# koide3/small_gicp

Measured on AMD Instinct MI355X. Metric: GICP iterations/sec (1M<->1M pts), higher is better.
Workload: dtype f32; 1 GPU; C3: GICP, per-point covariances k=20, 1000000 target <-> 1000000 source points, max_corr_dist 1.0 m; parallelism=single GPU

## Files before the change

include/small_gicp_amd_debug.h:

```cpp
#ifndef SMALL_GICP_AMD_DEBUG_H
#define SMALL_GICP_AMD_DEBUG_H

#include "small_gicp_amd.h"

#ifdef __cplusplus
extern "C" {
#endif

int sga_problem_set_search_stats(sga_context* ctx, sga_problem* pb, int enabled);
int sga_problem_get_search_stats(sga_context* ctx, const sga_problem* pb, int* leaves_per_point);
int sga_problem_get_sorted_points(sga_context* ctx, const sga_problem* pb, float* xyzw);
int sga_problem_get_last_plan(const sga_problem* pb, int out[8]);
int sga_problem_get_grid_stats(const sga_problem* pb, uint64_t out[6]);
void sga_set_grid_mode(int mode, long long min_points);
void sga_set_knn_wave_max(long long max_points);
int sga_index_spacing(const sga_index* index, double* spacing);
int sga_debug_kd_tree(sga_context* ctx, const sga_index* index, int* depth, float* nodes, float* xyzw);
int sga_debug_timer_start(sga_context* ctx);
int sga_debug_timer_stop(sga_context* ctx, double* ms);
#define SGA_FRAME_CHECK_DOUBLES 32
void sga_debug_shard_frame_pack(const double origin[3], double out[SGA_FRAME_CHECK_DOUBLES]);
int sga_debug_shard_frame_agree(const double sum[SGA_FRAME_CHECK_DOUBLES]);
int sga_debug_kd_trips(unsigned long long* out16);
int sga_debug_kd_wave_times(unsigned long long* out, int waves);

#ifdef __cplusplus
}
#endif
#endif
```

small_gicp_amd/_lib.py:

```python
import ctypes as C
import os
import sys

_HERE = os.path.dirname(os.path.abspath(__file__))
LIB_PATH = os.environ.get("SGA_LIB_PATH") or os.path.join(_HERE, "lib", "libsmall_gicp_amd.so")

SGA_OK = 0
ICP, PLANE_ICP, GICP = 0, 1, 2
FLAT_NORMALS, FLAT_COVS = 1, 2
ROBUST_NONE, ROBUST_HUBER, ROBUST_CAUCHY = 0, 1, 2
LEVENBERG_MARQUARDT, GAUSS_NEWTON = 0, 1
MATH_FP32, MATH_FP64 = 0, 1
ACCUM_DOUBLES = 30


class SgaError(RuntimeError):
    pass


class FactorParams(C.Structure):
    _fields_ = [("factor_kind", C.c_int), ("robust_kind", C.c_int), ("robust_c", C.c_double), ("max_dist_sq", C.c_double), ("math_mode", C.c_int)]


class RegistrationSettingC(C.Structure):
# ... 62 lines not shown
    ("sga_index_create_voxelmap_from_voxels", C.c_int, [_vp, C.c_double, C.c_void_p, _dp, _dp, C.c_size_t, _pvp]),
    ("sga_index_create_flatmap_from_voxels", C.c_int, [_vp, C.c_double, C.c_void_p, C.c_void_p, _dp, _dp, C.c_int, C.c_size_t, _pvp]),
    ("sga_index_refresh_attributes", C.c_int, [_vp, _vp, _vp]),
    ("sga_index_clone", C.c_int, [_vp, _vp, _pvp]),
    ("sga_index_destroy", C.c_int, [_vp]),
    ("sga_index_size", C.c_int, [_vp, C.POINTER(C.c_size_t)]),
    ("sga_index_voxelmap_download", C.c_int, [_vp, _vp, C.POINTER(C.c_int32), _fp, _fp, C.POINTER(C.c_uint32)]),
    ("sga_voxelmap_create", C.c_int, [_vp, C.c_double, _pvp]),
    ("sga_voxelmap_insert", C.c_int, [_vp, _vp, _vp, _dp]),
    ("sga_voxelmap_set_lru", C.c_int, [_vp, C.c_uint32, C.c_uint32]),
    ("sga_flatmap_create", C.c_int, [_vp, C.c_double, _pvp]),
    ("sga_flatmap_set_setting", C.c_int, [_vp, C.c_double, C.c_uint32]),
    ("sga_voxelmap_set_search_offsets", C.c_int, [_vp, C.c_int]),
    ("sga_flatmap_download", C.c_int, [_vp, _vp, C.POINTER(C.c_int32), C.POINTER(C.c_uint32), _fp, _fp]),
    ("sga_flatmap_create_contents", C.c_int, [_vp, C.c_double, C.c_int, _pvp]),
    ("sga_flatmap_get_contents", C.c_int, [_vp, C.POINTER(C.c_int)]),
    ("sga_flatmap_download_contents", C.c_int, [_vp, _vp, C.POINTER(C.c_int32), C.POINTER(C.c_uint32), _fp, _fp, _fp]),
    ("sga_index_create_flatmap_from_voxels_contents", C.c_int, [_vp, C.c_double, C.c_void_p, C.c_void_p, _dp, _dp, _dp, C.c_int, C.c_size_t, _pvp]),
    ("sga_index_knn", C.c_int, [_vp, _vp, _fp, C.c_size_t, C.c_int, C.c_double, C.POINTER(C.c_int64), _fp]),
    ("sga_index_knn_f64", C.c_int, [_vp, _vp, _dp, C.c_size_t, C.c_int, C.c_double, C.POINTER(C.c_int64), _dp]),
    ("sga_index_build_projective", C.c_int, [_vp, _vp, C.c_int, C.c_int, _pvp]),
    ("sga_projective_set_search_window", C.c_int, [_vp, C.c_int, C.c_int]),
    ("sga_projective_set_border_modes", C.c_int, [_vp, C.c_int, C.c_int]),
    ("sga_projective_get_params", C.c_int, [_vp, C.POINTER(C.c_int)]),
    ("sga_projective_download_map", C.c_int, [_vp, _vp, C.POINTER(C.c_uint32)]),
    ("sga_factor_params_default", None, [C.POINTER(FactorParams)]),
    ("sga_problem_create", C.c_int, [_vp, _vp, _vp, _dp, _pvp]),
    ("sga_problem_create_from_index", C.c_int, [_vp, _vp, _vp, _dp, _pvp]),
    ("sga_problem_destroy", C.c_int, [_vp]),
    ("sga_linearize", C.c_int, [_vp, _vp, C.POINTER(FactorParams), _dp, _dp, _dp, _dp, C.POINTER(C.c_uint64)]),
    ("sga_error", C.c_int, [_vp, _vp, C.POINTER(FactorParams), _dp, _dp]),
    ("sga_linearize_async", C.c_int, [_vp, _vp, C.POINTER(FactorParams), _dp, _vp]),
    ("sga_error_async", C.c_int, [_vp, _vp, C.POINTER(FactorParams), _dp, _vp]),
    ("sga_comm_unique_id", C.c_int, [C.POINTER(C.c_ubyte)]),
    ("sga_comm_init", C.c_int, [_vp, C.c_int, C.c_int, C.POINTER(C.c_ubyte)]),
    ("sga_comm_destroy", C.c_int, [_vp]),
    ("sga_comm_init_callback", C.c_int, [_vp, C.c_int, C.c_int, ALLREDUCE_FN, _vp]),
    ("sga_error_model_eval", C.c_int, [_dp, _dp, _dp, _dp]),
    ("sga_unpack_accumulator", None, [_dp, _dp, _dp, _dp, C.POINTER(C.c_uint64)]),
    ("sga_problem_set_rejector", C.c_int, [_vp, REJECTOR_FN, _vp]),
    ("sga_linearize_per_point", C.c_int, [_vp, _vp, C.POINTER(FactorParams), _dp, _dp, C.POINTER(C.c_ubyte)]),
    ("sga_problem_get_factors", C.c_int, [_vp, _vp, C.POINTER(C.c_int64), _fp]),
    ("sga_context_set_stream_ordered", C.c_int, [_vp, C.c_int]),
    ("sga_context_set_profiling", C.c_int, [_vp, C.c_int]),
    ("sga_context_get_kernel_ms", C.c_int, [_vp, _dp, C.POINTER(C.c_uint64), _dp, C.POINTER(C.c_uint64)]),
    ("sga_context_get_comm_ms", C.c_int, [_vp, _dp, C.POINTER(C.c_uint64)]),
    ("sga_context_get_search_ms", C.c_int, [_vp, _dp, C.POINTER(C.c_uint64)]),
    ("sga_context_get_pass_ms", C.c_int, [_vp, _dp, C.POINTER(C.c_uint64), _dp, C.POINTER(C.c_uint64), _dp]),
    ("sga_set_warm_limit", None, [C.c_double]),
    ("sga_set_error_model", None, [C.c_int]),
    ("sga_problem_set_search_stats", C.c_int, [C.c_void_p, C.c_void_p, C.c_int]),
    ("sga_problem_get_search_stats", C.c_int, [C.c_void_p, C.c_void_p, C.c_void_p]),
    ("sga_problem_get_sorted_points", C.c_int, [C.c_void_p, C.c_void_p, C.c_void_p]),
    ("sga_problem_get_grid_stats", C.c_int, [C.c_void_p, C.POINTER(C.c_uint64)]),
    ("sga_problem_get_last_plan", C.c_int, [C.c_void_p, C.POINTER(C.c_int)]),
    ("sga_set_grid_mode", None, [C.c_int, C.c_longlong]),
    ("sga_host_alloc", C.c_int, [C.c_size_t, C.POINTER(C.c_void_p)]),
    ("sga_host_free", C.c_int, [C.c_void_p]),
    ("sga_index_spacing", C.c_int, [C.c_void_p, C.POINTER(C.c_double)]),
    ("sga_set_knn_wave_max", None, [C.c_longlong]),
    ("sga_debug_kd_tree", C.c_int, [C.c_void_p, C.c_void_p, C.POINTER(C.c_int), C.c_void_p, C.c_void_p]),
    ("sga_debug_timer_start", C.c_int, [C.c_void_p]),
    ("sga_debug_timer_stop", C.c_int, [C.c_void_p, C.POINTER(C.c_double)]),
    ("sga_debug_shard_frame_pack", None, [C.POINTER(C.c_double), C.POINTER(C.c_double)]),
    ("sga_debug_shard_frame_agree", C.c_int, [C.POINTER(C.c_double)]),
    ("sga_debug_kd_trips", C.c_int, [C.c_void_p]),
    ("sga_debug_kd_wave_times", C.c_int, [C.c_void_p, C.c_int]),
    ("sga_set_search_mode", None, [C.c_int, C.c_int, C.c_int]),
    ("sga_get_warm_limit", C.c_double, []),
    ("sga_problem_get_pass_stats", C.c_int, [_vp, _vp, C.POINTER(C.c_uint64), C.POINTER(C.c_uint64), C.POINTER(C.c_uint64)]),
    ("sga_registration_setting_default", None, [C.POINTER(RegistrationSettingC)]),
    ("sga_align", C.c_int, [_vp, _vp, _vp, _dp, C.POINTER(RegistrationSettingC), C.POINTER(ResultC)]),
    ("sga_align_problem", C.c_int, [_vp, _vp, _dp, C.POINTER(RegistrationSettingC), C.POINTER(ResultC)]),
    ("sga_multi_create", C.c_int, [C.POINTER(C.c_int), C.c_int, _pvp]),
    ("sga_multi_destroy", C.c_int, [_vp]),
    ("sga_multi_num_devices", C.c_int, [_vp]),
    ("sga_multi_set_target_f64", C.c_int, [_vp, _dp, _dp, _dp, C.c_size_t]),
    ("sga_multi_set_target_f32", C.c_int, [_vp, _fp, _fp, _fp, C.c_size_t]),
    ("sga_multi_set_source_f32", C.c_int, [_vp, _fp, _fp, _fp, C.c_size_t, _dp]),
    ("sga_multi_set_target_f32_origin", C.c_int, [_vp, _fp, _fp, _fp, C.c_size_t, _dp]),
    ("sga_multi_set_source_f32_origin", C.c_int, [_vp, _fp, _fp, _fp, C.c_size_t, _dp, _dp]),
    ("sga_multi_set_target_voxels", C.c_int, [_vp, C.c_double, C.c_void_p, _dp, _dp, C.c_size_t]),
    ("sga_multi_set_search_offsets", C.c_int, [_vp, C.c_int]),
    ("sga_multi_set_rejector", C.c_int, [_vp, C.c_void_p, _vp]),
    ("sga_multi_set_target_flat_voxels", C.c_int, [_vp, C.c_double, C.c_void_p, C.c_void_p, _dp, _dp, C.c_int, C.c_size_t]),
    ("sga_multi_set_source_f64", C.c_int, [_vp, _dp, _dp, _dp, C.c_size_t, _dp]),
    ("sga_multi_linearize", C.c_int, [_vp, C.POINTER(FactorParams), _dp, _dp, _dp, _dp, C.POINTER(C.c_uint64)]),
    ("sga_multi_error", C.c_int, [_vp, C.POINTER(FactorParams), _dp, _dp]),
    ("sga_multi_align", C.c_int, [_vp, _dp, C.POINTER(RegistrationSettingC), C.POINTER(ResultC)]),
    ("sga_multi_reset_search_state", C.c_int, [_vp]),
    ("sga_multi_get_factors", C.c_int, [_vp, C.c_void_p, C.c_void_p]),
    ("sga_optimize", C.c_int, [C.POINTER(RegistrationSettingC), _dp, LINEARIZE_FN, ERROR_FN, _vp, C.POINTER(ResultC)]),
    ("sga_se3_exp", None, [_dp, _dp]),
]

_LIB = None


def load():
    global _LIB
    if _LIB is not None:
        return _LIB
    if not os.path.exists(LIB_PATH):
        raise SgaError(f"{LIB_PATH} is missing: build it with `make lib` (hipcc --offload-arch=gfx950). There is no CPU fallback.")
    if "torch" in sys.modules or os.environ.get("SGA_WITH_TORCH", "0") == "1":
        import torch
# ... 14 lines not shown
```

small_gicp_amd/api.py:

```python
import ctypes as C

import numpy as np

from . import _lib
from ._lib import GICP, ICP, PLANE_ICP, FactorParams, RegistrationSettingC, ResultC, check, load

_FACTOR_BY_NAME = {"ICP": ICP, "PLANE_ICP": PLANE_ICP, "GICP": GICP, "VGICP": GICP}


def _fp(a):
    return None if a is None else a.ctypes.data_as(C.POINTER(C.c_float))


def _dp(a):
    return None if a is None else a.ctypes.data_as(C.POINTER(C.c_double))


def _T16(T):
    T = np.eye(4) if T is None else np.asarray(T, dtype=np.float64).reshape(4, 4)
    return np.ascontiguousarray(T.T).reshape(16)


class Context:

# ... 705 lines not shown

                    traceback.print_exc()
                    return 1

            self._rejector_cb = _lib.REJECTOR_FN(cb)
        check(load().sga_problem_set_rejector(self.h, self._rejector_cb, None))

    def linearize_per_point(self, factor_params, T):
        n = self.source.size()
        vals = np.zeros((n, 28))
        ok = np.zeros(n, np.uint8)
        t16 = _T16(T)
        check(load().sga_linearize_per_point(self.ctx.h, self.h, C.byref(factor_params), _dp(t16), _dp(vals), ok.ctypes.data_as(C.POINTER(C.c_ubyte))))
        H = np.zeros((n, 6, 6))
        iu = np.triu_indices(6)
        H[:, iu[0], iu[1]] = vals[:, :21]
        H[:, iu[1], iu[0]] = vals[:, :21]
        return ok.astype(bool), H, vals[:, 21:27].copy(), vals[:, 27].copy()

    def factors(self):
        n = self.source.size()
        ti = np.empty(n, np.int64)
        m6 = np.empty((n, 6), np.float32)
        check(load().sga_problem_get_factors(self.ctx.h, self.h, ti.ctypes.data_as(C.POINTER(C.c_int64)), _fp(m6)))
        return ti, m6

    ROUTES = ("factors", "grid", "certify", "fused_lane", "fused_queue", "queue", "lane")

    def last_plan(self):
        out = (C.c_int * 8)()
        check(load().sga_problem_get_last_plan(self.h, out))
        v = list(out)
        return {"route": self.ROUTES[v[0]], "warm": bool(v[1]), "grid": bool(v[2]), "pts": v[3], "tail": bool(v[4]), "chunk_tiles": v[5], "reduce_rows": v[6], "reduce_groups": v[7]}

    def align(self, setting, init_T=None):
        res = ResultC()
        t16 = _T16(init_T)
        check(load().sga_align_problem(self.ctx.h, self.h, _dp(t16), C.byref(setting), C.byref(res)))
        return RegistrationResult(res)

    def search_stats(self, enable=None):
        if enable is not None:
            check(load().sga_problem_set_search_stats(self.ctx.h, self.h, 1 if enable else 0))
            return None
        out = np.zeros(len(self.source), dtype=np.int32)
        check(load().sga_problem_get_search_stats(self.ctx.h, self.h, out.ctypes.data_as(C.c_void_p)))
        return out

    def sorted_points(self):
        out = np.zeros((len(self.source), 4), dtype=np.float32)
        check(load().sga_problem_get_sorted_points(self.ctx.h, self.h, out.ctypes.data_as(C.c_void_p)))
        return out

    def pass_stats(self):
        c, w, f = C.c_uint64(), C.c_uint64(), C.c_uint64()
        check(load().sga_problem_get_pass_stats(self.ctx.h, self.h, C.byref(c), C.byref(w), C.byref(f)))
        g = (C.c_uint64 * 6)()
        check(load().sga_problem_get_grid_stats(self.h, g))
        return {"cold_passes": c.value, "warm_passes": w.value, "walked_points": f.value, "grid_passes": g[0], "grid_open": g[1], "grid_rings": g[2], "grid_cell_m": g[3] * 1e-6,
                "adj_queries": g[4], "adj_unsettled": g[5]}


class MultiProblem:

    def __init__(self, devices, target, source, init_T=None):
        devs = (C.c_int * len(devices))(*[int(d) for d in devices])
        self.h = C.c_void_p()
        check(load().sga_multi_create(devs, len(devices), C.byref(self.h)))
        tp, tn, tc = self._pack(*target)
        check(load().sga_multi_set_target_f64(self.h, _dp(tp), _dp(tn) if tn is not None else None, _dp(tc) if tc is not None else None, len(tp)))
        sp, sn, sc = self._pack(*source)
        self.n_source = len(sp)
        check(load().sga_multi_set_source_f64(self.h, _dp(sp), _dp(sn) if sn is not None else None, _dp(sc) if sc is not None else None, len(sp), _dp(_T16(np.eye(4) if init_T is None else init_T))))

    @staticmethod
    def _pack(points, normals=None, covs=None):
        p = np.ones((len(points), 4))
        p[:, :3] = np.asarray(points, dtype=np.float64)[:, :3]
        nr = cv = None
        if normals is not None:
            nr = np.zeros((len(points), 4))
            nr[:, :3] = np.asarray(normals, dtype=np.float64)[:, :3]
        if covs is not None:
            cv = np.zeros((len(points), 4, 4))
            cv[:, :3, :3] = np.asarray(covs, dtype=np.float64)[:, :3, :3]
            cv = np.ascontiguousarray(cv.transpose(0, 2, 1))
        return np.ascontiguousarray(p), nr, cv

    def __del__(self):
        if getattr(self, "h", None):
            load().sga_multi_destroy(self.h)
            self.h = None

    def linearize(self, factor_params, T):
        H, b, e, n = np.zeros(36), np.zeros(6), C.c_double(), C.c_uint64()
        check(load().sga_multi_linearize(self.h, C.byref(factor_params), _dp(_T16(T)), _dp(H), _dp(b), C.byref(e), C.byref(n)))
        return H.reshape(6, 6), b, e.value, n.value

    def error(self, factor_params, T):
        e = C.c_double()
        check(load().sga_multi_error(self.h, C.byref(factor_params), _dp(_T16(T)), C.byref(e)))
        return e.value

    def align(self, setting, init_T=None):
        res = ResultC()
        check(load().sga_multi_align(self.h, _dp(_T16(np.eye(4) if init_T is None else init_T)), C.byref(setting), C.byref(res)))
# ... 150 lines not shown
```

small_gicp_amd/csrc/cell_grid.hip:

```cpp
#include "common.hpp"

#include <algorithm>
#include <cmath>
#include <rocprim/rocprim.hpp>

#include "cell_grid.hpp"
#include "device_math.hpp"
#include "kd_search.hpp"
#include "sort_util.hpp"

namespace sga {

int ensure_temp(sga_context* ctx, size_t bytes);
extern int g_grid_mode;
extern long long g_grid_min_points;

__global__ void grid_keys_kernel(const float4* __restrict__ kd_pts, uint32_t n, GridView g, uint32_t* __restrict__ keys, uint32_t* __restrict__ vals) {
  const uint32_t i = blockIdx.x * blockDim.x + threadIdx.x;
  if (i >= n) return;
  const float4 p = kd_pts[i];
  const int cx = grid_cell(p.x, g.ox, g.inv_h, g.nx), cy = grid_cell(p.y, g.oy, g.inv_h, g.ny), cz = grid_cell(p.z, g.oz, g.inv_h, g.nz);
  keys[i] = static_cast<uint32_t>((cz * g.ny + cy) * g.nx + cx);
  if (vals != nullptr) vals[i] = i;
}
// ... 94 lines not shown
        SGA_TRY(bitmap.reserve(words));
        SGA_HIP(hipMemsetAsync(bitmap.p, 0, words * sizeof(uint32_t), ctx->stream));
        hipLaunchKernelGGL(grid_mark_cells_kernel, dim3(std::min<uint32_t>(2048u, (un + 255u) / 256u)), block, 0, ctx->stream, idx->kd_pts.p, un, g, bitmap.p, d_count.p);
      } else {
        hipLaunchKernelGGL(grid_keys_kernel, grid, block, 0, ctx->stream, idx->kd_pts.p, un, g, keys.p, static_cast<uint32_t*>(nullptr));
        SGA_HIP(rocprim::radix_sort_keys(ctx->d_temp.p, tb, keys.p, keys2.p, n, 0, 32, ctx->stream));
        hipLaunchKernelGGL(grid_count_distinct_kernel, dim3(256), block, 0, ctx->stream, keys2.p, un, d_count.p);
      }
      uint32_t occupied = 0;
      SGA_HIP(hipMemcpyAsync(&occupied, d_count.p, sizeof(uint32_t), hipMemcpyDeviceToHost, ctx->stream));
      SGA_HIP(hipStreamSynchronize(ctx->stream));
      const double m = static_cast<double>(n) / std::max<uint32_t>(occupied, 1u);
      if (std::fabs(std::log(m / fill)) < 0.08) break;
      const double next = std::max(h_floor, h * std::sqrt(fill / m));
      if (next == h) break;
      h = next;
    }
  }
  h = std::max(h, h_floor);
  grid_geometry(idx, h);
  const double cells_d = grid_cells(idx);
  if (cells_d > 2.0e9 || cells_d > 4.0 * max_cells) {
    idx->grid_h = 0.f;
    return SGA_OK;
  }
  const size_t cells = static_cast<size_t>(cells_d);
  const GridView g0 = make_grid_view(idx);
  SGA_TRY(idx->grid_start.alloc(cells + 1));
  SGA_TRY(idx->grid_pts.alloc(n));
  hipLaunchKernelGGL(grid_keys_kernel, grid, block, 0, ctx->stream, idx->kd_pts.p, un, g0, keys.p, vals.p);
  SGA_TRY(sort_pairs(ctx, keys.p, keys2.p, vals.p, vals2.p, n, 0, 32));
  hipLaunchKernelGGL(grid_gather_kernel, grid, block, 0, ctx->stream, idx->kd_pts.p, vals2.p, un, idx->grid_pts.p);
  SGA_HIP(hipMemsetAsync(idx->grid_start.p, 0, (cells + 1) * sizeof(uint32_t), ctx->stream));
  hipLaunchKernelGGL(grid_histogram_kernel, grid, block, 0, ctx->stream, keys2.p, un, idx->grid_start.p);
  size_t sb = 0;
  SGA_HIP(rocprim::exclusive_scan(nullptr, sb, idx->grid_start.p, idx->grid_start.p, 0u, cells + 1, rocprim::plus<uint32_t>(), ctx->stream));
  SGA_TRY(ensure_temp(ctx, sb));
  SGA_HIP(rocprim::exclusive_scan(ctx->d_temp.p, sb, idx->grid_start.p, idx->grid_start.p, 0u, cells + 1, rocprim::plus<uint32_t>(), ctx->stream));
  SGA_HIP(hipGetLastError());
  SGA_HIP(hipStreamSynchronize(ctx->stream));
  if (getenv("SGA_GRID_VERBOSE")) fprintf(stderr, "[sga] cell grid: h = %.4f m, %d x %d x %d = %.1f M cells, eps %.2e\n", h, idx->grid_dim[0], idx->grid_dim[1], idx->grid_dim[2], cells_d * 1e-6, idx->grid_eps);
  return SGA_OK;
}

template <typename Real>
struct GridParams {
  const float4* __restrict__ src_pts;
  int n;
  GridView g;
  Rigid<Real> T;
  float bound2;
  int* __restrict__ nn;
  int* __restrict__ nn2;
  float* __restrict__ rex;
  int chunk_tiles;
  uint32_t* __restrict__ stats;
};

__device__ __forceinline__ int grid_tile_of_block() {
  const int nblk = gridDim.x, per_xcd = nblk >> 3, b = blockIdx.x;
  return b < 8 * per_xcd ? (b & 7) * per_xcd + (b >> 3) : b;
}

constexpr int kRing1Waves = 4;
template <typename Real>
__global__ __launch_bounds__(64 * kRing1Waves) void grid_ring1_kernel(const GridParams<Real> p) {
  const int tile = grid_tile_of_block() * kRing1Waves + static_cast<int>(threadIdx.x >> 6);
  const int i = tile * 64 + static_cast<int>(threadIdx.x & 63);
  if (i >= p.n) return;
  const GridView& g = p.g;
  const float4 ps = p.src_pts[i];
  Real x, y, z;
  transform_point<Real>(p.T, ps.x, ps.y, ps.z, x, y, z);
  const float qx = static_cast<float>(x), qy = static_cast<float>(y), qz = static_cast<float>(z);
  int nn, nn2;
  float rex, seen;
  if (grid_ring1_lane(g, qx, qy, qz, p.bound2, nn, nn2, rex, seen)) {
    p.nn[i] = nn;
    p.nn2[i] = nn2;
    p.rex[i] = rex;
  } else {
    p.rex[i] = seen < 3.0e38f ? -fmaxf(seen, 1e-30f) : -INFINITY;
  }
}

constexpr int kGridQueue = 1024;
constexpr int kGridLaneRings = 3;

template <typename Real>
__global__ __launch_bounds__(64) void grid_finish_kernel(const GridParams<Real> p) {
  __shared__ int q_idx[kGridQueue];
  const int lane = threadIdx.x;
  const GridView& g = p.g;
  const int num_tiles = (p.n + 63) >> 6;
  const int nchunks = (num_tiles + p.chunk_tiles - 1) / p.chunk_tiles;
  const int per_xcd = nchunks >> 3, b = blockIdx.x;
  const int chunk = b < 8 * per_xcd ? (b & 7) * per_xcd + (b >> 3) : b;
  int total = 0;
  for (int t = 0; t < p.chunk_tiles; t++) {
    const int tile = chunk * p.chunk_tiles + t;
    const int i = tile * 64 + lane;
    const bool open = tile < num_tiles && i < p.n && p.rex[i] < 0.f;
    const unsigned long long m = __ballot(open);
    if (open) q_idx[total + __popcll(m & ((1ull << lane) - 1ull))] = i;
    total += __popcll(m);
  }
  if (total == 0) return;
  __syncthreads();
  const float reach = sqrtf(p.bound2) * 1.00001f;
  unsigned ring_sum = 0;
  for (int k0 = 0; k0 < total; k0 += 64) {
    const bool active = k0 + lane < total;
    const int i = active ? q_idx[k0 + lane] : 0;
    float qx = 0.f, qy = 0.f, qz = 0.f, seen = INFINITY;
    int cx = 1, cy = 1, cz = 1, r = 2;
    if (active) {
      const float4 ps = p.src_pts[i];
      Real x, y, z;
      transform_point<Real>(p.T, ps.x, ps.y, ps.z, x, y, z);
      qx = static_cast<float>(x), qy = static_cast<float>(y), qz = static_cast<float>(z);
      cx = grid_cell(qx, g.ox, g.inv_h, g.nx), cy = grid_cell(qy, g.oy, g.inv_h, g.ny), cz = grid_cell(qz, g.oz, g.inv_h, g.nz);
      seen = -p.rex[i];
      if (seen < 3.0e38f) r = grid_ring_for(g, fminf(seen * 1.00001f, reach), qx, qy, qz, cx, cy, cz);
    }
    bool done = !active;
    for (;;) {
      const bool mine = !done && r <= kGridLaneRings;
      int R = mine ? r : 0;
#pragma unroll
      for (int sft = 32; sft >= 1; sft >>= 1) R = max(R, __shfl_xor(R, sft, 64));
      if (R == 0) break;
      if (mine) ring_sum += static_cast<unsigned>(r);
      GridTop3 t = grid_top3();
      const int xlo = max(cx - r, 0), xhi = min(cx + r, g.nx - 1);
      for (int dz = -R; dz <= R; dz++) {
        const int zz = cz + dz;
        const bool zok = mine && dz >= -r && dz <= r && zz >= 0 && zz < g.nz;
        uint32_t s[8], e[8];
#pragma unroll
        for (int u = 0; u < 8; u++) {
          const int dy = u - R, yy = cy + dy;
          const bool ok = zok && u <= 2 * R && dy >= -r && dy <= r && yy >= 0 && yy < g.ny;
          s[u] = e[u] = 0u;
          if (ok) {
            const int row = (zz * g.ny + yy) * g.nx;
            s[u] = g.start[row + xlo];
            e[u] = g.start[row + xhi + 1];
          }
        }
#pragma unroll
        for (int u = 0; u < 8; u++) grid_scan_run(g, s[u], e[u], qx, qy, qz, t);
      }
      if (mine) {
        int nn, nn2;
        float rex;
        if (grid_settle(t, grid_rho2(g, qx, qy, qz, cx, cy, cz, r), p.bound2, nn, nn2, rex)) {
          p.nn[i] = nn;
          p.nn2[i] = nn2;
          p.rex[i] = rex;
          done = true;
        } else {
          const float d1 = sqrtf(grid_key_dist(t.k1));
          seen = fminf(seen, d1);
          r = seen < 3.0e38f ? max(r + 1, grid_ring_for(g, fminf(seen * 1.00001f, reach), qx, qy, qz, cx, cy, cz)) : r + 1;
        }
      }
    }
    unsigned long long open = __ballot(!done);
    while (open != 0ull) {
      const int l = __ffsll(static_cast<long long>(open)) - 1;
      open &= open - 1ull;
      const float ux = __shfl(qx, l, 64), uy = __shfl(qy, l, 64), uz = __shfl(qz, l, 64), useen = __shfl(seen, l, 64);
      const int ui = __shfl(i, l, 64);
      int nn, nn2;
      float rex;
      ring_sum += grid_settle_wave(g, lane, ux, uy, uz, useen, p.bound2, nn, nn2, rex);
      if (lane == 0) {
        p.nn[ui] = nn;
        p.nn2[ui] = nn2;
        p.rex[ui] = rex;
      }
    }
  }
  if (p.stats != nullptr) {
#pragma unroll
    for (int sft = 32; sft >= 1; sft >>= 1) ring_sum += __shfl_xor(ring_sum, sft, 64);
    if (lane == 0) {
      atomicAdd(&p.stats[0], static_cast<uint32_t>(total));
      atomicAdd(&p.stats[1], ring_sum);
    }
  }
}

template <typename Real>
int grid_search_pass(sga_context* ctx, const sga_index* idx, const float4* src_pts, int n, const Rigid<Real>& T, float reach2, int* nn, int* nn2, float* rex, uint32_t* stats) {
  static const int chunk_tiles = std::min(16, std::max(1, getenv("SGA_GRID_CHUNK") ? atoi(getenv("SGA_GRID_CHUNK")) : 4));
  GridParams<Real> p{};
  p.src_pts = src_pts;
  p.n = n;
  p.g = make_grid_view(idx);
  p.T = T;
  p.bound2 = reach2;
  p.nn = nn;
  p.nn2 = nn2;
  p.rex = rex;
  p.chunk_tiles = chunk_tiles;
  p.stats = stats;
  const int tiles = (n + 63) / 64;
  if (stats != nullptr) SGA_HIP(hipMemsetAsync(stats, 0, 2 * sizeof(uint32_t), ctx->stream));
  hipLaunchKernelGGL((grid_ring1_kernel<Real>), dim3((tiles + kRing1Waves - 1) / kRing1Waves), dim3(64 * kRing1Waves), 0, ctx->stream, p);
  hipLaunchKernelGGL((grid_finish_kernel<Real>), dim3((tiles + chunk_tiles - 1) / chunk_tiles), dim3(64), 0, ctx->stream, p);
  SGA_HIP(hipGetLastError());
  return SGA_OK;
}
template int grid_search_pass<float>(sga_context*, const sga_index*, const float4*, int, const Rigid<float>&, float, int*, int*, float*, uint32_t*);
template int grid_search_pass<double>(sga_context*, const sga_index*, const float4*, int, const Rigid<double>&, float, int*, int*, float*, uint32_t*);

int grid_rings_for(const sga_index* idx, double reach) {
  if (idx->grid_h <= 0.f) return -1;
  const double rings = std::ceil(reach / idx->grid_h) + 1.0;
  if ((2.0 * rings + 1.0) * (2.0 * rings + 1.0) > 1048576.0) return -1;
  return static_cast<int>(rings);
}

}
```

small_gicp_amd/csrc/cell_grid.hpp:

```cpp
#pragma once
#include <hip/hip_runtime.h>

#include "common.hpp"
#include "kd_search.hpp"

namespace sga {

struct GridView {
  const float4* __restrict__ pts;
  const uint32_t* __restrict__ start;
  float ox, oy, oz;
  float h, inv_h;
  float eps;
  int nx, ny, nz;
};

inline GridView make_grid_view(const sga_index* idx) {
  GridView g;
  g.pts = idx->grid_pts.p;
  g.start = idx->grid_start.p;
  g.ox = idx->grid_org[0], g.oy = idx->grid_org[1], g.oz = idx->grid_org[2];
  g.h = idx->grid_h;
  g.inv_h = 1.0f / idx->grid_h;
  g.eps = idx->grid_eps;
  g.nx = idx->grid_dim[0], g.ny = idx->grid_dim[1], g.nz = idx->grid_dim[2];
  return g;
}

__device__ __forceinline__ int grid_cell(float x, float o, float inv_h, int n) {
  const int c = static_cast<int>(floorf((x - o) * inv_h));
  return min(max(c, 1), n - 2);
}

struct GridTop3 {
  unsigned long long k1, k2;
  float d3;
};
constexpr unsigned long long kGridNoKey = (0x7f800000ull << 32) | 0x7fffffffull;
__device__ __forceinline__ GridTop3 grid_top3() { return {kGridNoKey, kGridNoKey, INFINITY}; }
__device__ __forceinline__ float grid_key_dist(unsigned long long k) { return __uint_as_float(static_cast<uint32_t>(k >> 32)); }
__device__ __forceinline__ int grid_key_pos(unsigned long long k) { return static_cast<int>(static_cast<uint32_t>(k)); }
__device__ __forceinline__ void grid_offer(GridTop3& s, float d, uint32_t pos) {
  const unsigned long long key = (static_cast<unsigned long long>(__float_as_uint(d)) << 32) | pos;
  const bool lt1 = key < s.k1, lt2 = key < s.k2;
  s.d3 = __builtin_amdgcn_fmed3f(grid_key_dist(s.k2), s.d3, d);
  s.k2 = lt1 ? s.k1 : (lt2 ? key : s.k2);
  s.k1 = lt1 ? key : s.k1;
}

struct GridBatch {
  float4 c[4];
};
__device__ __forceinline__ GridBatch grid_load4(const GridView& g, uint32_t j, uint32_t e) {
  GridBatch b;
#pragma unroll
  for (int u = 0; u < 4; u++) b.c[u] = g.pts[j + u < e ? j + u : 0u];
  return b;
}
__device__ __forceinline__ void grid_offer4(const GridBatch& b, uint32_t j, uint32_t e, float qx, float qy, float qz, GridTop3& t) {
#pragma unroll
  for (int u = 0; u < 4; u++) {
    const bool v = j + u < e;
    grid_offer(t, v ? kd_dist2(b.c[u].x, b.c[u].y, b.c[u].z, qx, qy, qz) : INFINITY, v ? __float_as_uint(b.c[u].w) : 0x7fffffffu);
  }
}
__device__ __forceinline__ void grid_scan_run(const GridView& g, uint32_t s, uint32_t e, float qx, float qy, float qz, GridTop3& t) {
  uint32_t j = s;
  while (__ballot(j < e) != 0ull) {
    const GridBatch b = grid_load4(g, j, e);
    grid_offer4(b, j, e, qx, qy, qz, t);
    j += 4u;
  }
}

__device__ __forceinline__ float grid_axis_rho(float q, float o, float h, int c, int r, int n) {
  float rho = INFINITY;
  const int a = c - r, b = c + r;
  if (a > 1) rho = fminf(rho, q - fmaf(static_cast<float>(a), h, o));
  if (b < n - 2) rho = fminf(rho, fmaf(static_cast<float>(b + 1), h, o) - q);
  return rho;
}
__device__ __forceinline__ float grid_rho2(const GridView& g, float qx, float qy, float qz, int cx, int cy, int cz, int r) {
  const float rho = fminf(fminf(grid_axis_rho(qx, g.ox, g.h, cx, r, g.nx), grid_axis_rho(qy, g.oy, g.h, cy, r, g.ny)), grid_axis_rho(qz, g.oz, g.h, cz, r, g.nz));
  if (!(rho < 3.0e38f)) return INFINITY;
  const float safe = (rho - g.eps) * 0.99999f;
  return safe > 0.f ? safe * safe : 0.f;
}

__device__ __forceinline__ float grid_rex_from_r2(float r2) { return sqrtf(r2) * 0.9999995f; }

__device__ __forceinline__ bool grid_settle(const GridTop3& t, float rho2, float bound2, int& nn, int& nn2, float& rex, bool* by_face = nullptr) {
  const float d1 = grid_key_dist(t.k1);
  const bool hit = d1 < bound2;
  const bool settled = d1 < rho2 || rho2 >= bound2;
  nn = hit ? grid_key_pos(t.k1) : -1;
  nn2 = (hit && t.k2 != kGridNoKey) ? grid_key_pos(t.k2) : -1;
  rex = grid_rex_from_r2(fminf(hit ? t.d3 : d1, rho2));
  if (by_face != nullptr) *by_face = rho2 < (hit ? t.d3 : d1);
  return settled;
}

__device__ __forceinline__ bool grid_ring1_lane(const GridView& g, float qx, float qy, float qz, float bound2, int& nn, int& nn2, float& rex, float& seen, bool* by_face = nullptr) {
  const int cx = grid_cell(qx, g.ox, g.inv_h, g.nx), cy = grid_cell(qy, g.oy, g.inv_h, g.ny), cz = grid_cell(qz, g.oz, g.inv_h, g.nz);
  uint32_t s[9], e[9];
#pragma unroll
  for (int r = 0; r < 9; r++) {
    constexpr int order[9] = {4, 3, 5, 1, 7, 0, 2, 6, 8};
    const int k = order[r];
    const int row = ((cz + k / 3 - 1) * g.ny + (cy + k % 3 - 1)) * g.nx + cx;
    s[r] = g.start[row - 1];
    e[r] = g.start[row + 2];
  }
  GridTop3 t = grid_top3();
  GridBatch nxt = grid_load4(g, s[0], e[0]);
#pragma unroll
  for (int r = 0; r < 9; r++) {
    const GridBatch cur = nxt;
    if (r + 1 < 9) nxt = grid_load4(g, s[r + 1], e[r + 1]);
    grid_offer4(cur, s[r], e[r], qx, qy, qz, t);
    grid_scan_run(g, s[r] + 4u, e[r], qx, qy, qz, t);
  }
  seen = t.k1 != kGridNoKey ? sqrtf(grid_key_dist(t.k1)) : INFINITY;
  return grid_settle(t, grid_rho2(g, qx, qy, qz, cx, cy, cz, 1), bound2, nn, nn2, rex, by_face);
}

__device__ __forceinline__ unsigned long long grid_wave_min_u64(unsigned long long v) {
#pragma unroll
  for (int sft = 32; sft >= 1; sft >>= 1) {
    const uint32_t lo = __shfl_xor(static_cast<uint32_t>(v), sft, 64), hi = __shfl_xor(static_cast<uint32_t>(v >> 32), sft, 64);
    const unsigned long long o = (static_cast<unsigned long long>(hi) << 32) | lo;
    v = o < v ? o : v;
  }
  return v;
}
__device__ __forceinline__ float grid_wave_min_f32(float v) {
#pragma unroll
  for (int sft = 32; sft >= 1; sft >>= 1) v = fminf(v, __shfl_xor(v, sft, 64));
  return v;
}

__device__ __forceinline__ int grid_ring_for(const GridView& g, float need, float qx, float qy, float qz, int cx, int cy, int cz) {
  const float fx = qx - fmaf(static_cast<float>(cx), g.h, g.ox), fy = qy - fmaf(static_cast<float>(cy), g.h, g.oy), fz = qz - fmaf(static_cast<float>(cz), g.h, g.oz);
  const float inside = fminf(fminf(fminf(fx, g.h - fx), fminf(fy, g.h - fy)), fminf(fz, g.h - fz));
  const float rr = ceilf((need - inside + 2.f * g.eps) * g.inv_h * 1.0001f);
  return static_cast<int>(fminf(fmaxf(rr, 2.f), 1.0e6f));
}

__device__ __forceinline__ unsigned grid_settle_wave(const GridView& g, int lane, float ux, float uy, float uz, float useen, float bound2, int& nn, int& nn2, float& rex) {
  const float reach = sqrtf(bound2) * 1.00001f;
  const int rcap = max(max(g.nx, g.ny), g.nz);
  const int ucx = grid_cell(ux, g.ox, g.inv_h, g.nx), ucy = grid_cell(uy, g.oy, g.inv_h, g.ny), ucz = grid_cell(uz, g.oz, g.inv_h, g.nz);
  int ur = min(grid_ring_for(g, fminf(useen * 1.00001f, reach), ux, uy, uz, ucx, ucy, ucz), rcap);
  unsigned ring_sum = 0;
  for (;;) {
    ring_sum += lane == 0 ? static_cast<unsigned>(ur) : 0u;
    const int W = 2 * ur + 1, rows = W * W;
    const float inv_w = 1.0f / static_cast<float>(W);
    const int xlo = max(ucx - ur, 0), xhi = min(ucx + ur, g.nx - 1);
    GridTop3 t = grid_top3();
    for (int base = 0; base < rows; base += 64) {
      const int k = base + lane;
      int a = static_cast<int>((static_cast<float>(k) + 0.5f) * inv_w);
      a -= a * W > k ? 1 : 0;
      a += (a + 1) * W <= k ? 1 : 0;
      const int zz = ucz + a - ur, yy = ucy + (k - a * W) - ur;
      uint32_t s = 0u, e = 0u;
      if (k < rows && zz >= 0 && zz < g.nz && yy >= 0 && yy < g.ny) {
        const int row = (zz * g.ny + yy) * g.nx;
        s = g.start[row + xlo];
        e = g.start[row + xhi + 1];
      }
      grid_scan_run(g, s, e, ux, uy, uz, t);
    }
    const unsigned long long g1 = grid_wave_min_u64(t.k1);
    const unsigned long long c2 = t.k1 == g1 ? t.k2 : t.k1;
    const unsigned long long g2 = grid_wave_min_u64(c2);
    const float third = t.k1 == g1 ? (t.k2 == g2 ? t.d3 : grid_key_dist(t.k2)) : (t.k1 == g2 ? grid_key_dist(t.k2) : grid_key_dist(t.k1));
    GridTop3 m;
    m.k1 = g1;
    m.k2 = g2;
    m.d3 = grid_wave_min_f32(third);
    if (grid_settle(m, grid_rho2(g, ux, uy, uz, ucx, ucy, ucz, ur), bound2, nn, nn2, rex)) return ring_sum;
    const float d1 = sqrtf(grid_key_dist(g1));
    ur = min(max(ur + 1, d1 < 3.0e38f ? grid_ring_for(g, fminf(d1 * 1.00001f, reach), ux, uy, uz, ucx, ucy, ucz) : ur + 1), rcap + 1);
  }
}

__device__ __forceinline__ bool grid_ring1_group(const GridView& g, int G, int gl, bool has, float qx, float qy, float qz, float bound2, int& nn, int& nn2, float& rex, float& seen, bool* by_face = nullptr) {
  const int cx = grid_cell(qx, g.ox, g.inv_h, g.nx), cy = grid_cell(qy, g.oy, g.inv_h, g.ny), cz = grid_cell(qz, g.oz, g.inv_h, g.nz);
  uint32_t off[9], pre[10];
  pre[0] = 0u;
#pragma unroll
  for (int r = 0; r < 9; r++) {
    const int row = ((cz + r / 3 - 1) * g.ny + (cy + r % 3 - 1)) * g.nx + cx;
    const uint32_t s = has ? g.start[row - 1] : 0u, e = has ? g.start[row + 2] : 0u;
    off[r] = s - pre[r];
    pre[r + 1] = pre[r] + (e - s);
  }
  const uint32_t total = pre[9];
  GridTop3 t = grid_top3();
  for (uint32_t c0 = static_cast<uint32_t>(gl); __ballot(c0 < total) != 0ull; c0 += 4u * static_cast<uint32_t>(G)) {
    float4 cand[4];
    bool ok[4];
#pragma unroll
    for (int u = 0; u < 4; u++) {
      const uint32_t c = c0 + static_cast<uint32_t>(u * G);
      ok[u] = c < total;
      uint32_t o = off[0];
#pragma unroll
      for (int r = 1; r < 9; r++) o = c >= pre[r] ? off[r] : o;
      cand[u] = g.pts[ok[u] ? c + o : 0u];
    }
#pragma unroll
    for (int u = 0; u < 4; u++) grid_offer(t, ok[u] ? kd_dist2(cand[u].x, cand[u].y, cand[u].z, qx, qy, qz) : INFINITY, ok[u] ? __float_as_uint(cand[u].w) : 0x7fffffffu);
  }
  auto min_u64 = [G](unsigned long long v) {
    for (int sft = G >> 1; sft >= 1; sft >>= 1) {
      const uint32_t lo = __shfl_xor(static_cast<uint32_t>(v), sft, 64), hi = __shfl_xor(static_cast<uint32_t>(v >> 32), sft, 64);
      const unsigned long long o = (static_cast<unsigned long long>(hi) << 32) | lo;
      v = o < v ? o : v;
    }
    return v;
  };
  const unsigned long long g1 = min_u64(t.k1);
  const unsigned long long c2 = t.k1 == g1 ? t.k2 : t.k1;
  const unsigned long long g2 = min_u64(c2);
  float third = t.k1 == g1 ? (t.k2 == g2 ? t.d3 : grid_key_dist(t.k2)) : (t.k1 == g2 ? grid_key_dist(t.k2) : grid_key_dist(t.k1));
  for (int sft = G >> 1; sft >= 1; sft >>= 1) third = fminf(third, __shfl_xor(third, sft, 64));
  GridTop3 m;
  m.k1 = g1, m.k2 = g2, m.d3 = third;
  seen = g1 != kGridNoKey ? sqrtf(grid_key_dist(g1)) : INFINITY;
  return grid_settle(m, grid_rho2(g, qx, qy, qz, cx, cy, cz, 1), bound2, nn, nn2, rex, by_face);
}

}
```

small_gicp_amd/csrc/common.hpp:

```cpp
#pragma once
#include <hip/hip_runtime.h>

#include <atomic>
#include <cstdarg>
#include <cstdint>
#include <cstdio>
#include <cstdlib>
#include <cstring>
#include <string>
#include <vector>

#include "../../include/small_gicp_amd.h"
#include "../../include/small_gicp_amd_debug.h"

namespace sga {

void set_error(const char* fmt, ...);
int fail(int code, const char* fmt, ...);

#define SGA_HIP(expr)                                                                                             \
  do {                                                                                                            \
    hipError_t _e = (expr);                                                                                       \
    if (_e != hipSuccess) return ::sga::fail(SGA_ERR_HIP, "%s:%d %s -> %s", __FILE__, __LINE__, #expr, hipGetErrorString(_e)); \
  } while (0)
// ... 169 lines not shown
  sga::DevBuf<float4> kd_boxes;
  sga::DevBuf<float4> kd_groups;
  sga::DevBuf<float4> kd_leaf;
  int kd_depth = 0;
  float bbox_lo[3] = {0, 0, 0}, bbox_hi[3] = {0, 0, 0};
  mutable std::atomic<double> spacing{0.0};
  mutable std::atomic<unsigned long long> spacing_seq{0};
  sga::DevBuf<float4> grid_pts;
  sga::DevBuf<uint32_t> grid_start;
  float grid_h = 0.f, grid_eps = 0.f;
  float grid_org[3] = {0, 0, 0};
  int grid_dim[3] = {0, 0, 0};
  sga::DevBuf<float4> pts;
  double leaf = 0.0;
  sga::DevBuf<unsigned long long> hkeys;
  sga::DevBuf<uint32_t> hvals;
  uint32_t hmask = 0;
  sga::DevBuf<int> vcoords;
  sga::DevBuf<uint32_t> vcounts;
  bool incremental = false;
  size_t vcap = 0;
  sga::DevBuf<double> vmean64;
  sga::DevBuf<double> vcov64;
  sga::DevBuf<uint32_t> vlru;
  uint32_t lru_counter = 0, lru_horizon = 100, lru_clear_cycle = 10;
  sga::DevBuf<double> fpts64;
  sga::DevBuf<double> fnrm64;
  sga::DevBuf<double> fcov64;
  uint32_t flat_max = 10;
  double flat_min_sq = 0.1 * 0.1;
  int search_offsets = 1;
  sga::DevBuf<uint32_t> proj_img;
  int proj_w = 0, proj_h = 0;
  int proj_win_h = 10, proj_win_v = 5;
  int proj_repeat_h = 1, proj_repeat_v = 0;
};

struct sga_problem {
  int device = 0;
  const sga_index* target = nullptr;
  size_t n = 0;
  double src_origin[3] = {0, 0, 0};
  bool frame_checked = false;
  bool has_normals = false, has_covs = false;
  sga::DevBuf<float4> pts;
  sga::DevBuf<sga::Cov8> cov;
  const float4* pts_view = nullptr;
  const sga::Cov8* cov_view = nullptr;
  const float4* src_pts() const { return pts_view ? pts_view : pts.p; }
  const sga::Cov8* src_cov() const { return cov_view ? cov_view : cov.p; }
  sga::DevBuf<int> corr;
  sga::DevBuf<int> hint;
  sga::DevBuf<int> hint2;
  sga::DevBuf<float> rex;
  sga::DevBuf<int> dbg_leaves;
  sga::DevBuf<uint32_t> walked;
  bool state_fresh = false;
  double T_prev[16] = {0};
  bool prev_valid = false;
  int prev_math = 0;
  int lin_factor = -1;
  double lin_T[16] = {0};
  bool maha_valid = false;
  int last_math = 0;
  float bbox_lo[3] = {0, 0, 0}, bbox_hi[3] = {0, 0, 0};
  uint64_t cold_passes = 0, warm_passes = 0;
  uint64_t grid_passes = 0;
  sga::DevBuf<uint32_t> grid_stats;
  bool grid_stats_pending = false;
  uint64_t grid_open_total = 0, grid_ring_total = 0;
  double grid_open_frac = 0.0;
  sga::DevBuf<uint32_t> tile_cost, tile_order;
  unsigned order_tiles = 0;
  hipStream_t order_stream = nullptr;
  sga::DevBuf<float> maha;
  sga::DevBuf<double> maha64;
  sga_rejector_fn rejector_fn = nullptr;
  void* rejector_user = nullptr;
  const double* caller_T = nullptr;
  sga::DevBuf<unsigned char> reject;
  bool model_valid = false;
  double model[96] = {0};
  double model_T[16] = {0};
  int last_plan[8] = {0};
  sga::DevBuf<double> partials;
};
```

small_gicp_amd/csrc/kd_search.hpp:

```cpp
#pragma once
#include <hip/hip_runtime.h>

#include "common.hpp"

namespace sga {

constexpr int kKdLeafMax = 8;
constexpr int kKdMaxDepth = 24;

struct KdView {
  const float4* __restrict__ pts;
  const float2* __restrict__ nodes;
  const float4* __restrict__ nodes4;
  const float4* __restrict__ boxes;
  const float4* __restrict__ groups;
  const float4* __restrict__ leafblk;
  uint32_t n;
  int depth;
  int gdepth;
  int glevels;
};

inline KdView make_kd_view(const sga_index* idx) {
  KdView k;
  k.pts = idx->kd_pts.p;
  k.nodes = idx->kd_nodes.p;
  k.nodes4 = idx->kd_nodes4.p;
  k.boxes = idx->kd_boxes.p;
  k.groups = idx->kd_groups.p;
  k.leafblk = idx->kd_leaf.p;
  k.n = static_cast<uint32_t>(idx->n);
  k.depth = idx->kd_depth;
  k.glevels = idx->kd_depth < 2 ? idx->kd_depth : 2;
  k.gdepth = idx->kd_depth - k.glevels;
  return k;
}

struct KdBest {
  float d2;
  int idx;
  int idx2;
  float r2;
  int leaves;
};

__host__ __device__ __forceinline__ uint32_t kd_bound(uint32_t n, int d, uint32_t k) { return static_cast<uint32_t>((static_cast<unsigned long long>(k) * n) >> d); }

__device__ __forceinline__ uint32_t kd_leaf_of(uint32_t i, uint32_t n, int d) {
  uint32_t k = static_cast<uint32_t>((static_cast<unsigned long long>(i) << d) / n);
  while (kd_bound(n, d, k + 1) <= i) k++;
  while (kd_bound(n, d, k) > i) k--;
  return k;
}

__host__ __device__ __forceinline__ uint32_t kd_pair_index(int , uint32_t node) { return node; }
__host__ __device__ __forceinline__ uint32_t kd_pair_count(int D) { return 1u << D; }

__device__ __forceinline__ uint32_t kd_pack(float cut, int depth) { return ((__float_as_uint(cut) >> 4) << 5) | static_cast<uint32_t>(depth); }
__device__ __forceinline__ float kd_cut(uint32_t e) { return __uint_as_float((e >> 5) << 4); }

__device__ __forceinline__ float kd_min(float a, float b) { return __builtin_amdgcn_fmed3f(a, b, -INFINITY); }

__device__ __forceinline__ float kd_dist2(float cx, float cy, float cz, float qx, float qy, float qz) {
  const float dx = cx - qx, dy = cy - qy, dz = cz - qz;
  return fmaf(dx, dx, fmaf(dy, dy, dz * dz));
}

__device__ __forceinline__ float kd_box_dist2(const KdView& t, uint32_t node, float qx, float qy, float qz) {
  const float4 lo = t.boxes[2 * node], hi = t.boxes[2 * node + 1];
  const float dx = fmaxf(fmaxf(lo.x - qx, qx - hi.x), 0.f);
  const float dy = fmaxf(fmaxf(lo.y - qy, qy - hi.y), 0.f);
  const float dz = fmaxf(fmaxf(lo.z - qz, qz - hi.z), 0.f);
  return fmaf(dx, dx, fmaf(dy, dy, dz * dz));
}

struct KdState {
  unsigned long long win;
  unsigned long long second;
  float third;
  float dropped;
  float prune0;
  float prune;
  float open;
  float slack;
  int leaves;
#ifdef SGA_KD_TRIPS
  int own[8], wav[8];
#endif
};
#ifdef SGA_KD_TRIPS
static __device__ unsigned long long g_kd_trips[16];
#define KD_TRIP(s, k)                                                                      \
  do {                                                                                     \
    (s).own[k]++;                                                                          \
    if (static_cast<int>(threadIdx.x & 63) == __ffsll(static_cast<long long>(__ballot(true))) - 1) (s).wav[k]++; \
  } while (0)
#else
#define KD_TRIP(s, k)
#endif

constexpr unsigned long long kKdNoPoint = (0x7f800000ull << 32) | 0xffffffffull;
__device__ __forceinline__ float kd_open_bound(float prune, float slack) {
  return slack > 0.f ? fmaf(slack, fmaf(2.f, sqrtf(prune), slack), prune) * 1.000001f : prune;
}
__device__ __forceinline__ KdState kd_state(float prune0, float slack = 0.f) {
  KdState s{};
  s.win = s.second = kKdNoPoint;
  s.third = s.dropped = INFINITY;
  s.prune0 = s.prune = prune0;
  s.open = kd_open_bound(prune0, slack);
  s.slack = slack;
  return s;
}
__device__ __forceinline__ float kd_key_dist(unsigned long long key) { return __uint_as_float(static_cast<uint32_t>(key >> 32)); }

__device__ __forceinline__ KdBest kd_result(const KdState& s, float bound2) {
  KdBest best;
  const float wd2 = kd_key_dist(s.win);
  const bool hit = wd2 < bound2;
  best.idx = hit ? static_cast<int>(static_cast<uint32_t>(s.win)) : -1;
  best.idx2 = (hit && s.second != kKdNoPoint) ? static_cast<int>(static_cast<uint32_t>(s.second)) : -1;
  best.d2 = hit ? wd2 : bound2;
  best.r2 = hit ? fminf(s.third, s.dropped) : fminf(wd2, s.dropped);
  best.leaves = s.leaves;
  return best;
}

__device__ __forceinline__ void kd_scan_leaf(const KdView& t, uint32_t leaf_node, float qx, float qy, float qz, KdState& s) {
  const uint32_t k = leaf_node - (1u << t.depth);
  const uint32_t first = kd_bound(t.n, t.depth, k);
  const uint32_t count = kd_bound(t.n, t.depth, k + 1) - first;
  const float4* __restrict__ lp = t.pts + first;
  float4 p[kKdLeafMax];
#pragma unroll
  for (int i = 0; i < kKdLeafMax; i++) p[i] = lp[i];
#pragma unroll
  for (int i = 0; i < kKdLeafMax; i++) {
    float d2 = kd_dist2(p[i].x, p[i].y, p[i].z, qx, qy, qz);
    d2 = static_cast<uint32_t>(i) < count ? d2 : INFINITY;
    s.third = __builtin_amdgcn_fmed3f(kd_key_dist(s.second), s.third, d2);
    const unsigned long long key = (static_cast<unsigned long long>(__float_as_uint(d2)) << 32) | (first + static_cast<uint32_t>(i));
    const bool before_win = key < s.win;
    const unsigned long long low = key < s.second ? key : s.second;
    s.second = before_win ? s.win : low;
    s.win = before_win ? key : s.win;
  }
  s.prune = fminf(s.prune0, kd_key_dist(s.win));
  s.open = kd_open_bound(s.prune, s.slack);
  s.leaves++;
  KD_TRIP(s, 3);
}

constexpr float kKdFar = 1e18f;
constexpr uint32_t kKdNoneKey = 0x7149f2cau;
struct KdFast {
  uint32_t w1, w2, w3;
  uint32_t l1, l2;
  float dropped;
  float prune0;
  float open;
  float slack;
  int leaves;
#ifdef SGA_KD_TRIPS
  int own[8], wav[8];
#endif
};
__device__ __forceinline__ KdFast kd_fast_state(float prune0, float slack = 0.f) {
  KdFast s{};
  s.w1 = s.w2 = s.w3 = 0xffffffffu;
  s.l1 = s.l2 = 0u;
  s.dropped = INFINITY;
  s.prune0 = prune0;
  s.open = kd_open_bound(prune0, slack);
  s.slack = slack;
  return s;
}
__device__ __forceinline__ uint32_t kd_umed3(uint32_t a, uint32_t b, uint32_t c) { return max(min(a, b), min(max(a, b), c)); }
__device__ __forceinline__ float kd_key_hi(uint32_t key) { return key < kKdNoneKey ? __uint_as_float(key | 7u) : INFINITY; }
__device__ __forceinline__ float kd_key_lo(uint32_t key) { return key < kKdNoneKey ? __uint_as_float(key & ~7u) : INFINITY; }

typedef float kd_f32x2 __attribute__((ext_vector_type(2)));
__device__ __forceinline__ void kd_scan_leaf(const KdView& t, uint32_t leaf_node, float qx, float qy, float qz, KdFast& s) {
  const uint32_t k = leaf_node - (1u << t.depth);
  const float4* __restrict__ b = t.leafblk + 8ull * k;
  const float4 x0 = b[0], x1 = b[1], y0 = b[2], y1 = b[3], z0 = b[4], z1 = b[5];
  const kd_f32x2 X[4] = {{x0.x, x0.y}, {x0.z, x0.w}, {x1.x, x1.y}, {x1.z, x1.w}};
  const kd_f32x2 Y[4] = {{y0.x, y0.y}, {y0.z, y0.w}, {y1.x, y1.y}, {y1.z, y1.w}};
  const kd_f32x2 Z[4] = {{z0.x, z0.y}, {z0.z, z0.w}, {z1.x, z1.y}, {z1.z, z1.w}};
  const uint32_t o1 = s.w1, o2 = s.w2;
#pragma unroll
  for (int i = 0; i < 4; i++) {
    const kd_f32x2 dx = X[i] - qx, dy = Y[i] - qy, dz = Z[i] - qz;
    const kd_f32x2 d2 = __builtin_elementwise_fma(dx, dx, __builtin_elementwise_fma(dy, dy, dz * dz));
    const uint32_t k0 = (__float_as_uint(d2.x) & ~7u) | static_cast<uint32_t>(2 * i), k1 = (__float_as_uint(d2.y) & ~7u) | static_cast<uint32_t>(2 * i + 1);
    s.w3 = kd_umed3(s.w2, s.w3, k0);
    s.w2 = kd_umed3(s.w1, s.w2, k0);
    s.w1 = min(s.w1, k0);
    s.w3 = kd_umed3(s.w2, s.w3, k1);
    s.w2 = kd_umed3(s.w1, s.w2, k1);
    s.w1 = min(s.w1, k1);
  }
  s.l2 = s.w2 != o2 ? (s.w2 == o1 ? s.l1 : k) : s.l2;
  s.l1 = s.w1 != o1 ? k : s.l1;
  s.open = kd_open_bound(fminf(s.prune0, kd_key_hi(s.w1)), s.slack);
  s.leaves++;
  KD_TRIP(s, 3);
}

__device__ __forceinline__ float kd_box_dist2_vals(float lox, float loy, float loz, float hix, float hiy, float hiz, float qx, float qy, float qz) {
  const float dx = fmaxf(fmaxf(lox - qx, qx - hix), 0.f);
  const float dy = fmaxf(fmaxf(loy - qy, qy - hiy), 0.f);
  const float dz = fmaxf(fmaxf(loz - qz, qz - hiz), 0.f);
  return fmaf(dx, dx, fmaf(dy, dy, dz * dz));
}

template <class S>
__device__ __forceinline__ void kd_visit_group(const KdView& t, uint32_t gnode, float qx, float qy, float qz, S& s) {
  const float4* __restrict__ h = t.groups + 8ull * (gnode - (1u << t.gdepth));
  const float4 lox = h[0], loy = h[1], loz = h[2], hix = h[3], hiy = h[4], hiz = h[5];
  float lb0 = kd_box_dist2_vals(lox.x, loy.x, loz.x, hix.x, hiy.x, hiz.x, qx, qy, qz);
  float lb1 = kd_box_dist2_vals(lox.y, loy.y, loz.y, hix.y, hiy.y, hiz.y, qx, qy, qz);
  float lb2 = kd_box_dist2_vals(lox.z, loy.z, loz.z, hix.z, hiy.z, hiz.z, qx, qy, qz);
  float lb3 = kd_box_dist2_vals(lox.w, loy.w, loz.w, hix.w, hiy.w, hiz.w, qx, qy, qz);
  const uint32_t leaf0 = gnode << t.glevels;
  KD_TRIP(s, 2);
  for (int trip = 0; trip < 4; trip++) {
    float m = lb0;
    uint32_t l = 0;
    if (lb1 < m) m = lb1, l = 1;
    if (lb2 < m) m = lb2, l = 2;
    if (lb3 < m) m = lb3, l = 3;
    if (!(m <= s.open)) break;
    kd_scan_leaf(t, leaf0 + l, qx, qy, qz, s);
    lb0 = l == 0 ? INFINITY : lb0;
    lb1 = l == 1 ? INFINITY : lb1;
    lb2 = l == 2 ? INFINITY : lb2;
    lb3 = l == 3 ? INFINITY : lb3;
  }
  s.dropped = kd_min(s.dropped, fminf(fminf(lb0, lb1), fminf(lb2, lb3)));
}

template <int STRIDE, class S>
__device__ __forceinline__ void kd_walk(const KdView& t, float qx, float qy, float qz, S& s, uint32_t node, int depth, int sp, uint32_t* __restrict__ stack, int tid) {
  const int D = t.gdepth;
  for (;;) {
    KD_TRIP(s, 5);
    while (depth < D) {
      KD_TRIP(s, 1);
      const int odd = depth & 1;
      typedef unsigned int u32x4 __attribute__((ext_vector_type(4)));
      u32x4 raw;
      asm volatile("global_load_dwordx4 %0, %1, off\n\ts_waitcnt vmcnt(0)" : "=v"(raw) : "v"(t.nodes4 + kd_pair_index(depth - odd, node >> odd)) : "memory");
      const float4 nd = make_float4(__uint_as_float(raw.x), __uint_as_float(raw.y), __uint_as_float(raw.z), __uint_as_float(raw.w));
      const uint32_t axes = raw.w;
// ... 135 lines not shown
      const float qa = axis == 0 ? qx : (axis == 1 ? qy : qz);
      const float diff = qa - nd.x;
      const float cut = diff * diff;
      depth++;
      stack[sp * STRIDE + tid] = kd_pack(cut, depth);
      const bool keep = cut <= s.open;
      sp += keep ? 1 : 0;
      s.dropped = kd_min(s.dropped, keep ? INFINITY : cut);
      node = 2 * node + (diff < 0.f ? 0u : 1u);
    }
    if (depth < D) {
      const uint32_t right = node & 1u;
      const uint32_t axis = (axes >> (2u + 2u * right)) & 3u;
      const float thr = right ? nd.z : nd.y;
      const float qa = axis == 0 ? qx : (axis == 1 ? qy : qz);
      const float diff = qa - thr;
      const float cut = diff * diff;
      depth++;
      stack[sp * STRIDE + tid] = kd_pack(cut, depth);
      const bool keep = cut <= s.open;
      sp += keep ? 1 : 0;
      s.dropped = kd_min(s.dropped, keep ? INFINITY : cut);
      node = 2 * node + (diff < 0.f ? 0u : 1u);
    }
  }
}

template <int STRIDE, class S>
__device__ __forceinline__ bool kd_pop(const KdView& t, float qx, float qy, float qz, S& s, uint32_t& node, int& depth, int& sp, const uint32_t* __restrict__ stack, int tid) {
  const int D = t.gdepth;
  uint32_t e = 0;
  bool found = false;
  while (sp > 0 && !found) {
    sp--;
    e = stack[sp * STRIDE + tid];
    float lb = kd_cut(e);
    if (lb <= s.open) {
      lb = fmaxf(lb, kd_box_dist2(t, (node >> (D - static_cast<int>(e & 31u))) ^ 1u, qx, qy, qz));
      found = lb <= s.open;
    }
    s.dropped = kd_min(s.dropped, found ? INFINITY : lb);
  }
  if (found) {
    depth = static_cast<int>(e & 31u);
    node = (node >> (D - depth)) ^ 1u;
  }
  return found;
}

__device__ __forceinline__ float kd_next_up(float d2) { return __uint_as_float(__float_as_uint(d2) + 1u); }

template <int STRIDE>
__device__ __forceinline__ KdBest kd_nearest(const KdView& t, float qx, float qy, float qz, float bound2, int seed, uint32_t* __restrict__ stack, int tid, float slack = 0.f) {
  if (t.n == 0) return {bound2, -1, -1, INFINITY, 0};
  float prune0 = bound2;
  if (seed >= 0 && static_cast<uint32_t>(seed) < t.n) {
    const float4 c = t.pts[seed];
    const float d2 = kd_dist2(c.x, c.y, c.z, qx, qy, qz);
    prune0 = d2 < prune0 ? kd_next_up(d2) : prune0;
  }
  KdState s = kd_state(prune0, slack);
  const int D = t.gdepth;
  int sp = 0, depth = 0;
  uint32_t node = 1;
  {
    const unsigned long long active = __ballot(true);
    while (depth < D) {
      KD_TRIP(s, 0);
      const uint32_t un = __builtin_amdgcn_readfirstlane(node);
      const float2 nd = t.nodes[un];
      const int axis = __builtin_amdgcn_readfirstlane(__float_as_int(nd.y));
      const float thr = __int_as_float(__builtin_amdgcn_readfirstlane(__float_as_int(nd.x)));
      const float qa = axis == 0 ? qx : (axis == 1 ? qy : qz);
      const float diff = qa - thr;
      const unsigned long long right = __ballot(!(diff < 0.f));
      if (right != 0ull && right != active) break;
      const float cut = diff * diff;
      depth++;
      stack[sp * STRIDE + tid] = kd_pack(cut, depth);
      const bool keep = cut <= s.open;
      sp += keep ? 1 : 0;
      s.dropped = kd_min(s.dropped, keep ? INFINITY : cut);
      node = 2 * un + (right != 0ull ? 1u : 0u);
    }
  }
  kd_walk<STRIDE>(t, qx, qy, qz, s, node, depth, sp, stack, tid);
#if defined(SGA_KD_TRIPS) && !defined(SGA_KD_NO_COUNT)
  for (int k = 0; k < 8; k++) {
    atomicAdd(&g_kd_trips[k], static_cast<unsigned long long>(s.own[k]));
    atomicAdd(&g_kd_trips[8 + k], static_cast<unsigned long long>(s.wav[k]));
  }
#endif
  return kd_result(s, bound2);
}

struct KdBestFast {
  KdBest best;
  bool ambiguous;
};
__device__ __forceinline__ KdBestFast kd_result(const KdView& t, const KdFast& s, float bound2) {
  KdBestFast r;
  const bool none = s.w1 >= kKdNoneKey;
  const float lo = kd_key_lo(s.w1), hi = kd_key_hi(s.w1);
  const bool hit = !none && hi < bound2;
  const bool miss = none ? bound2 <= 1e30f : !(lo < bound2);
  r.ambiguous = !(hit || miss) || (hit && ((s.w1 ^ s.w2) < 8u));
  r.best.idx = hit ? static_cast<int>(kd_bound(t.n, t.depth, s.l1) + (s.w1 & 7u)) : -1;
  r.best.idx2 = (hit && s.w2 < kKdNoneKey) ? static_cast<int>(kd_bound(t.n, t.depth, s.l2) + (s.w2 & 7u)) : -1;
  r.best.d2 = hit ? lo : bound2;
  r.best.r2 = hit ? fminf(kd_key_lo(s.w3), s.dropped) : fminf(lo, s.dropped);
  r.best.leaves = s.leaves;
  return r;
}

template <int STRIDE>
__device__ __forceinline__ KdBestFast kd_nearest_fast(const KdView& t, float qx, float qy, float qz, float bound2, int seed, uint32_t* __restrict__ stack, int tid, float slack = 0.f) {
  if (t.n == 0) return {{bound2, -1, -1, INFINITY, 0}, false};
  float prune0 = bound2;
  if (seed >= 0 && static_cast<uint32_t>(seed) < t.n) {
    const float4 c = t.pts[seed];
    const float d2 = kd_dist2(c.x, c.y, c.z, qx, qy, qz);
    prune0 = d2 < prune0 ? kd_next_up(d2) : prune0;
  }
  KdFast s = kd_fast_state(prune0, slack);
  const int D = t.gdepth;
  int sp = 0, depth = 0;
  uint32_t node = 1;
  {
    const unsigned long long active = __ballot(true);
    while (depth < D) {
      KD_TRIP(s, 0);
      const uint32_t un = __builtin_amdgcn_readfirstlane(node);
      const float2 nd = t.nodes[un];
      const int axis = __builtin_amdgcn_readfirstlane(__float_as_int(nd.y));
      const float thr = __int_as_float(__builtin_amdgcn_readfirstlane(__float_as_int(nd.x)));
      const float qa = axis == 0 ? qx : (axis == 1 ? qy : qz);
      const float diff = qa - thr;
      const unsigned long long right = __ballot(!(diff < 0.f));
      if (right != 0ull && right != active) break;
      const float cut = diff * diff;
      depth++;
      stack[sp * STRIDE + tid] = kd_pack(cut, depth);
      const bool keep = cut <= s.open;
      sp += keep ? 1 : 0;
      s.dropped = kd_min(s.dropped, keep ? INFINITY : cut);
      node = 2 * un + (right != 0ull ? 1u : 0u);
    }
  }
  kd_walk<STRIDE>(t, qx, qy, qz, s, node, depth, sp, stack, tid);
#if defined(SGA_KD_TRIPS) && !defined(SGA_KD_NO_COUNT)
  for (int k = 0; k < 8; k++) {
    atomicAdd(&g_kd_trips[k], static_cast<unsigned long long>(s.own[k]));
    atomicAdd(&g_kd_trips[8 + k], static_cast<unsigned long long>(s.wav[k]));
  }
#endif
  return kd_result(t, s, bound2);
}


template <int STRIDE>
__device__ __forceinline__ void kd_knn(const KdView& t, float qx, float qy, float qz, int k, float bound2, float* __restrict__ sd, int* __restrict__ si, uint32_t* __restrict__ stack, int tid, bool sort_result = true,
                                       uint32_t pre_first = 0, uint32_t pre_end = 0, const float4* __restrict__ pre_pts = nullptr ,
                                       uint32_t pre_own_first = 0, uint32_t pre_own_end = 0 ) {
  if (t.n == 0) return;
  const int D = t.depth;
  float worst = bound2;
  int worst_id = 0x7fffffff;
  int worst_slot = 0, count = 0;
  auto scan_range = [&](uint32_t first, uint32_t end, bool skip_pre) {
    for (uint32_t j0 = first; j0 < end; j0 += 4) {
// ... 312 lines not shown
```

small_gicp_amd/csrc/linearize.hip:

```cpp
#include <algorithm>
#include <chrono>
#include <thread>
#include <type_traits>
#include <utility>

#include "common.hpp"
#include "device_math.hpp"
#include "cell_grid.hpp"
#include "kd_search.hpp"
#include "projective.hpp"
#include "voxel_hash.hpp"

void sga_profile_collect_pending(sga_context* ctx);

namespace sga {

int comm_allreduce_sum(sga_context* ctx, double* d_buf, size_t count);
template <typename Real>
int grid_search_pass(sga_context* ctx, const sga_index* idx, const float4* src_pts, int n, const Rigid<Real>& T, float reach2, int* nn, int* nn2, float* rex, uint32_t* stats);
int grid_rings_for(const sga_index* idx, double reach);

#ifndef SGA_SPACING_REF
#define SGA_SPACING_REF 0.5486
#endif
constexpr int kTile = 256;
constexpr int kRow = 96;
constexpr int kCols = 128;
constexpr int kModelOff = 32;
constexpr int kModelCols = 95;
constexpr int kStatsCol = 30;
constexpr int kSearchBlock = 64;
#ifndef SGA_MAX_BLOCKS
#define SGA_MAX_BLOCKS 2048
#endif
constexpr int kMaxBlocks = SGA_MAX_BLOCKS;

constexpr int kFuseMaxBlocks = 32;
constexpr int kSeqWord = 128;
struct FusedTail {
  int enabled;
  unsigned* ticket;
  double* out;
  int out_n;
  double* host;
  unsigned long long seq;
};

__host__ __device__ inline double derived_entry(int col, const double* m);
__host__ __device__ inline bool is_derived_col(int c);

__device__ __forceinline__ void fused_tail(const FusedTail& f, const double* __restrict__ partials, int nrows, int ncols, int row_stride, bool derive = false) {
  __shared__ unsigned sh_last;
  asm volatile("s_waitcnt vmcnt(0)" ::: "memory");
  __syncthreads();
  if (threadIdx.x == 0) sh_last = __hip_atomic_fetch_add(f.ticket, 1u, __ATOMIC_ACQ_REL, __HIP_MEMORY_SCOPE_AGENT) == static_cast<unsigned>(nrows - 1) ? 1u : 0u;
  __syncthreads();
  if (!sh_last) return;
  __shared__ double sh_slice[2][kCols];
  {
    const int c = threadIdx.x & (kCols - 1), sl = threadIdx.x / kCols;
    double t = 0.0;
    if (c < ncols && sl < 2)
      for (int r = sl; r < nrows; r += 2) t += __hip_atomic_load(&partials[static_cast<size_t>(r) * row_stride + c], __ATOMIC_RELAXED, __HIP_MEMORY_SCOPE_AGENT);
    if (sl < 2) sh_slice[sl][c] = t;
  }
  __syncthreads();
  if (derive) {
    if (threadIdx.x < kCols) sh_slice[0][threadIdx.x] += sh_slice[1][threadIdx.x];
    __syncthreads();
    if (threadIdx.x < kCols) sh_slice[1][threadIdx.x] = 0.0;
    __syncthreads();
  }
  if (threadIdx.x < kCols) {
    const int c = threadIdx.x;
    const double t = (derive && is_derived_col(c)) ? derived_entry(c, sh_slice[0]) : sh_slice[0][c] + sh_slice[1][c];
    if (c < f.out_n) {
      const double v = c < ncols ? t : 0.0;
      f.out[c] = v;
      if (f.host != nullptr) f.host[c] = v;
    }
  }
  if (threadIdx.x == 0) __hip_atomic_store(f.ticket, 0u, __ATOMIC_RELAXED, __HIP_MEMORY_SCOPE_AGENT);
  if (f.host != nullptr) {
    __threadfence_system();
    __syncthreads();
    if (threadIdx.x == 0) __hip_atomic_store(reinterpret_cast<unsigned long long*>(f.host + kSeqWord), f.seq, __ATOMIC_RELEASE, __HIP_MEMORY_SCOPE_SYSTEM);
  }
}

template <typename Real>
struct LinParams {
  const float4* __restrict__ src_pts;
  const Cov8* __restrict__ src_cov;
  int n;
  int num_tiles;
  const float4* __restrict__ tgt_pts;
  const float4* __restrict__ tgt_nrm;
  const Cov8* __restrict__ tgt_cov;
  KdView kd;
  VoxelView vox;
  FlatView flat;
  int* __restrict__ corr;
  const int* __restrict__ hint;
  const unsigned char* __restrict__ reject;
  Real* __restrict__ maha;
  int store_maha;
  Rigid<Real> T;
  Real max_sq;
  float bound2;
  int robust_kind;
  Real robust_c;
  double* __restrict__ partials;
  FusedTail tail;
  int* __restrict__ cert_nn;
  int* __restrict__ cert_nn2;
  float* __restrict__ cert_rex;
  uint32_t* __restrict__ cert_walked;
  Rigid<Real> T_prev;
  float cert_within2, cert_slack_min, cert_slack_max;
  float cert_pad;
};

__device__ __forceinline__ void tile_schedule(int num_tiles, int& first, int& stride, int& end, int nblocks = 0) {
  if (nblocks == 0) nblocks = gridDim.x;
  if (nblocks % 8 == 0 && num_tiles >= nblocks) {
    const int xcd = blockIdx.x & 7, slot = blockIdx.x >> 3, per_xcd_blocks = nblocks >> 3;
    const int t0 = static_cast<int>((static_cast<long long>(num_tiles) * xcd) >> 3);
    const int t1 = static_cast<int>((static_cast<long long>(num_tiles) * (xcd + 1)) >> 3);
    first = t0 + slot;
    stride = per_xcd_blocks;
    end = t1;
  } else {
    first = blockIdx.x;
    stride = nblocks;
    end = num_tiles;
  }
}

template <typename Real>
__device__ __forceinline__ Sym3<Real> load_sym(const Cov8* __restrict__ c, int i) {
  const float4 a = reinterpret_cast<const float4*>(c)[2 * i];
  const float4 b = reinterpret_cast<const float4*>(c)[2 * i + 1];
  return {Real(a.x), Real(a.y), Real(a.z), Real(a.w), Real(b.x), Real(b.y)};
}

__device__ __forceinline__ float rex_from_r2(float r2) { return sqrtf(r2) * 0.9999995f; }

constexpr float kSearchMargin = 0.05f;

template <typename Real>
struct NNParams {
  const float4* __restrict__ src_pts;
  int n;
  KdView kd;
  Rigid<Real> T;
  float bound2;
  float within2;
  float slack_min, slack_max;
  float cert_pad;
  int* __restrict__ nn;
  int* __restrict__ nn2;
  float* __restrict__ rex;
  int check;
  Rigid<Real> T_prev;
  uint32_t* __restrict__ walked;
  const uint32_t* __restrict__ tile_order;
  uint32_t* __restrict__ tile_cost;
  int* __restrict__ leaves;
  double inv_leaf;
  int chunk_tiles;
  int fast;
  GridView grid;
  int grid_walk;
};

__device__ __forceinline__ float certify(float rex, float moved, bool has_neighbour, float d2_new, float within2, float pad) {
  const float lim = rex - moved * 1.000001f;
  const float lim_d = lim - moved * pad;
  const float lim2 = lim_d > 0.f ? lim_d * lim_d * 0.999995f : -1.f;
  const bool ok = has_neighbour ? d2_new < lim2 : lim2 > within2;
  return ok ? lim * 0.9999995f : -1.f;
}

template <typename Real, int BLOCK>
__device__ __forceinline__ int walk_lane(const NNParams<Real>& p, int i, float fx, float fy, float fz, int seed, float slack, uint32_t* __restrict__ kd_stack, int tid) {
  KdBest nb{};
  bool exact = p.fast == 0;
  if (!exact) {
    const KdBestFast f = kd_nearest_fast<BLOCK>(p.kd, fx, fy, fz, p.bound2, seed, kd_stack, tid, slack);
    nb = f.best;
    exact = f.ambiguous;
  }
  if (exact) nb = kd_nearest<BLOCK>(p.kd, fx, fy, fz, p.bound2, seed, kd_stack, tid, slack);
  p.nn[i] = nb.idx;
  p.nn2[i] = nb.idx2;
  p.rex[i] = rex_from_r2(nb.r2);
  if (p.leaves != nullptr) p.leaves[i] = nb.leaves;
  return nb.idx;
}

template <typename Real, int BLOCK, bool CHECK>
__device__ __forceinline__ int search_lane(const NNParams<Real>& p, int tile, int i, const float4& ps, float fx, float fy, float fz, uint32_t* __restrict__ kd_stack) {
  int seed = p.nn[i];
  float slack = 0.f;
  if constexpr (CHECK) {
    Real ox, oy, oz;
    transform_point<Real>(p.T_prev, ps.x, ps.y, ps.z, ox, oy, oz);
    const float moved = sqrtf(kd_dist2(static_cast<float>(ox), static_cast<float>(oy), static_cast<float>(oz), fx, fy, fz));
    const int cand2 = p.nn2[i];
    float d1 = INFINITY, d2 = INFINITY;
    if (seed >= 0) {
      const float4 c = p.kd.pts[seed];
      d1 = kd_dist2(c.x, c.y, c.z, fx, fy, fz);
    }
    if (cand2 >= 0) {
      const float4 c = p.kd.pts[cand2];
      d2 = kd_dist2(c.x, c.y, c.z, fx, fy, fz);
    }
    const bool swap = cand2 >= 0 && (d2 < d1 || (d2 == d1 && cand2 < seed));
    const int best = swap ? cand2 : seed;
    const float r = certify(p.rex[i], moved, best >= 0, swap ? d2 : d1, p.within2, p.cert_pad);
    if (r >= 0.f) {
      p.rex[i] = r;
      if (swap) {
        p.nn[i] = cand2;
        p.nn2[i] = seed;
      }
      return best;
    }
    seed = best;
    slack = fminf(fmaxf(moved, p.slack_min), p.slack_max);
    const unsigned long long walking = __ballot(true);
    if (threadIdx.x == __ffsll(static_cast<long long>(walking)) - 1) p.walked[tile] += static_cast<uint32_t>(__popcll(walking));
    if (p.grid_walk & 2) {
      int g_nn, g_nn2;
      float g_rex, g_seen;
      bool g_face = false;
      if (grid_ring1_lane(p.grid, fx, fy, fz, p.bound2, g_nn, g_nn2, g_rex, g_seen, &g_face) && !(g_face && g_nn >= 0 && (p.grid_walk & 32) && g_rex - g_seen < slack)) {
        p.nn[i] = g_nn;
        p.nn2[i] = g_nn2;
        p.rex[i] = g_rex;
        return g_nn;
      }
    }
  }
  return walk_lane<Real, BLOCK>(p, i, fx, fy, fz, seed, CHECK ? slack : 0.f, kd_stack, threadIdx.x);
}

__device__ __forceinline__ int search_tile_of_block(int nblk = 0) {
  if (nblk == 0) nblk = gridDim.x;
  const int per_xcd = nblk >> 3, b = blockIdx.x;
  return b < 8 * per_xcd ? (b & 7) * per_xcd + (b >> 3) : b;
}

#ifdef SGA_KD_TRIPS
static __device__ unsigned long long g_kd_wave_times[2 * 32768];
#endif

template <typename Real, int BLOCK, bool CHECK>
__global__ __launch_bounds__(BLOCK) __attribute__((amdgpu_waves_per_eu(8, 8))) void nn_search_kernel(const NNParams<Real> p) {
  extern __shared__ uint32_t kd_stack[];
#ifdef SGA_KD_TRIPS
  const unsigned long long wave_t0 = wall_clock64();
#endif
  const int tile = search_tile_of_block();
  const int i = tile * BLOCK + threadIdx.x;
  if (i >= p.n) return;
  const float4 ps = p.src_pts[i];
  Real x, y, z;
  transform_point<Real>(p.T, ps.x, ps.y, ps.z, x, y, z);
  search_lane<Real, BLOCK, CHECK>(p, tile, i, ps, static_cast<float>(x), static_cast<float>(y), static_cast<float>(z), kd_stack);
#ifdef SGA_KD_TRIPS
  if (blockIdx.x < 32768) {
    const unsigned long long t1 = wall_clock64();
    if (threadIdx.x == __ffsll(static_cast<long long>(__ballot(true))) - 1) {
      g_kd_wave_times[2 * blockIdx.x] = wave_t0;
      g_kd_wave_times[2 * blockIdx.x + 1] = t1;
    }
  }
#endif
}

constexpr int kQueueCap = 128;
constexpr int kPathRecords = 10;

template <typename Real, int FACTOR, int TARGET, int PTS, bool FRESH_NN = false, bool CERT = false, bool STAGED = false>
__device__ __forceinline__ void linearize_group(const LinParams<Real>& p, int first, int stride, int limit, double* __restrict__ acc_row, int lane, unsigned long long* __restrict__ failed_masks = nullptr,
                                                const ProjView* __restrict__ proj = nullptr);
template <typename Real, int FACTOR, bool OWN_D2 = true>
__device__ __forceinline__ bool pair_moments(const LinParams<Real>& p, int i, int j, bool within_bound, Real qx, Real qy, Real qz, Real tx, Real ty, Real tz, Sym3<Real>& Mp, Real* g, Real& e, Sym3<Real>& M_out,
                                             const float4* nn_pre = nullptr);
template <typename Real, int PTS>
__device__ __forceinline__ void accumulate_moments(const Real (&P)[PTS][3], const Sym3<Real> (&Mp)[PTS], const Real (&G)[PTS][3], const Real (&E)[PTS], int inliers, double* __restrict__ acc_row, int lane);

template <typename Real, bool CHECK, int FACTOR = -1>
__global__ __launch_bounds__(64) __attribute__((amdgpu_waves_per_eu(4, 6))) void nn_search_queue_kernel(const NNParams<Real> p, const LinParams<Real> lp) {
  extern __shared__ uint32_t kd_stack[];
  __shared__ float4 q_pt[kQueueCap];
  __shared__ int q_idx[kQueueCap];
  __shared__ uint32_t q_leaf[kQueueCap];
  const int lane = threadIdx.x;
  const int D = p.kd.gdepth;
  const int num_tiles = (p.n + 63) >> 6;
  const int nblk = static_cast<int>(gridDim.x), per_xcd = nblk >> 3, b = blockIdx.x;
  const int chunk = b < 8 * per_xcd ? (b & 7) * per_xcd + (b >> 3) : b;
  int tile = chunk * p.chunk_tiles;
  const int tile_end = min(tile + p.chunk_tiles, num_tiles);
  int q_head = 0, q_count = 0;
#ifdef SGA_KD_TRIPS
  const unsigned long long qt0 = wall_clock64();
  unsigned long long qt_stage = 0, qt_last = qt0;
#endif

  bool busy = false, fresh = false;
  float qx = 0.f, qy = 0.f, qz = 0.f;
  int qi = -1;
  uint32_t node = 1;
  int depth = 0, sp = 0;
  KdState s = kd_state(p.bound2, 0.f);

  for (;;) {
    while (tile < tile_end && q_count <= kQueueCap - 64) {
      const int i = tile * 64 + lane;
      bool need = i < p.n;
      float fx = 0.f, fy = 0.f, fz = 0.f, slack = 0.f;
      int seed = -1, cand2 = -1;
      if (need) {
        const float4 ps = p.src_pts[i];
        Real x, y, z;
        transform_point<Real>(p.T, ps.x, ps.y, ps.z, x, y, z);
        fx = static_cast<float>(x), fy = static_cast<float>(y), fz = static_cast<float>(z);
        seed = p.nn[i];
        cand2 = p.nn2[i];
        if constexpr (CHECK) {
          Real ox, oy, oz;
          transform_point<Real>(p.T_prev, ps.x, ps.y, ps.z, ox, oy, oz);
          const float moved = sqrtf(kd_dist2(static_cast<float>(ox), static_cast<float>(oy), static_cast<float>(oz), fx, fy, fz));
          float d1 = INFINITY, d2 = INFINITY;
          if (seed >= 0) {
            const float4 c = p.kd.pts[seed];
            d1 = kd_dist2(c.x, c.y, c.z, fx, fy, fz);
          }
          if (cand2 >= 0) {
            const float4 c = p.kd.pts[cand2];
            d2 = kd_dist2(c.x, c.y, c.z, fx, fy, fz);
          }
          const bool swap = cand2 >= 0 && (d2 < d1 || (d2 == d1 && cand2 < seed));
          const int best = swap ? cand2 : seed;
          const float r = certify(p.rex[i], moved, best >= 0, swap ? d2 : d1, p.within2, p.cert_pad);
          if (r >= 0.f) {
            p.rex[i] = r;
            if (swap) {
              p.nn[i] = cand2;
              p.nn2[i] = seed;
            }
            need = false;
          }
          seed = best;
          slack = fminf(fmaxf(moved, p.slack_min), p.slack_max);
        }
      }
      uint32_t leaf = 0;
      const bool seeded = need && seed >= 0, remembered = need && seed < 0 && cand2 <= -2;
      if (seeded) leaf = (1u << D) + (kd_leaf_rank(static_cast<uint32_t>(seed), p.kd.n, p.kd.depth, p.inv_leaf) >> p.kd.glevels);
      if (remembered) leaf = (1u << D) + min(static_cast<uint32_t>(-2 - cand2), (1u << D) - 1u);
      if (__ballot(need && !seeded && !remembered) != 0ull) {
        if (need && !seeded && !remembered) leaf = kd_locate(p.kd, fx, fy, fz);
      }
      const unsigned long long mask = __ballot(need);
      if (mask != 0ull) {
        if (need) {
          const int rank = __builtin_amdgcn_mbcnt_hi(static_cast<uint32_t>(mask >> 32), __builtin_amdgcn_mbcnt_lo(static_cast<uint32_t>(mask), 0u));
          const int slot = (q_head + q_count + rank) & (kQueueCap - 1);
          q_pt[slot] = make_float4(fx, fy, fz, slack);
          q_idx[slot] = i;
          q_leaf[slot] = leaf;
        }
        const int added = __popcll(mask);
        if constexpr (CHECK) {
          if (lane == 0) p.walked[tile] += static_cast<uint32_t>(added);
        }
        q_count += added;
      }
      tile++;
    }
#ifdef SGA_KD_TRIPS
    {
      const unsigned long long now = wall_clock64();
      qt_stage += now - qt_last;
      qt_last = now;
    }
#endif
    const unsigned long long idle = __ballot(!busy);
    if (q_count > 0 && idle != 0ull) {
      const int rank = __builtin_amdgcn_mbcnt_hi(static_cast<uint32_t>(idle >> 32), __builtin_amdgcn_mbcnt_lo(static_cast<uint32_t>(idle), 0u));
      if (!busy && rank < q_count) {
        const int slot = (q_head + rank) & (kQueueCap - 1);
        const float4 e = q_pt[slot];
        qx = e.x, qy = e.y, qz = e.z;
        qi = q_idx[slot];
        node = q_leaf[slot];
        depth = D;
        sp = 0;
        s = kd_state(p.bound2, CHECK ? e.w : 0.f);
        busy = true;
        fresh = true;
      }
      const int taken = min(__popcll(idle), q_count);
      q_head = (q_head + taken) & (kQueueCap - 1);
      q_count -= taken;
      if constexpr (CHECK) {
        if (p.grid_walk & 4) {
          const bool trying = busy && fresh;
          if (__ballot(trying) != 0ull) {
            if (trying) {
              int g_nn, g_nn2;
              float g_rex, g_seen;
              bool g_face = false;
              if (grid_ring1_lane(p.grid, qx, qy, qz, p.bound2, g_nn, g_nn2, g_rex, g_seen, &g_face) && !(g_face && g_nn >= 0 && (p.grid_walk & 32) && g_rex - g_seen < s.slack)) {
                p.nn[qi] = g_nn;
                p.nn2[qi] = g_nn2;
                p.rex[qi] = g_rex;
                busy = false;
                fresh = false;
              }
            }
          }
        }
      }
    }
    if (__ballot(busy) == 0ull) {
      if (tile >= tile_end && q_count == 0) break;
      continue;
    }
    if (busy) {
      kd_descend<64>(p.kd, qx, qy, qz, s, node, depth, sp, kd_stack, lane);
      kd_visit_group(p.kd, node, qx, qy, qz, s);
    }
    if (__ballot(fresh) != 0ull) {
      if (fresh) {
        kd_push_path<64, kPathRecords>(p.kd, node, 0, qx, qy, qz, s, sp, kd_stack, lane);
        if (D > 2 * kPathRecords) kd_push_path<64, kKdMaxDepth / 2 - kPathRecords>(p.kd, node, 2 * kPathRecords, qx, qy, qz, s, sp, kd_stack, lane);
        fresh = false;
      }
    }
    if (busy) {
      if (!kd_pop<64>(p.kd, qx, qy, qz, s, node, depth, sp, kd_stack, lane)) {
        const KdBest nb = kd_result(s, p.bound2);
        p.nn[qi] = nb.idx;
        p.nn2[qi] = nb.idx >= 0 ? nb.idx2 : -2 - static_cast<int>(node - (1u << D));
        p.rex[qi] = rex_from_r2(nb.r2);
        busy = false;
      }
    }
  }
#ifdef SGA_KD_TRIPS
  const unsigned long long qt1 = wall_clock64();
#endif
  if constexpr (FACTOR >= 0) {
    asm volatile("s_waitcnt vmcnt(0)" ::: "memory");
    __syncthreads();
    double* row = reinterpret_cast<double*>(kd_stack);
    for (int c = lane; c < kRow; c += 64) row[c] = 0.0;
    __syncthreads();
    const int limit = min(p.n, tile_end * 64);
    if (p.chunk_tiles == 1)
      linearize_group<Real, FACTOR, 0, 1, true>(lp, chunk * 64 + lane, 64, limit, row, lane);
    else
      for (int t0 = chunk * p.chunk_tiles; t0 < tile_end; t0 += 4) linearize_group<Real, FACTOR, 0, 4, true>(lp, t0 * 64 + lane, 64, limit, row, lane);
    __syncthreads();
    for (int c = lane; c < kRow; c += 64) lp.partials[static_cast<size_t>(chunk) * kRow + c] = row[c];
  }
#ifdef SGA_KD_TRIPS
  if (lane == 0) {
    const unsigned long long qt2 = wall_clock64();
    atomicAdd(&g_kd_trips[12], qt_stage);
    atomicAdd(&g_kd_trips[13], (qt1 - qt0) - qt_stage);
    atomicAdd(&g_kd_trips[14], qt2 - qt1);
    atomicAdd(&g_kd_trips[15], 1ull);
    if (blockIdx.x < 32768) {
      g_kd_wave_times[2 * blockIdx.x] = qt0;
      g_kd_wave_times[2 * blockIdx.x + 1] = qt2;
    }
  }
#endif
}

template <typename Real, int FACTOR>
__device__ __forceinline__ bool pair_factor(const LinParams<Real>& p, int i, int j, bool within_bound, Real px, Real py, Real pz, Real qx, Real qy, Real qz, Real tx, Real ty, Real tz, Real* vals, Sym3<Real>* Mp_out = nullptr,
                                            Real* g_out = nullptr) {
  const Real rx = tx - qx, ry = ty - qy, rz = tz - qz;
  const Real d2 = rx * rx + ry * ry + rz * rz;
  const bool inlier = (j >= 0) && within_bound && !(d2 > p.max_sq);
  if (inlier) {
    Sym3<Real> M;
    if constexpr (FACTOR == SGA_GICP) {
      const Sym3<Real> Cs = load_sym<Real>(p.src_cov, i);
      const Sym3<Real> Ct = load_sym<Real>(p.tgt_cov, j);
      const Sym3<Real> RCR = rotate_sym(p.T.r, Cs);
      M = inverse_sym<Real>({Ct.xx + RCR.xx, Ct.xy + RCR.xy, Ct.xz + RCR.xz, Ct.yy + RCR.yy, Ct.yz + RCR.yz, Ct.zz + RCR.zz});
      Real* m = p.maha + static_cast<size_t>(i) * 6;
      m[0] = M.xx;
      m[1] = M.xy;
// ... 170 lines not shown
  int inliers = 0;
  float4 ps4[PTS];
  int jn[PTS];
  bool act[PTS];
#pragma unroll
  for (int u = 0; u < PTS; u++) {
    const int i = first + u * stride;
    act[u] = i < limit;
    ps4[u] = act[u] ? p.src_pts[i] : make_float4(0.f, 0.f, 0.f, 0.f);
    jn[u] = -1;
    if constexpr (TARGET == 0 && CERT)
      jn[u] = act[u] ? p.cert_nn[i] : -1;
    else if constexpr (TARGET == 0)
      jn[u] = act[u] ? (FRESH_NN ? __hip_atomic_load(&p.hint[i], __ATOMIC_RELAXED, __HIP_MEMORY_SCOPE_AGENT) : p.hint[i]) : -1;
  }
  Real Q[PTS][3], Tg[PTS][3];
  bool within[PTS];
  {
  SGA_STAGE_PARAMS(p);
#pragma unroll
  for (int u = 0; u < PTS; u++) {
    P[u][0] = ps4[u].x, P[u][1] = ps4[u].y, P[u][2] = ps4[u].z;
    Q[u][0] = Q[u][1] = Q[u][2] = Real(0);
    if (act[u]) transform_point(p.T, P[u][0], P[u][1], P[u][2], Q[u][0], Q[u][1], Q[u][2]);
    Tg[u][0] = Tg[u][1] = Tg[u][2] = Real(0);
    within[u] = true;
    if constexpr (TARGET == 2) {
      if (act[u]) {
        float4 m = make_float4(0.f, 0.f, 0.f, 0.f);
        jn[u] = flat_nearest<Real>(p.flat, p.tgt_pts, Q[u][0], Q[u][1], Q[u][2], m);
        Tg[u][0] = m.x, Tg[u][1] = m.y, Tg[u][2] = m.z;
      }
    } else if constexpr (TARGET == 3) {
      if (act[u]) {
        Real d2 = Real(0);
        jn[u] = projective_nearest<Real>(*proj, p.tgt_pts, Q[u][0], Q[u][1], Q[u][2], d2);
        within[u] = jn[u] >= 0 && !(d2 > p.max_sq);
        const float4 m = jn[u] >= 0 ? p.tgt_pts[jn[u]] : make_float4(0.f, 0.f, 0.f, 0.f);
        Tg[u][0] = m.x, Tg[u][1] = m.y, Tg[u][2] = m.z;
      }
    } else if constexpr (TARGET == 1) {
      if (act[u]) {
        if (p.vox.offsets == 1)
          jn[u] = voxel_lookup(p.vox, static_cast<float>(Q[u][0]), static_cast<float>(Q[u][1]), static_cast<float>(Q[u][2]));
        else
          jn[u] = voxel_nearest<Real>(p.vox, p.tgt_pts, Q[u][0], Q[u][1], Q[u][2]);
      }
    }
  }
  }
  if constexpr (TARGET != 2 && TARGET != 3) {
    float4 m4[PTS];
    if constexpr (CERT && TARGET == 0) {
      int c2[PTS];
      float rx[PTS];
      float4 m4b[PTS];
      {
        SGA_STAGE_PARAMS(p);
#pragma unroll
        for (int u = 0; u < PTS; u++) {
          const int i = first + u * stride;
          c2[u] = act[u] ? p.cert_nn2[i] : -1;
          rx[u] = act[u] ? p.cert_rex[i] : 0.f;
        }
#pragma unroll
        for (int u = 0; u < PTS; u++) {
          m4[u] = jn[u] >= 0 ? p.tgt_pts[jn[u]] : make_float4(0.f, 0.f, 0.f, 0.f);
          m4b[u] = c2[u] >= 0 ? p.tgt_pts[c2[u]] : make_float4(0.f, 0.f, 0.f, 0.f);
        }
      }
      SGA_STAGE_PARAMS(p);
#pragma unroll
      for (int u = 0; u < PTS; u++) {
        const int i = first + u * stride;
        bool failed = false;
        if (act[u]) {
          const float fx = static_cast<float>(Q[u][0]), fy = static_cast<float>(Q[u][1]), fz = static_cast<float>(Q[u][2]);
          Real ox, oy, oz;
          transform_point<Real>(p.T_prev, P[u][0], P[u][1], P[u][2], ox, oy, oz);
          const float moved = sqrtf(kd_dist2(static_cast<float>(ox), static_cast<float>(oy), static_cast<float>(oz), fx, fy, fz));
          const float d1 = jn[u] >= 0 ? kd_dist2(m4[u].x, m4[u].y, m4[u].z, fx, fy, fz) : INFINITY;
          const float d2 = c2[u] >= 0 ? kd_dist2(m4b[u].x, m4b[u].y, m4b[u].z, fx, fy, fz) : INFINITY;
          const bool swap = c2[u] >= 0 && (d2 < d1 || (d2 == d1 && c2[u] < jn[u]));
          const int best = swap ? c2[u] : jn[u];
          const float r = certify(rx[u], moved, best >= 0, swap ? d2 : d1, p.cert_within2, p.cert_pad);
          failed = !(r >= 0.f);
          p.cert_rex[i] = failed ? -fminf(fmaxf(moved, p.cert_slack_min), p.cert_slack_max) : r;
          if (swap) {
            p.cert_nn[i] = c2[u];
            p.cert_nn2[i] = jn[u];
            m4[u] = m4b[u];
          }
          jn[u] = failed ? -1 : best;
        }
        const unsigned long long fm = __ballot(failed);
        if (lane == 0) {
          failed_masks[u] = fm;
          if (fm != 0ull) p.cert_walked[i >> 6] += static_cast<uint32_t>(__popcll(fm));
        }
        if (failed) act[u] = false;
      }
    } else {
#pragma unroll
      for (int u = 0; u < PTS; u++) m4[u] = jn[u] >= 0 ? p.tgt_pts[jn[u]] : make_float4(0.f, 0.f, 0.f, 0.f);
    }
    bool decided64[PTS];
#pragma unroll
    for (int u = 0; u < PTS; u++) decided64[u] = false;
    if constexpr (TARGET == 0 && !CERT && sizeof(Real) == 8) {
      if (p.cert_nn2 != nullptr) {
#pragma unroll
        for (int u = 0; u < PTS; u++) {
          const int i = first + u * stride;
          if (!act[u] || jn[u] < 0) continue;
          const int j2 = p.cert_nn2[i];
          const double ax = static_cast<double>(m4[u].x) - Q[u][0], ay = static_cast<double>(m4[u].y) - Q[u][1], az = static_cast<double>(m4[u].z) - Q[u][2];
          double d1 = ax * ax + ay * ay + az * az;
          if (j2 >= 0) {
            const float4 c = p.tgt_pts[j2];
            const double bx = static_cast<double>(c.x) - Q[u][0], by = static_cast<double>(c.y) - Q[u][1], bz = static_cast<double>(c.z) - Q[u][2];
            const double d2 = bx * bx + by * by + bz * bz;
            if (d2 < d1 || (d2 == d1 && j2 < jn[u])) {
              d1 = d2;
              jn[u] = j2;
              m4[u] = c;
            }
          }
          within[u] = d1 <= p.max_sq;
          if (p.reject != nullptr) within[u] = within[u] && p.reject[__float_as_uint(ps4[u].w)] == 0;
          decided64[u] = true;
        }
      }
    }
    SGA_STAGE_PARAMS(p);
#pragma unroll
    for (int u = 0; u < PTS; u++) {
      Tg[u][0] = m4[u].x, Tg[u][1] = m4[u].y, Tg[u][2] = m4[u].z;
      if constexpr (TARGET == 0) {
        if (jn[u] >= 0 && !decided64[u]) {
          within[u] = kd_dist2(m4[u].x, m4[u].y, m4[u].z, static_cast<float>(Q[u][0]), static_cast<float>(Q[u][1]), static_cast<float>(Q[u][2])) < p.bound2;
          if (p.reject != nullptr) within[u] = within[u] && p.reject[__float_as_uint(ps4[u].w)] == 0;
        }
      }
    }
  }
  Sym3<Real> Mh[PTS];
  bool inl[PTS];
  constexpr bool kFlatNormals = TARGET == 2 && FACTOR == SGA_PLANE_ICP;
  float4 nn4[kFlatNormals ? PTS : 1];
  if constexpr (kFlatNormals) {
    SGA_STAGE_PARAMS(p);
#pragma unroll
    for (int u = 0; u < PTS; u++) nn4[u] = act[u] && jn[u] >= 0 ? p.tgt_nrm[jn[u]] : make_float4(0.f, 0.f, 0.f, 0.f);
  }
  {
  SGA_STAGE_PARAMS(p);
#pragma unroll
  for (int u = 0; u < PTS; u++) {
    const int i = first + u * stride;
    inl[u] = false;
    Mp[u] = Sym3<Real>{};
    Mh[u] = Sym3<Real>{};
    G[u][0] = G[u][1] = G[u][2] = E[u] = Real(0);
    if (act[u]) inl[u] = pair_moments<Real, FACTOR, TARGET != 3>(p, i, jn[u], within[u], Q[u][0], Q[u][1], Q[u][2], Tg[u][0], Tg[u][1], Tg[u][2], Mp[u], G[u], E[u], Mh[u], kFlatNormals ? &nn4[u] : nullptr);
    inliers += __popcll(__ballot(inl[u]));
  }
  }
  SGA_STAGE_PARAMS(pw);
#pragma unroll
  for (int u = 0; u < PTS; u++) {
    const int i = first + u * stride;
    if (act[u]) {
      pw.corr[i] = inl[u] ? jn[u] : -1;
      if constexpr (FACTOR == SGA_GICP) {
        if (inl[u] && pw.store_maha) {
          Real* m = pw.maha + static_cast<size_t>(i) * 6;
          m[0] = Mh[u].xx, m[1] = Mh[u].xy, m[2] = Mh[u].xz, m[3] = Mh[u].yy, m[4] = Mh[u].yz, m[5] = Mh[u].zz;
// ... 57 lines not shown

#ifndef SGA_CERT_WAVES
#define SGA_CERT_WAVES 4
#endif
template <typename Real, int FACTOR, int PTS>
__global__ __launch_bounds__(kTile) __attribute__((amdgpu_waves_per_eu(SGA_CERT_WAVES))) void certify_linearize_kernel(const LinParams<Real> p, const NNParams<Real> q_arg) {
  extern __shared__ uint32_t kd_stack[];
  __shared__ double sh_acc[kTile / 64][kRow];
  __shared__ unsigned long long sh_failed[kTile / 64][PTS];
  __shared__ int sh_list[PTS * kTile];
  const int lane = threadIdx.x & 63, wave = threadIdx.x >> 6;
  for (int c = lane; c < kRow; c += 64) sh_acc[wave][c] = 0.0;
  double* acc_row = sh_acc[wave];

  int tile, stride, tile_end;
  tile_schedule(p.num_tiles, tile, stride, tile_end);
  for (; tile < tile_end; tile += stride) {
    const int base = tile * PTS * kTile;
    linearize_group<Real, FACTOR, 0, PTS, false, true, true>(p, base + static_cast<int>(threadIdx.x), kTile, p.n, acc_row, lane, sh_failed[wave]);
    __syncthreads();
    {
      int total = 0;
#pragma unroll
      for (int u = 0; u < PTS; u++)
#pragma unroll
        for (int w = 0; w < kTile / 64; w++) {
          const unsigned long long m = sh_failed[w][u];
          if (wave == 0 && ((m >> lane) & 1ull)) sh_list[total + __popcll(m & ((1ull << lane) - 1ull))] = base + u * kTile + w * 64 + lane;
          total += __popcll(m);
        }
      __syncthreads();
      using SearchArgs = const __attribute__((address_space(4))) NNParams<Real>;
      static_assert(alignof(NNParams<Real>) <= 8 && sizeof(LinParams<Real>) % 8 == 0, "kernel argument layout");
      SearchArgs* qa = (SearchArgs*)((const __attribute__((address_space(4))) char*)__builtin_amdgcn_kernarg_segment_ptr() + sizeof(LinParams<Real>));
      asm volatile("" : "+s"(qa));
      const NNParams<Real>& q = *(const NNParams<Real>*)qa;
      uint32_t* my_stack = kd_stack + static_cast<size_t>(wave) * static_cast<size_t>(max(q.kd.depth, 1)) * 64;
      int Gw = 1;
      if ((q.grid_walk & 8) && total > 0 && total <= kTile / 2) {
        Gw = 64;
        while (Gw * total > kTile) Gw >>= 1;
      }
      const int per_round = kTile / Gw;
      for (int k0 = 0; k0 < total; k0 += per_round) {
        const int sub = lane / Gw, gl = lane & (Gw - 1);
        const int k = k0 + 4 * sub + wave;
        const bool has = k < total, mine = has && gl == 0;
        const int i = has ? sh_list[k] : 0;
        Real P[1][3] = {{Real(0), Real(0), Real(0)}}, G[1][3] = {{Real(0), Real(0), Real(0)}}, E[1] = {Real(0)};
        Sym3<Real> Mp[1] = {Sym3<Real>{}};
        Sym3<Real> Mh{};
        bool inl = false;
        bool g_settled = false;
        int g_nn = -1, g_nn2 = -1;
        float g_rex = 0.f, g_seen = INFINITY;
        bool g_face = false;
        if (Gw > 1) {
          float gx = 0.f, gy = 0.f, gz = 0.f;
          if (has) {
            const float4 ps = p.src_pts[i];
            Real t[3];
            transform_point<Real>(p.T, Real(ps.x), Real(ps.y), Real(ps.z), t[0], t[1], t[2]);
            gx = static_cast<float>(t[0]), gy = static_cast<float>(t[1]), gz = static_cast<float>(t[2]);
          }
          g_settled = grid_ring1_group(q.grid, Gw, gl, has, gx, gy, gz, q.bound2, g_nn, g_nn2, g_rex, g_seen, &g_face);
        }
        if (mine) {
          const float4 ps = p.src_pts[i];
          P[0][0] = ps.x, P[0][1] = ps.y, P[0][2] = ps.z;
          Real t[3];
          transform_point<Real>(p.T, P[0][0], P[0][1], P[0][2], t[0], t[1], t[2]);
          const float fx = static_cast<float>(t[0]), fy = static_cast<float>(t[1]), fz = static_cast<float>(t[2]);
          int j = -1;
          bool settled = g_settled;
          if (Gw == 1 && (q.grid_walk & 1)) settled = grid_ring1_lane(q.grid, fx, fy, fz, q.bound2, g_nn, g_nn2, g_rex, g_seen, &g_face);
          if (settled && g_face && g_nn >= 0 && (q.grid_walk & 32)) {
            const float need = -__hip_atomic_load(&q.rex[i], __ATOMIC_RELAXED, __HIP_MEMORY_SCOPE_AGENT);
            if (g_rex - g_seen < need) settled = false;
          }
          if (settled) {
            q.nn[i] = g_nn;
            q.nn2[i] = g_nn2;
            q.rex[i] = g_rex;
            j = g_nn;
          }
          if (!settled) {
            const int seed = __hip_atomic_load(&q.nn[i], __ATOMIC_RELAXED, __HIP_MEMORY_SCOPE_AGENT);
            const float slack = -__hip_atomic_load(&q.rex[i], __ATOMIC_RELAXED, __HIP_MEMORY_SCOPE_AGENT);
            j = walk_lane<Real, 64>(q, i, fx, fy, fz, seed, slack, my_stack, lane);
          }
          if (j >= 0) {
            const float4 m = p.tgt_pts[j];
            const bool within = kd_dist2(m.x, m.y, m.z, fx, fy, fz) < p.bound2;
            inl = pair_moments<Real, FACTOR>(p, i, j, within, t[0], t[1], t[2], Real(m.x), Real(m.y), Real(m.z), Mp[0], G[0], E[0], Mh);
          }
          p.corr[i] = inl ? j : -1;
          if constexpr (FACTOR == SGA_GICP) {
            if (inl && p.store_maha) {
              Real* mm = p.maha + static_cast<size_t>(i) * 6;
              mm[0] = Mh.xx, mm[1] = Mh.xy, mm[2] = Mh.xz, mm[3] = Mh.yy, mm[4] = Mh.yz, mm[5] = Mh.zz;
            }
          }
        }
        const int inliers = __popcll(__ballot(inl));
        if (inliers > 0) accumulate_moments<Real, 1>(P, Mp, G, E, inliers, acc_row, lane);
      }
    }
    __syncthreads();
  }
  __syncthreads();
  if (threadIdx.x < kRow) {
    double t = 0.0;
#pragma unroll
    for (int w = 0; w < kTile / 64; w++) t += sh_acc[w][threadIdx.x];
    if (p.tail.enabled)
      __hip_atomic_store(&p.partials[static_cast<size_t>(blockIdx.x) * kRow + threadIdx.x], t, __ATOMIC_RELAXED, __HIP_MEMORY_SCOPE_AGENT);
    else
      p.partials[static_cast<size_t>(blockIdx.x) * kRow + threadIdx.x] = t;
  }
  if (p.tail.enabled) fused_tail(p.tail, p.partials, gridDim.x, kModelCols, kRow, true);
}

#ifndef SGA_SL_WAVES
#define SGA_SL_WAVES 7
#endif
#ifndef SGA_SL_WAVES_WARM
#define SGA_SL_WAVES_WARM 6
#endif
template <typename Real, int FACTOR, bool CHECK>
__global__ __launch_bounds__(64) __attribute__((amdgpu_waves_per_eu(CHECK ? SGA_SL_WAVES_WARM : SGA_SL_WAVES, CHECK ? SGA_SL_WAVES_WARM : SGA_SL_WAVES))) void search_linearize_kernel(const NNParams<Real> p, const LinParams<Real> lp) {
  extern __shared__ uint32_t kd_stack[];
#ifdef SGA_KD_TRIPS
  const unsigned long long wave_t0 = wall_clock64();
#endif
  const int lane = threadIdx.x;
// ... 423 lines not shown
  if constexpr (sizeof(Real) == 8) {
    if (rejects && p.n > 0 && max_sq_f < 3.0e38f) {
      double m2 = 0.0;
      for (int a = 0; a < 3; a++) {
        double ma = std::fabs(T[12 + a]);
        for (int b = 0; b < 3; b++) ma += std::fabs(T[4 * b + a]) * std::max(std::fabs(static_cast<double>(pb->bbox_lo[b])), std::fabs(static_cast<double>(pb->bbox_hi[b])));
        m2 += ma * ma;
      }
      const double r = std::sqrt(fp->max_dist_sq) + 0x1p-24 * (1.0 + 1e-6) * std::sqrt(m2);
      p.bound2 = std::max(p.bound2, static_cast<float>(r * r * (1.0 + 0x1p-20)));
    }
  }
  p.robust_kind = fp->robust_kind;
  p.robust_c = static_cast<Real>(fp->robust_c);
  return p;
}

template <typename Real>
static int linearize_dispatch(sga_context* ctx, sga_problem* pb, const sga_factor_params* fp, const double T[16], double* d_out30, double* host, unsigned long long seq, bool with_model = false) {
  const sga_index* idx = pb->target;
  const bool voxel = idx->kind != SGA_INDEX_KDTREE;
  const bool flat = idx->kind == SGA_INDEX_FLATMAP;
  const bool proj = idx->kind == SGA_INDEX_PROJECTIVE;
  if (fp->factor_kind == SGA_GICP && ((pb->n > 0 && !pb->has_covs) || (idx->n > 0 && !idx->has_covs))) return fail(SGA_ERR_INVALID, "GICP needs covariances on both source and target");
  if (fp->factor_kind == SGA_PLANE_ICP && proj && idx->n > 0 && !idx->has_normals) return fail(SGA_ERR_UNSUPPORTED, "PLANE_ICP needs a projective search over a target with normals");
  if (fp->factor_kind == SGA_PLANE_ICP && !proj && ((voxel && !flat) || ((flat || idx->n > 0) && !idx->has_normals)))
    return fail(SGA_ERR_UNSUPPORTED, "PLANE_ICP needs a kd-tree index over a target with normals");
  if (fp->factor_kind < 0 || fp->factor_kind > 2) return fail(SGA_ERR_INVALID, "invalid factor_kind %d", fp->factor_kind);

  if constexpr (sizeof(Real) == 8)
    if (pb->maha64.n < pb->n * 6) SGA_TRY(pb->maha64.alloc(pb->n * 6));
  const bool host_rejector = pb->rejector_fn != nullptr && !voxel;
  LinParams<Real> p = factor_params<Real>(pb, fp, T, host_rejector);
  if (flat) {
    p.flat.hkeys = idx->hkeys.p;
    p.flat.hvals = idx->hvals.p;
    p.flat.hmask = idx->hmask;
    p.flat.inv_leaf = 1.0 / idx->leaf;
    p.flat.vnum = idx->vcounts.p;
    p.flat.offsets = idx->search_offsets;
    for (int k = 0; k < 3; k++) p.flat.org[k] = idx->origin[k];
  } else if (proj) {
  } else if (voxel) {
    p.vox.hkeys = idx->hkeys.p;
    p.vox.hvals = idx->hvals.p;
    p.vox.hmask = idx->hmask;
    p.vox.inv_leaf = 1.0 / idx->leaf;
    for (int k = 0; k < 3; k++) p.vox.org[k] = idx->origin[k];
    p.vox.offsets = idx->search_offsets;
  } else {
    p.kd = make_kd_view(idx);
  }
  p.cert_nn2 = (!voxel && sizeof(Real) == 8) ? pb->hint2.p : nullptr;
  p.store_maha = fp->robust_kind != SGA_ROBUST_NONE ? 1 : 0;
  p.partials = pb->partials.p;
  const int ncols = kModelCols, out_n = with_model ? kRow : SGA_ACCUM_DOUBLES;

  const int math = sizeof(Real) == 4 ? SGA_MATH_FP32 : SGA_MATH_FP64;
  const double displacement = (!voxel && p.n > 0 && pb->prev_valid && pb->prev_math == math) ? max_displacement(T, pb->T_prev, pb->bbox_lo, pb->bbox_hi) : INFINITY;
  const double unit = voxel ? 1.0 : routing_unit(idx);
  NNParams<Real> q{};
  q.src_pts = pb->src_pts();
  q.n = p.n;
  q.kd = p.kd;
  q.T = p.T;
  q.within2 = p.bound2;
  q.slack_min = static_cast<float>(kSlackMin * unit), q.slack_max = static_cast<float>(kSlackMax * unit);
  q.cert_pad = std::max(g_cert_pad, 0.f);
  q.bound2 = p.bound2 * (1.f + kSearchMargin) * (1.f + kSearchMargin);
  q.nn = pb->hint.p, q.nn2 = pb->hint2.p, q.rex = pb->rex.p, q.walked = pb->walked.p;
  q.fast = g_fast_scan;
  q.leaves = pb->dbg_leaves.n >= pb->n ? pb->dbg_leaves.p : nullptr;

  const PassPlan plan = plan_pass<Real>(ctx, pb, q, displacement, unit, host_rejector);
  p.num_tiles = factor_tiles(p.n, plan.pts);
  const int blocks = grid_blocks(p.num_tiles);
  p.tail = FusedTail{plan.tail ? 1 : 0, ctx->d_ticket.p, d_out30, out_n, host, seq};
  q.check = plan.warm ? 1 : 0;
  if (plan.warm) q.T_prev = rigid_from_colmajor<Real>(pb->T_prev);
  if (plan.grid) {
    q.grid_walk = g_grid_walk;
    q.grid = make_grid_view(idx);
  }
  q.chunk_tiles = plan.chunk_tiles;

  const bool timed = ctx->profiling && (ctx->lin_seq++ % ctx->profile_period) == 0;
  if (timed) {
    sga_profile_collect_pending(ctx);
    (void)hipEventRecord(ctx->ev0, ctx->stream);
    ctx->pending_warm = plan.warm;
  }
  int rows = p.n > 0 ? blocks : 0;
  const bool first_pass = !pb->prev_valid;
  if (!voxel) pb->prev_valid = false;
  pb->state_fresh = false;
  if (plan.route != Route::kFactors) {
    if (q.leaves != nullptr) SGA_HIP(hipMemsetAsync(q.leaves, 0, pb->n * sizeof(int), ctx->stream));
    if (plan.grid && (first_pass || (plan.route != Route::kGrid && !plan.warm))) pb->grid_open_frac = 0.0;
    pb->order_tiles = 0;
    const size_t words = static_cast<size_t>(p.kd.depth);
    const dim3 sgrid((p.n + kSearchBlock - 1) / kSearchBlock), sblock(kSearchBlock);
    switch (plan.route) {
      case Route::kGrid:
        if (pb->grid_stats.n < 4) {
          SGA_TRY(pb->grid_stats.alloc(4));
          SGA_HIP(hipMemsetAsync(pb->grid_stats.p, 0, 4 * sizeof(uint32_t), ctx->stream));
        }
        SGA_TRY(grid_search_pass<Real>(ctx, idx, pb->src_pts(), p.n, p.T, q.bound2, pb->hint.p, pb->hint2.p, pb->rex.p, pb->grid_stats.p));
        pb->grid_passes++;
        break;
      case Route::kCertify:
        if constexpr (sizeof(Real) == 4) {
          p.cert_nn = q.nn, p.cert_nn2 = q.nn2, p.cert_rex = q.rex, p.cert_walked = q.walked;
          p.T_prev = q.T_prev, p.cert_within2 = q.within2, p.cert_pad = q.cert_pad;
          p.cert_slack_min = q.slack_min, p.cert_slack_max = q.slack_max;
          const size_t lds = std::max<size_t>(words, 1) * 64 * sizeof(uint32_t) * (kTile / 64);
          with_factor(fp->factor_kind, [&](auto f) { hipLaunchKernelGGL((certify_linearize_kernel<Real, decltype(f)::value, 1>), dim3(blocks), dim3(kTile), lds, ctx->stream, p, q); });
        }
        break;
      case Route::kFusedLane:
        if constexpr (sizeof(Real) == 4) {
          rows = static_cast<int>(sgrid.x);
          if (plan.order_record) {
            SGA_TRY(pb->tile_cost.reserve(sgrid.x));
            SGA_TRY(pb->tile_order.reserve(sgrid.x));
            q.tile_cost = pb->tile_cost.p;
            if (plan.order_use) q.tile_order = pb->tile_order.p;
          }
          const size_t lds = std::max<size_t>(words, 3) * 64 * sizeof(uint32_t);
          with_factor(fp->factor_kind, [&](auto f) {
            if (plan.warm)
              hipLaunchKernelGGL((search_linearize_kernel<Real, decltype(f)::value, true>), sgrid, sblock, lds, ctx->stream, q, p);
            else
              hipLaunchKernelGGL((search_linearize_kernel<Real, decltype(f)::value, false>), sgrid, sblock, lds, ctx->stream, q, p);
          });
        }
        break;
      case Route::kFusedQueue:
      case Route::kQueue: {
        q.inv_leaf = p.kd.n > 0 ? std::ldexp(1.0, p.kd.depth) / static_cast<double>(p.kd.n) : 0.0;
        const dim3 qgrid((sgrid.x + q.chunk_tiles - 1) / q.chunk_tiles);
        const size_t lds = std::max<size_t>(words, 3) * 64 * sizeof(uint32_t);
        if (plan.route == Route::kFusedQueue) {
          if constexpr (sizeof(Real) == 4) {
            rows = static_cast<int>(qgrid.x);
            with_factor(fp->factor_kind, [&](auto f) { hipLaunchKernelGGL((nn_search_queue_kernel<Real, true, decltype(f)::value>), qgrid, sblock, lds, ctx->stream, q, p); });
          }
        } else if (plan.warm)
          hipLaunchKernelGGL((nn_search_queue_kernel<Real, true>), qgrid, sblock, lds, ctx->stream, q, p);
        else
          hipLaunchKernelGGL((nn_search_queue_kernel<Real, false>), qgrid, sblock, lds, ctx->stream, q, p);
        break;
      }
      case Route::kLane:
        if (plan.warm)
          hipLaunchKernelGGL((nn_search_kernel<Real, kSearchBlock, true>), sgrid, sblock, words * kSearchBlock * sizeof(uint32_t), ctx->stream, q);
        else
          hipLaunchKernelGGL((nn_search_kernel<Real, kSearchBlock, false>), sgrid, sblock, words * kSearchBlock * sizeof(uint32_t), ctx->stream, q);
        break;
      case Route::kFactors: break;
    }
    if (timed) {
      (void)hipEventRecord(ctx->ev_mid, ctx->stream);
      ctx->mid_recorded = true;
    }
    if (host_rejector) {
// ... 551 lines not shown

extern "C" {

int sga_error(sga_context* ctx, sga_problem* pb, const sga_factor_params* fp, const double T[16], double* e) {
  SGA_TRY(check_args(ctx, pb, fp, T));
  if (!e) return fail(SGA_ERR_INVALID, "null output");
  if (pb->model_valid && fp->robust_kind == SGA_ROBUST_NONE && g_error_model) {
    double Tdev[16];
    *e = evaluate_error_model(pb->model, pb->model_T, problem_pose(pb, T, Tdev));
    return SGA_OK;
  }
  SGA_ENTER(ctx);
  unsigned long long seq = 0;
  SGA_TRY(error_enqueue(ctx, pb, fp, T, &seq));
  return error_collect(ctx, seq, e);
}

int sga_error_model_eval(const double acc96[SGA_MODEL_DOUBLES], const double T_lin[16], const double T[16], double* e) {
  if (!acc96 || !T_lin || !T || !e) return fail(SGA_ERR_INVALID, "null argument");
  *e = evaluate_error_model(acc96, T_lin, T);
  return SGA_OK;
}

void sga_set_error_model(int enabled) { g_error_model = enabled != 0; }

int sga_problem_set_search_stats(sga_context* ctx, sga_problem* pb, int enabled) {
  if (!ctx || !pb) return fail(SGA_ERR_INVALID, "null argument");
  SGA_ENTER(ctx);
  if (enabled) return pb->dbg_leaves.alloc(pb->n);
  pb->dbg_leaves.release();
  return SGA_OK;
}
int sga_problem_get_sorted_points(sga_context* ctx, const sga_problem* pb, float* xyzw) {
  if (!ctx || !pb || !xyzw) return fail(SGA_ERR_INVALID, "null argument");
  if (pb->n == 0) return SGA_OK;
  SGA_ENTER(ctx);
  SGA_HIP(hipMemcpyAsync(xyzw, pb->src_pts(), pb->n * sizeof(float4), hipMemcpyDeviceToHost, ctx->stream));
  SGA_HIP(hipStreamSynchronize(ctx->stream));
  return SGA_OK;
}
int sga_problem_get_last_plan(const sga_problem* pb, int out[8]) {
  if (!pb || !out) return fail(SGA_ERR_INVALID, "null argument");
  std::copy(pb->last_plan, pb->last_plan + 8, out);
  return SGA_OK;
}
int sga_problem_get_search_stats(sga_context* ctx, const sga_problem* pb, int* leaves_per_point) {
  if (!ctx || !pb || !leaves_per_point) return fail(SGA_ERR_INVALID, "null argument");
  if (pb->dbg_leaves.n < pb->n) return fail(SGA_ERR_INVALID, "search statistics are not enabled");
  SGA_ENTER(ctx);
  SGA_HIP(hipMemcpyAsync(leaves_per_point, pb->dbg_leaves.p, pb->n * sizeof(int), hipMemcpyDeviceToHost, ctx->stream));
  SGA_HIP(hipStreamSynchronize(ctx->stream));
  return SGA_OK;
}

#ifdef SGA_KD_TRIPS
int sga_debug_kd_trips(unsigned long long* out16) {
  unsigned long long zero[16] = {0};
  if (hipMemcpyFromSymbol(out16, HIP_SYMBOL(g_kd_trips), sizeof(zero)) != hipSuccess) return SGA_ERR_HIP;
  if (hipMemcpyToSymbol(HIP_SYMBOL(g_kd_trips), zero, sizeof(zero)) != hipSuccess) return SGA_ERR_HIP;
  return SGA_OK;
}
int sga_debug_kd_wave_times(unsigned long long* out, int waves) {
  if (waves > 32768) waves = 32768;
  if (hipMemcpyFromSymbol(out, HIP_SYMBOL(g_kd_wave_times), sizeof(unsigned long long) * 2 * static_cast<size_t>(waves)) != hipSuccess) return SGA_ERR_HIP;
  return SGA_OK;
}
#else
int sga_debug_kd_trips(unsigned long long*) { return fail(SGA_ERR_UNSUPPORTED, "loop-trip counters exist in the diagnostics build only (make trips)"); }
int sga_debug_kd_wave_times(unsigned long long*, int) { return fail(SGA_ERR_UNSUPPORTED, "wave timers exist in the diagnostics build only (make trips)"); }
#endif

}

namespace sga {
void preload_hot_kernels() {
  hipFuncAttributes a;
#define SGA_PRELOAD(...) (void)hipFuncGetAttributes(&a, reinterpret_cast<const void*>(&__VA_ARGS__))
#define SGA_PRELOAD_FACTOR(F)                                        \
  SGA_PRELOAD(search_linearize_kernel<float, F, false>);            \
  SGA_PRELOAD(search_linearize_kernel<float, F, true>);             \
  SGA_PRELOAD(nn_search_queue_kernel<float, true, F>);              \
  SGA_PRELOAD(certify_linearize_kernel<float, F, 1>);               \
  SGA_PRELOAD(linearize_kernel<float, F, 0, kLinPts>);              \
  SGA_PRELOAD(linearize_kernel<float, F, 0, 1>)
  SGA_PRELOAD_FACTOR(SGA_GICP);
  SGA_PRELOAD_FACTOR(SGA_PLANE_ICP);
  SGA_PRELOAD_FACTOR(SGA_ICP);
  SGA_PRELOAD(linearize_kernel<float, SGA_GICP, 1, kLinPts>);
  SGA_PRELOAD(linearize_kernel<float, SGA_GICP, 1, 1>);
  SGA_PRELOAD(reduce_rows_kernel);
  SGA_PRELOAD(tile_order_kernel);
  SGA_PRELOAD(publish_kernel);
  SGA_PRELOAD(error_kernel<float, SGA_GICP>);
#undef SGA_PRELOAD_FACTOR
#undef SGA_PRELOAD
  (void)hipGetLastError();
}
}

extern "C" {

void sga_set_grid_mode(int mode, long long min_points) {
  if (mode >= 0) sga::g_grid_mode = mode;
  if (min_points >= 0) sga::g_grid_min_points = min_points;
}

// ... 8 lines not shown
```

small_gicp_amd/csrc/multi.hip:

```cpp
#include <memory>
#include <vector>

#include "common.hpp"

namespace sga {
int linearize_enqueue(sga_context* ctx, sga_problem* pb, const sga_factor_params* fp, const double T[16], unsigned long long* seq_out, int* count_out);
int linearize_collect(sga_context* ctx, sga_problem* pb, const double T[16], unsigned long long seq, int count);
int error_enqueue(sga_context* ctx, sga_problem* pb, const sga_factor_params* fp, const double T[16], unsigned long long* seq_out);
int error_collect(sga_context* ctx, unsigned long long seq, double* e);
double error_model_value(const double* acc96, const double T_lin[16], const double T[16]);
bool error_model_enabled();
const double* problem_pose(const sga_problem* pb, const double T[16], double Td[16]);
void problem_system_to_caller(const sga_problem* pb, double H[36], double b[6]);
int cloud_create_f32_about(sga_context* ctx, const float* xyz, const float* normals, const float* cov6, size_t n, const double origin[3], sga_cloud** out);
void host_bbox_f32(const float* xyz, size_t n, double lo[3], double hi[3]);
void host_bbox_f64(const double* xyzw, size_t n, double lo[3], double hi[3]);
}

using namespace sga;

struct sga_multi {
  struct Shard {
    int device = 0;
    sga_context* ctx = nullptr;
// ... 263 lines not shown
    m->model_valid = true;
  }
  return SGA_OK;
}

int sga_multi_error(sga_multi* m, const sga_factor_params* fp, const double T[16], double* e) {
  if (!m || !fp || !T || !e) return fail(SGA_ERR_INVALID, "null argument");
  if (!m->has_source) return fail(SGA_ERR_INVALID, "sga_multi_error without clouds");
  if (m->model_valid && fp->robust_kind == SGA_ROBUST_NONE && error_model_enabled()) {
    double Tdev[16];
    *e = error_model_value(m->model, m->model_T, problem_pose(m->shards[0].problem, T, Tdev));
    return SGA_OK;
  }
  const size_t G = m->shards.size();
  std::vector<unsigned long long> seq(G, 0);
  for (size_t g = 0; g < G; g++) {
    auto& s = m->shards[g];
    SGA_HIP(hipSetDevice(s.device));
    Entered in(s.ctx);
    SGA_TRY(error_enqueue(s.ctx, s.problem, fp, T, &seq[g]));
  }
  double sum = 0.0;
  for (size_t g = 0; g < G; g++) {
    auto& s = m->shards[g];
    SGA_HIP(hipSetDevice(s.device));
    Entered in(s.ctx);
    double part = 0.0;
    SGA_TRY(error_collect(s.ctx, seq[g], &part));
    sum += part;
  }
  *e = sum;
  return SGA_OK;
}

int sga_multi_get_factors(sga_multi* m, int64_t* target_index, float* mahalanobis6) {
  if (!m) return fail(SGA_ERR_INVALID, "null argument");
  if (!m->has_source) return fail(SGA_ERR_INVALID, "sga_multi_get_factors without clouds");
  for (auto& s : m->shards) {
    if (s.count == 0) continue;
    SGA_TRY(sga_problem_get_factors(s.ctx, s.problem, target_index ? target_index + s.first : nullptr, mahalanobis6 ? mahalanobis6 + 6 * s.first : nullptr));
  }
  return SGA_OK;
}

int sga_multi_reset_search_state(sga_multi* m) {
  if (!m) return fail(SGA_ERR_INVALID, "null argument");
  for (auto& s : m->shards) {
    if (!s.problem) continue;
    SGA_HIP(hipSetDevice(s.device));
    Entered in(s.ctx);
    sga_problem* pb = s.problem;
    if (pb->n > 0 && pb->hint.n >= pb->n) SGA_HIP(hipMemsetAsync(pb->hint.p, 0xff, pb->n * sizeof(int), s.ctx->stream));
    if (pb->n > 0 && pb->hint2.n >= pb->n) SGA_HIP(hipMemsetAsync(pb->hint2.p, 0xff, pb->n * sizeof(int), s.ctx->stream));
    pb->prev_valid = false;
  }
  m->model_valid = false;
  return SGA_OK;
}

int sga_multi_align(sga_multi* m, const double init_T[16], const sga_registration_setting* setting, sga_result* out) {
  if (!m || !setting || !out) return fail(SGA_ERR_INVALID, "null argument");
  if (!m->has_source) return fail(SGA_ERR_INVALID, "sga_multi_align without clouds");
  static const double I16[16] = {1, 0, 0, 0, 0, 1, 0, 0, 0, 0, 1, 0, 0, 0, 0, 1};
  if (m->n_target <= 10) std::fprintf(stderr, "warning: target point cloud is too small. |target|=%zu\n", m->n_target);
  if (m->n_source <= 10) std::fprintf(stderr, "warning: source point cloud is too small. |source|=%zu\n", m->n_source);
  SGA_TRY(sga_multi_reset_search_state(m));
  MultiReduction r{m, &setting->factor};
  return sga_optimize(setting, init_T ? init_T : I16, multi_lin_cb, multi_err_cb, &r, out);
}

}

namespace {
int multi_lin_cb(void* user, const double T[16], double H[36], double b[6], double* e, uint64_t* inl) {
  auto* r = static_cast<MultiReduction*>(user);
  return sga_multi_linearize(r->m, r->fp, T, H, b, e, inl);
}
int multi_err_cb(void* user, const double T[16], double* e) {
  auto* r = static_cast<MultiReduction*>(user);
  return sga_multi_error(r->m, r->fp, T, e);
}
}
```

small_gicp_amd/csrc/optimizer.hip:

```cpp
#include <cmath>
#include <cstdio>

#include "common.hpp"

namespace sga {

struct M4 {
  double a[16];
};

static M4 mul(const M4& A, const M4& B) {
  M4 C;
  for (int c = 0; c < 4; c++)
    for (int r = 0; r < 4; r++) {
      double s = 0;
      for (int k = 0; k < 4; k++) s += A.a[4 * k + r] * B.a[4 * c + k];
      C.a[4 * c + r] = s;
    }
  return C;
}

static M4 se3_exp(const double d[6]) {
  const double wx = d[0], wy = d[1], wz = d[2];
  const double theta_sq = wx * wx + wy * wy + wz * wz;
// ... 166 lines not shown
};

static int gpu_linearize(void* user, const double T[16], double H[36], double b[6], double* e, uint64_t* inl) {
  auto* g = static_cast<GpuReduction*>(user);
  return sga_linearize(g->ctx, g->pb, g->fp, T, H, b, e, inl);
}
static int gpu_error(void* user, const double T[16], double* e) {
  auto* g = static_cast<GpuReduction*>(user);
  return sga_error(g->ctx, g->pb, g->fp, T, e);
}

}

using namespace sga;

extern "C" {

void sga_registration_setting_default(sga_registration_setting* s) {
  if (!s) return;
  sga_factor_params_default(&s->factor);
  s->optimizer = SGA_LEVENBERG_MARQUARDT;
  s->max_iterations = 20;
  s->max_inner_iterations = 10;
  s->init_lambda = 1e-3;
  s->lambda_factor = 10.0;
  s->gn_lambda = 1e-6;
  s->translation_eps = 1e-3;
  s->rotation_eps = 0.1 * M_PI / 180.0;
  s->verbose = 0;
  s->restrict_dof_lambda = 0.0;
  for (int i = 0; i < 6; i++) s->restrict_dof_mask[i] = 1.0;
}

void sga_se3_exp(const double twist[6], double T[16]) {
  const M4 m = se3_exp(twist);
  memcpy(T, m.a, sizeof(m.a));
}

int sga_optimize(const sga_registration_setting* setting, const double init_T[16], sga_linearize_fn linearize, sga_error_fn error, void* user, sga_result* out) {
  if (!setting || !init_T || !linearize || !out) return fail(SGA_ERR_INVALID, "null argument");
  if (setting->optimizer == SGA_LEVENBERG_MARQUARDT && !error) return fail(SGA_ERR_INVALID, "LM needs an error callback");
  return optimize_impl(*setting, init_T, linearize, error, user, out);
}

int sga_align_problem(sga_context* ctx, sga_problem* problem, const double init_T[16], const sga_registration_setting* setting, sga_result* out) {
  if (!ctx || !problem || !setting || !out) return fail(SGA_ERR_INVALID, "null argument");
  static const double I16[16] = {1, 0, 0, 0, 0, 1, 0, 0, 0, 0, 1, 0, 0, 0, 0, 1};
  if (problem->target->n <= 10) std::fprintf(stderr, "warning: target point cloud is too small. |target|=%zu\n", problem->target->n);
  if (problem->n <= 10) std::fprintf(stderr, "warning: source point cloud is too small. |source|=%zu\n", problem->n);
  if (!problem->state_fresh) {
    SGA_HIP(hipSetDevice(ctx->device));
    if (problem->n > 0) SGA_HIP(hipMemsetAsync(problem->hint.p, 0xff, problem->n * sizeof(int), ctx->stream));
    if (problem->n > 0 && problem->hint2.n >= problem->n) SGA_HIP(hipMemsetAsync(problem->hint2.p, 0xff, problem->n * sizeof(int), ctx->stream));
  }
  problem->prev_valid = false;
  GpuReduction g{ctx, problem, &setting->factor};
  return optimize_impl(*setting, init_T ? init_T : I16, gpu_linearize, gpu_error, &g, out);
}

int sga_align(sga_context* ctx, const sga_index* target, const sga_cloud* source, const double init_T[16], const sga_registration_setting* setting, sga_result* out) {
  if (!ctx || !target || !source || !setting || !out) return fail(SGA_ERR_INVALID, "null argument");
  sga_problem* pb = nullptr;
  SGA_TRY(sga_problem_create(ctx, target, source, init_T, &pb));
  const int rc = sga_align_problem(ctx, pb, init_T, setting, out);
  sga_problem_destroy(pb);
  return rc;
}

}
```

small_gicp_amd/csrc/problem.hip:

```cpp
#include "common.hpp"

#include <cmath>
#include <memory>
#include <rocprim/rocprim.hpp>
#include "device_math.hpp"
#include "kd_search.hpp"
#include "sort_util.hpp"
#include "voxel_hash.hpp"

namespace sga {

int ensure_temp(sga_context* ctx, size_t bytes);
size_t problem_partials_doubles(size_t n);
int problem_ensure_maha(sga_context* ctx, sga_problem* pb);
int cloud_bbox(sga_context* ctx, const float4* pts, size_t n, float lo[3], float hi[3]);
int projective_source_keys(sga_context* ctx, const sga_index* idx, const float4* pts, size_t n, const double T_dev[16], unsigned long long* keys, uint32_t* vals);
int projective_index_knn(sga_context* ctx, const sga_index* index, const float* queries, const double* queries64, size_t m, int k, double max_sq_dist, int64_t* idx, float* sq_dist, double* sq_dist64);

__device__ __forceinline__ unsigned long long spread3(unsigned long long v) {
  v &= 0x1fffffull;
  v = (v | (v << 32)) & 0x1f00000000ffffull;
  v = (v | (v << 16)) & 0x1f0000ff0000ffull;
  v = (v | (v << 8)) & 0x100f00f00f00f00full;
  v = (v | (v << 4)) & 0x10c30c30c30c30c3ull;
// ... 154 lines not shown
  auto push = [&](long long index, float d) {
    if (d > max_sq || d >= d2[k - 1]) return;
    int loc = min(found, k - 1);
    for (; loc > 0 && d < d2[loc - 1]; loc--) {
      idx[loc] = idx[loc - 1];
      d2[loc] = d2[loc - 1];
    }
    idx[loc] = index;
    d2[loc] = d;
    found = min(found + 1, k);
  };
  auto scan = [&](int ox, int oy, int oz) {
    const int vox = flat_voxel_at(v, cx + ox, cy + oy, cz + oz);
    if (vox < 0) return;
    const uint32_t n = FLAT ? v.vnum[vox] : 1u;
    for (uint32_t i = 0; i < n; i++) {
      const float4 p = FLAT ? pts[static_cast<size_t>(vox) * kFlatCap + i] : pts[vox];
      const double dx = static_cast<double>(p.x) - qx, dy = static_cast<double>(p.y) - qy, dz = static_cast<double>(p.z) - qz;
      push((static_cast<long long>(vox) << 32) | static_cast<long long>(i), static_cast<float>(dx * dx + dy * dy + dz * dz));
    }
  };
  scan(0, 0, 0);
  if (v.offsets == 27) {
    for (int a = -1; a <= 1; a++)
      for (int b = -1; b <= 1; b++)
        for (int c = -1; c <= 1; c++) scan(a, b, c);
  } else {
    if (v.offsets == 7) {
      scan(1, 0, 0);
      scan(0, 1, 0);
      scan(0, 0, 1);
      scan(-1, 0, 0);
      scan(0, -1, 0);
      scan(0, 0, -1);
    }
  }
}

}

using namespace sga;

extern "C" {

void sga_factor_params_default(sga_factor_params* p) {
  if (!p) return;
  p->factor_kind = SGA_GICP;
  p->robust_kind = SGA_ROBUST_NONE;
  p->robust_c = 1.0;
  p->max_dist_sq = 1.0;
  p->math_mode = SGA_MATH_FP32;
}

__global__ void problem_state_init_kernel(int* __restrict__ corr, int* __restrict__ hint, int* __restrict__ hint2, uint32_t* __restrict__ walked, size_t n) {
  const size_t i = blockIdx.x * static_cast<size_t>(blockDim.x) + threadIdx.x;
  if (i < n) corr[i] = hint[i] = hint2[i] = -1;
  if (i < n / 64 + 1) walked[i] = 0u;
}

static int problem_alloc_state(sga_context* ctx, sga_problem* pb, size_t n, bool has_covs, bool own_arrays = true) {
  SGA_TRY(pb->partials.alloc(problem_partials_doubles(n)));
  SGA_TRY(pb->walked.alloc(n / 64 + 1));
  if (n > 0 && own_arrays) {
    SGA_TRY(pb->pts.alloc(n));
    if (has_covs) SGA_TRY(pb->cov.alloc(n));
  }
  if (n > 0) {
    SGA_TRY(pb->corr.alloc(n));
    SGA_TRY(pb->hint.alloc(n));
    SGA_TRY(pb->hint2.alloc(n));
    SGA_TRY(pb->rex.alloc(n));
    SGA_TRY(pb->maha.alloc(n * 6));
  }
  hipLaunchKernelGGL(problem_state_init_kernel, dim3((n + 255) / 256 + 1), dim3(256), 0, ctx->stream, pb->corr.p, pb->hint.p, pb->hint2.p, pb->walked.p, n);
  SGA_HIP(hipGetLastError());
  pb->state_fresh = true;
  return SGA_OK;
}

int sga_problem_create_from_index(sga_context* ctx, const sga_index* target, const sga_index* source, const double init_T[16], sga_problem** out) {
  if (!ctx || !target || !source || !out) return fail(SGA_ERR_INVALID, "null argument");
  if (target->device != ctx->device || source->device != ctx->device) return fail(SGA_ERR_INVALID, "target/source live on another device");
  if (source->kind == SGA_INDEX_PROJECTIVE) return fail(SGA_ERR_UNSUPPORTED, "a projective search cannot serve as the source index: pass its cloud");
  if (source->kind != SGA_INDEX_KDTREE) return fail(SGA_ERR_INVALID, "the source index must be a kd-tree");
  (void)init_T;
  *out = nullptr;
  SGA_ENTER(ctx);
  SGA_TRY(wait_ready(ctx, target->ready));
  SGA_TRY(wait_ready(ctx, source->ready));
  std::unique_ptr<sga_problem> pb(new sga_problem);
  pb->device = ctx->device;
  pb->target = target;
  pb->n = source->n;
  pb->has_normals = source->has_normals;
  pb->has_covs = source->has_covs;
  const size_t n = source->n;
  SGA_TRY(problem_alloc_state(ctx, pb.get(), n, source->has_covs, false));
  if (n > 0) {
    for (int k = 0; k < 3; k++) pb->src_origin[k] = source->origin[k];
    pb->pts_view = source->kd_pts.p;
    pb->cov_view = source->has_covs ? source->cov.p : nullptr;
    for (int k = 0; k < 3; k++) {
      pb->bbox_lo[k] = source->bbox_lo[k];
      pb->bbox_hi[k] = source->bbox_hi[k];
    }
  }
  *out = pb.release();
  return SGA_OK;
}

int sga_problem_create(sga_context* ctx, const sga_index* target, const sga_cloud* source, const double init_T[16], sga_problem** out) {
  if (!ctx || !target || !source || !out) return fail(SGA_ERR_INVALID, "null argument");
  if (target->device != ctx->device || source->device != ctx->device) return fail(SGA_ERR_INVALID, "target/source live on another device");
  *out = nullptr;
  SGA_ENTER(ctx);
  SGA_TRY(wait_ready(ctx, target->ready));
  SGA_TRY(wait_ready(ctx, source->ready));
  static const double I16[16] = {1, 0, 0, 0, 0, 1, 0, 0, 0, 0, 1, 0, 0, 0, 0, 1};
  double T[16];
  pose_to_device(init_T ? init_T : I16, source->origin, target->origin, T);
  std::unique_ptr<sga_problem> pb(new sga_problem);
  pb->device = ctx->device;
  pb->target = target;
  pb->n = source->n;
  for (int k = 0; k < 3; k++) pb->src_origin[k] = source->origin[k];
  pb->has_normals = source->has_normals;
  pb->has_covs = source->has_covs;
// ... 184 lines not shown
```

Baseline: 8896 iterations/s.

## Track third-nearest candidate in correspondence certificates to widen warm-start radius

Extends the grid and kd-tree searches from tracking the top two neighbours to the top three, plus the fourth distance as the certificate bound. A third hint array is stored per source point, and the certify pass checks all three cached candidates. The larger certified radius should let more points skip a full re-search on later iterations. The cost is extra registers, a 64-bit compare per offered point, and one more int array written per search. A debug getter for certificates is also added.

```diff
diff --git a/include/small_gicp_amd_debug.h b/include/small_gicp_amd_debug.h
--- a/include/small_gicp_amd_debug.h
+++ b/include/small_gicp_amd_debug.h
@@ -10,6 +10,7 @@
 int sga_problem_set_search_stats(sga_context* ctx, sga_problem* pb, int enabled);
 int sga_problem_get_search_stats(sga_context* ctx, const sga_problem* pb, int* leaves_per_point);
 int sga_problem_get_sorted_points(sga_context* ctx, const sga_problem* pb, float* xyzw);
+int sga_problem_get_certificates(sga_context* ctx, const sga_problem* pb, int* cand, float* rex);
 int sga_problem_get_last_plan(const sga_problem* pb, int out[8]);
 int sga_problem_get_grid_stats(const sga_problem* pb, uint64_t out[6]);
 void sga_set_grid_mode(int mode, long long min_points);
diff --git a/small_gicp_amd/_lib.py b/small_gicp_amd/_lib.py
--- a/small_gicp_amd/_lib.py
+++ b/small_gicp_amd/_lib.py
@@ -138,6 +138,7 @@
     ("sga_problem_set_search_stats", C.c_int, [C.c_void_p, C.c_void_p, C.c_int]),
     ("sga_problem_get_search_stats", C.c_int, [C.c_void_p, C.c_void_p, C.c_void_p]),
     ("sga_problem_get_sorted_points", C.c_int, [C.c_void_p, C.c_void_p, C.c_void_p]),
+    ("sga_problem_get_certificates", C.c_int, [C.c_void_p, C.c_void_p, C.c_void_p, C.c_void_p]),
     ("sga_problem_get_grid_stats", C.c_int, [C.c_void_p, C.POINTER(C.c_uint64)]),
     ("sga_problem_get_last_plan", C.c_int, [C.c_void_p, C.POINTER(C.c_int)]),
     ("sga_set_grid_mode", None, [C.c_int, C.c_longlong]),
diff --git a/small_gicp_amd/api.py b/small_gicp_amd/api.py
--- a/small_gicp_amd/api.py
+++ b/small_gicp_amd/api.py
@@ -781,6 +781,12 @@
         check(load().sga_problem_get_sorted_points(self.ctx.h, self.h, out.ctypes.data_as(C.c_void_p)))
         return out
 
+    def certificates(self):
+        cand = np.zeros((len(self.source), 3), dtype=np.int32)
+        rex = np.zeros(len(self.source), dtype=np.float32)
+        check(load().sga_problem_get_certificates(self.ctx.h, self.h, cand.ctypes.data_as(C.c_void_p), rex.ctypes.data_as(C.c_void_p)))
+        return cand, rex
+
     def pass_stats(self):
         c, w, f = C.c_uint64(), C.c_uint64(), C.c_uint64()
         check(load().sga_problem_get_pass_stats(self.ctx.h, self.h, C.byref(c), C.byref(w), C.byref(f)))
diff --git a/small_gicp_amd/csrc/cell_grid.hip b/small_gicp_amd/csrc/cell_grid.hip
--- a/small_gicp_amd/csrc/cell_grid.hip
+++ b/small_gicp_amd/csrc/cell_grid.hip
@@ -170,6 +170,7 @@
   float bound2;
   int* __restrict__ nn;
   int* __restrict__ nn2;
+  int* __restrict__ nn3;
   float* __restrict__ rex;
   int chunk_tiles;
   uint32_t* __restrict__ stats;
@@ -191,11 +192,12 @@
   Real x, y, z;
   transform_point<Real>(p.T, ps.x, ps.y, ps.z, x, y, z);
   const float qx = static_cast<float>(x), qy = static_cast<float>(y), qz = static_cast<float>(z);
-  int nn, nn2;
+  int nn, nn2, nn3;
   float rex, seen;
-  if (grid_ring1_lane(g, qx, qy, qz, p.bound2, nn, nn2, rex, seen)) {
+  if (grid_ring1_lane(g, qx, qy, qz, p.bound2, nn, nn2, nn3, rex, seen)) {
     p.nn[i] = nn;
     p.nn2[i] = nn2;
+    p.nn3[i] = nn3;
     p.rex[i] = rex;
   } else {
     p.rex[i] = seen < 3.0e38f ? -fmaxf(seen, 1e-30f) : -INFINITY;
@@ -249,7 +251,7 @@
       for (int sft = 32; sft >= 1; sft >>= 1) R = max(R, __shfl_xor(R, sft, 64));
       if (R == 0) break;
       if (mine) ring_sum += static_cast<unsigned>(r);
-      GridTop3 t = grid_top3();
+      GridTop4 t = grid_top4();
       const int xlo = max(cx - r, 0), xhi = min(cx + r, g.nx - 1);
       for (int dz = -R; dz <= R; dz++) {
         const int zz = cz + dz;
@@ -270,11 +272,12 @@
         for (int u = 0; u < 8; u++) grid_scan_run(g, s[u], e[u], qx, qy, qz, t);
       }
       if (mine) {
-        int nn, nn2;
+        int nn, nn2, nn3;
         float rex;
-        if (grid_settle(t, grid_rho2(g, qx, qy, qz, cx, cy, cz, r), p.bound2, nn, nn2, rex)) {
+        if (grid_settle(t, grid_rho2(g, qx, qy, qz, cx, cy, cz, r), p.bound2, nn, nn2, nn3, rex)) {
           p.nn[i] = nn;
           p.nn2[i] = nn2;
+          p.nn3[i] = nn3;
           p.rex[i] = rex;
           done = true;
         } else {
@@ -290,12 +293,13 @@
       open &= open - 1ull;
       const float ux = __shfl(qx, l, 64), uy = __shfl(qy, l, 64), uz = __shfl(qz, l, 64), useen = __shfl(seen, l, 64);
       const int ui = __shfl(i, l, 64);
-      int nn, nn2;
+      int nn, nn2, nn3;
       float rex;
-      ring_sum += grid_settle_wave(g, lane, ux, uy, uz, useen, p.bound2, nn, nn2, rex);
+      ring_sum += grid_settle_wave(g, lane, ux, uy, uz, useen, p.bound2, nn, nn2, nn3, rex);
       if (lane == 0) {
         p.nn[ui] = nn;
         p.nn2[ui] = nn2;
+        p.nn3[ui] = nn3;
         p.rex[ui] = rex;
       }
     }
@@ -311,7 +315,7 @@
 }
 
 template <typename Real>
-int grid_search_pass(sga_context* ctx, const sga_index* idx, const float4* src_pts, int n, const Rigid<Real>& T, float reach2, int* nn, int* nn2, float* rex, uint32_t* stats) {
+int grid_search_pass(sga_context* ctx, const sga_index* idx, const float4* src_pts, int n, const Rigid<Real>& T, float reach2, int* nn, int* nn2, int* nn3, float* rex, uint32_t* stats) {
   static const int chunk_tiles = std::min(16, std::max(1, getenv("SGA_GRID_CHUNK") ? atoi(getenv("SGA_GRID_CHUNK")) : 4));
   GridParams<Real> p{};
   p.src_pts = src_pts;
@@ -321,6 +325,7 @@
   p.bound2 = reach2;
   p.nn = nn;
   p.nn2 = nn2;
+  p.nn3 = nn3;
   p.rex = rex;
   p.chunk_tiles = chunk_tiles;
   p.stats = stats;
@@ -331,8 +336,8 @@
   SGA_HIP(hipGetLastError());
   return SGA_OK;
 }
-template int grid_search_pass<float>(sga_context*, const sga_index*, const float4*, int, const Rigid<float>&, float, int*, int*, float*, uint32_t*);
-template int grid_search_pass<double>(sga_context*, const sga_index*, const float4*, int, const Rigid<double>&, float, int*, int*, float*, uint32_t*);
+template int grid_search_pass<float>(sga_context*, const sga_index*, const float4*, int, const Rigid<float>&, float, int*, int*, int*, float*, uint32_t*);
+template int grid_search_pass<double>(sga_context*, const sga_index*, const float4*, int, const Rigid<double>&, float, int*, int*, int*, float*, uint32_t*);
 
 int grid_rings_for(const sga_index* idx, double reach) {
   if (idx->grid_h <= 0.f) return -1;
diff --git a/small_gicp_amd/csrc/cell_grid.hpp b/small_gicp_amd/csrc/cell_grid.hpp
--- a/small_gicp_amd/csrc/cell_grid.hpp
+++ b/small_gicp_amd/csrc/cell_grid.hpp
@@ -32,20 +32,37 @@
   return min(max(c, 1), n - 2);
 }
 
-struct GridTop3 {
-  unsigned long long k1, k2;
-  float d3;
+struct GridTop4 {
+  unsigned long long k1, k2, k3;
+  float d4;
 };
 constexpr unsigned long long kGridNoKey = (0x7f800000ull << 32) | 0x7fffffffull;
-__device__ __forceinline__ GridTop3 grid_top3() { return {kGridNoKey, kGridNoKey, INFINITY}; }
+__device__ __forceinline__ GridTop4 grid_top4() { return {kGridNoKey, kGridNoKey, kGridNoKey, INFINITY}; }
 __device__ __forceinline__ float grid_key_dist(unsigned long long k) { return __uint_as_float(static_cast<uint32_t>(k >> 32)); }
 __device__ __forceinline__ int grid_key_pos(unsigned long long k) { return static_cast<int>(static_cast<uint32_t>(k)); }
-__device__ __forceinline__ void grid_offer(GridTop3& s, float d, uint32_t pos) {
+__device__ __forceinline__ void grid_offer(GridTop4& s, float d, uint32_t pos) {
   const unsigned long long key = (static_cast<unsigned long long>(__float_as_uint(d)) << 32) | pos;
-  const bool lt1 = key < s.k1, lt2 = key < s.k2;
-  s.d3 = __builtin_amdgcn_fmed3f(grid_key_dist(s.k2), s.d3, d);
+  const bool lt1 = key < s.k1, lt2 = key < s.k2, lt3 = key < s.k3;
+  s.d4 = __builtin_amdgcn_fmed3f(grid_key_dist(s.k3), s.d4, d);
+  s.k3 = lt2 ? s.k2 : (lt3 ? key : s.k3);
   s.k2 = lt1 ? s.k1 : (lt2 ? key : s.k2);
   s.k1 = lt1 ? key : s.k1;
+}
+
+template <class Min64, class MinF>
+__device__ __forceinline__ GridTop4 grid_merge_top4(const GridTop4& t, Min64 min64, MinF minf) {
+  GridTop4 m;
+  m.k1 = min64(t.k1);
+  int taken = t.k1 == m.k1 ? 1 : 0;
+  const unsigned long long c2 = taken == 0 ? t.k1 : t.k2;
+  m.k2 = min64(c2);
+  taken += c2 == m.k2 ? 1 : 0;
+  const unsigned long long c3 = taken == 0 ? t.k1 : (taken == 1 ? t.k2 : t.k3);
+  m.k3 = min64(c3);
+  taken += c3 == m.k3 ? 1 : 0;
+  const float d4 = taken == 0 ? grid_key_dist(t.k1) : (taken == 1 ? grid_key_dist(t.k2) : (taken == 2 ? grid_key_dist(t.k3) : t.d4));
+  m.d4 = minf(d4);
+  return m;
 }
 
 struct GridBatch {
@@ -57,14 +74,14 @@
   for (int u = 0; u < 4; u++) b.c[u] = g.pts[j + u < e ? j + u : 0u];
   return b;
 }
-__device__ __forceinline__ void grid_offer4(const GridBatch& b, uint32_t j, uint32_t e, float qx, float qy, float qz, GridTop3& t) {
+__device__ __forceinline__ void grid_offer4(const GridBatch& b, uint32_t j, uint32_t e, float qx, float qy, float qz, GridTop4& t) {
 #pragma unroll
   for (int u = 0; u < 4; u++) {
     const bool v = j + u < e;
     grid_offer(t, v ? kd_dist2(b.c[u].x, b.c[u].y, b.c[u].z, qx, qy, qz) : INFINITY, v ? __float_as_uint(b.c[u].w) : 0x7fffffffu);
   }
 }
-__device__ __forceinline__ void grid_scan_run(const GridView& g, uint32_t s, uint32_t e, float qx, float qy, float qz, GridTop3& t) {
+__device__ __forceinline__ void grid_scan_run(const GridView& g, uint32_t s, uint32_t e, float qx, float qy, float qz, GridTop4& t) {
   uint32_t j = s;
   while (__ballot(j < e) != 0ull) {
     const GridBatch b = grid_load4(g, j, e);
@@ -89,18 +106,19 @@
 
 __device__ __forceinline__ float grid_rex_from_r2(float r2) { return sqrtf(r2) * 0.9999995f; }
 
-__device__ __forceinline__ bool grid_settle(const GridTop3& t, float rho2, float bound2, int& nn, int& nn2, float& rex, bool* by_face = nullptr) {
+__device__ __forceinline__ bool grid_settle(const GridTop4& t, float rho2, float bound2, int& nn, int& nn2, int& nn3, float& rex, bool* by_face = nullptr) {
   const float d1 = grid_key_dist(t.k1);
   const bool hit = d1 < bound2;
   const bool settled = d1 < rho2 || rho2 >= bound2;
   nn = hit ? grid_key_pos(t.k1) : -1;
   nn2 = (hit && t.k2 != kGridNoKey) ? grid_key_pos(t.k2) : -1;
-  rex = grid_rex_from_r2(fminf(hit ? t.d3 : d1, rho2));
-  if (by_face != nullptr) *by_face = rho2 < (hit ? t.d3 : d1);
+  nn3 = (hit && t.k3 != kGridNoKey) ? grid_key_pos(t.k3) : -1;
+  rex = grid_rex_from_r2(fminf(hit ? t.d4 : d1, rho2));
+  if (by_face != nullptr) *by_face = rho2 < (hit ? t.d4 : d1);
   return settled;
 }
 
-__device__ __forceinline__ bool grid_ring1_lane(const GridView& g, float qx, float qy, float qz, float bound2, int& nn, int& nn2, float& rex, float& seen, bool* by_face = nullptr) {
+__device__ __forceinline__ bool grid_ring1_lane(const GridView& g, float qx, float qy, float qz, float bound2, int& nn, int& nn2, int& nn3, float& rex, float& seen, bool* by_face = nullptr) {
   const int cx = grid_cell(qx, g.ox, g.inv_h, g.nx), cy = grid_cell(qy, g.oy, g.inv_h, g.ny), cz = grid_cell(qz, g.oz, g.inv_h, g.nz);
   uint32_t s[9], e[9];
 #pragma unroll
@@ -111,7 +129,7 @@
     s[r] = g.start[row - 1];
     e[r] = g.start[row + 2];
   }
-  GridTop3 t = grid_top3();
+  GridTop4 t = grid_top4();
   GridBatch nxt = grid_load4(g, s[0], e[0]);
 #pragma unroll
   for (int r = 0; r < 9; r++) {
@@ -121,7 +139,7 @@
     grid_scan_run(g, s[r] + 4u, e[r], qx, qy, qz, t);
   }
   seen = t.k1 != kGridNoKey ? sqrtf(grid_key_dist(t.k1)) : INFINITY;
-  return grid_settle(t, grid_rho2(g, qx, qy, qz, cx, cy, cz, 1), bound2, nn, nn2, rex, by_face);
+  return grid_settle(t, grid_rho2(g, qx, qy, qz, cx, cy, cz, 1), bound2, nn, nn2, nn3, rex, by_face);
 }
 
 __device__ __forceinline__ unsigned long long grid_wave_min_u64(unsigned long long v) {
@@ -146,7 +164,7 @@
   return static_cast<int>(fminf(fmaxf(rr, 2.f), 1.0e6f));
 }
 
-__device__ __forceinline__ unsigned grid_settle_wave(const GridView& g, int lane, float ux, float uy, float uz, float useen, float bound2, int& nn, int& nn2, float& rex) {
+__device__ __forceinline__ unsigned grid_settle_wave(const GridView& g, int lane, float ux, float uy, float uz, float useen, float bound2, int& nn, int& nn2, int& nn3, float& rex) {
   const float reach = sqrtf(bound2) * 1.00001f;
   const int rcap = max(max(g.nx, g.ny), g.nz);
   const int ucx = grid_cell(ux, g.ox, g.inv_h, g.nx), ucy = grid_cell(uy, g.oy, g.inv_h, g.ny), ucz = grid_cell(uz, g.oz, g.inv_h, g.nz);
@@ -157,7 +175,7 @@
     const int W = 2 * ur + 1, rows = W * W;
     const float inv_w = 1.0f / static_cast<float>(W);
     const int xlo = max(ucx - ur, 0), xhi = min(ucx + ur, g.nx - 1);
-    GridTop3 t = grid_top3();
+    GridTop4 t = grid_top4();
     for (int base = 0; base < rows; base += 64) {
       const int k = base + lane;
       int a = static_cast<int>((static_cast<float>(k) + 0.5f) * inv_w);
@@ -172,21 +190,14 @@
       }
       grid_scan_run(g, s, e, ux, uy, uz, t);
     }
-    const unsigned long long g1 = grid_wave_min_u64(t.k1);
-    const unsigned long long c2 = t.k1 == g1 ? t.k2 : t.k1;
-    const unsigned long long g2 = grid_wave_min_u64(c2);
-    const float third = t.k1 == g1 ? (t.k2 == g2 ? t.d3 : grid_key_dist(t.k2)) : (t.k1 == g2 ? grid_key_dist(t.k2) : grid_key_dist(t.k1));
-    GridTop3 m;
-    m.k1 = g1;
-    m.k2 = g2;
-    m.d3 = grid_wave_min_f32(third);
-    if (grid_settle(m, grid_rho2(g, ux, uy, uz, ucx, ucy, ucz, ur), bound2, nn, nn2, rex)) return ring_sum;
-    const float d1 = sqrtf(grid_key_dist(g1));
+    const GridTop4 m = grid_merge_top4(t, grid_wave_min_u64, grid_wave_min_f32);
+    if (grid_settle(m, grid_rho2(g, ux, uy, uz, ucx, ucy, ucz, ur), bound2, nn, nn2, nn3, rex)) return ring_sum;
+    const float d1 = sqrtf(grid_key_dist(m.k1));
     ur = min(max(ur + 1, d1 < 3.0e38f ? grid_ring_for(g, fminf(d1 * 1.00001f, reach), ux, uy, uz, ucx, ucy, ucz) : ur + 1), rcap + 1);
   }
 }
 
-__device__ __forceinline__ bool grid_ring1_group(const GridView& g, int G, int gl, bool has, float qx, float qy, float qz, float bound2, int& nn, int& nn2, float& rex, float& seen, bool* by_face = nullptr) {
+__device__ __forceinline__ bool grid_ring1_group(const GridView& g, int G, int gl, bool has, float qx, float qy, float qz, float bound2, int& nn, int& nn2, int& nn3, float& rex, float& seen, bool* by_face = nullptr) {
   const int cx = grid_cell(qx, g.ox, g.inv_h, g.nx), cy = grid_cell(qy, g.oy, g.inv_h, g.ny), cz = grid_cell(qz, g.oz, g.inv_h, g.nz);
   uint32_t off[9], pre[10];
   pre[0] = 0u;
@@ -198,7 +209,7 @@
     pre[r + 1] = pre[r] + (e - s);
   }
   const uint32_t total = pre[9];
-  GridTop3 t = grid_top3();
+  GridTop4 t = grid_top4();
   for (uint32_t c0 = static_cast<uint32_t>(gl); __ballot(c0 < total) != 0ull; c0 += 4u * static_cast<uint32_t>(G)) {
     float4 cand[4];
     bool ok[4];
@@ -222,15 +233,13 @@
     }
     return v;
   };
-  const unsigned long long g1 = min_u64(t.k1);
-  const unsigned long long c2 = t.k1 == g1 ? t.k2 : t.k1;
-  const unsigned long long g2 = min_u64(c2);
-  float third = t.k1 == g1 ? (t.k2 == g2 ? t.d3 : grid_key_dist(t.k2)) : (t.k1 == g2 ? grid_key_dist(t.k2) : grid_key_dist(t.k1));
-  for (int sft = G >> 1; sft >= 1; sft >>= 1) third = fminf(third, __shfl_xor(third, sft, 64));
-  GridTop3 m;
-  m.k1 = g1, m.k2 = g2, m.d3 = third;
-  seen = g1 != kGridNoKey ? sqrtf(grid_key_dist(g1)) : INFINITY;
-  return grid_settle(m, grid_rho2(g, qx, qy, qz, cx, cy, cz, 1), bound2, nn, nn2, rex, by_face);
-}
-
-}
+  auto min_f32 = [G](float v) {
+    for (int sft = G >> 1; sft >= 1; sft >>= 1) v = fminf(v, __shfl_xor(v, sft, 64));
+    return v;
+  };
+  const GridTop4 m = grid_merge_top4(t, min_u64, min_f32);
+  seen = m.k1 != kGridNoKey ? sqrtf(grid_key_dist(m.k1)) : INFINITY;
+  return grid_settle(m, grid_rho2(g, qx, qy, qz, cx, cy, cz, 1), bound2, nn, nn2, nn3, rex, by_face);
+}
+
+}
diff --git a/small_gicp_amd/csrc/common.hpp b/small_gicp_amd/csrc/common.hpp
--- a/small_gicp_amd/csrc/common.hpp
+++ b/small_gicp_amd/csrc/common.hpp
@@ -245,6 +245,7 @@
   sga::DevBuf<int> corr;
   sga::DevBuf<int> hint;
   sga::DevBuf<int> hint2;
+  sga::DevBuf<int> hint3;
   sga::DevBuf<float> rex;
   sga::DevBuf<int> dbg_leaves;
   sga::DevBuf<uint32_t> walked;
diff --git a/small_gicp_amd/csrc/kd_search.hpp b/small_gicp_amd/csrc/kd_search.hpp
--- a/small_gicp_amd/csrc/kd_search.hpp
+++ b/small_gicp_amd/csrc/kd_search.hpp
@@ -40,6 +40,7 @@
   float d2;
   int idx;
   int idx2;
+  int idx3;
   float r2;
   int leaves;
 };
@@ -77,7 +78,8 @@
 struct KdState {
   unsigned long long win;
   unsigned long long second;
-  float third;
+  unsigned long long third;
+  float fourth;
   float dropped;
   float prune0;
   float prune;
@@ -105,8 +107,8 @@
 }
 __device__ __forceinline__ KdState kd_state(float prune0, float slack = 0.f) {
   KdState s{};
-  s.win = s.second = kKdNoPoint;
-  s.third = s.dropped = INFINITY;
+  s.win = s.second = s.third = kKdNoPoint;
+  s.fourth = s.dropped = INFINITY;
   s.prune0 = s.prune = prune0;
   s.open = kd_open_bound(prune0, slack);
   s.slack = slack;
@@ -120,8 +122,9 @@
   const bool hit = wd2 < bound2;
   best.idx = hit ? static_cast<int>(static_cast<uint32_t>(s.win)) : -1;
   best.idx2 = (hit && s.second != kKdNoPoint) ? static_cast<int>(static_cast<uint32_t>(s.second)) : -1;
+  best.idx3 = (hit && s.third != kKdNoPoint) ? static_cast<int>(static_cast<uint32_t>(s.third)) : -1;
   best.d2 = hit ? wd2 : bound2;
-  best.r2 = hit ? fminf(s.third, s.dropped) : fminf(wd2, s.dropped);
+  best.r2 = hit ? fminf(s.fourth, s.dropped) : fminf(wd2, s.dropped);
   best.leaves = s.leaves;
   return best;
 }
@@ -138,11 +141,13 @@
   for (int i = 0; i < kKdLeafMax; i++) {
     float d2 = kd_dist2(p[i].x, p[i].y, p[i].z, qx, qy, qz);
     d2 = static_cast<uint32_t>(i) < count ? d2 : INFINITY;
-    s.third = __builtin_amdgcn_fmed3f(kd_key_dist(s.second), s.third, d2);
+    s.fourth = __builtin_amdgcn_fmed3f(kd_key_dist(s.third), s.fourth, d2);
     const unsigned long long key = (static_cast<unsigned long long>(__float_as_uint(d2)) << 32) | (first + static_cast<uint32_t>(i));
-    const bool before_win = key < s.win;
-    const unsigned long long low = key < s.second ? key : s.second;
-    s.second = before_win ? s.win : low;
+    const bool before_win = key < s.win, before_second = key < s.second;
+    const unsigned long long low3 = key < s.third ? key : s.third;
+    s.third = before_second ? s.second : low3;
+    const unsigned long long low2 = before_second ? key : s.second;
+    s.second = before_win ? s.win : low2;
     s.win = before_win ? key : s.win;
   }
   s.prune = fminf(s.prune0, kd_key_dist(s.win));
@@ -154,8 +159,8 @@
 constexpr float kKdFar = 1e18f;
 constexpr uint32_t kKdNoneKey = 0x7149f2cau;
 struct KdFast {
-  uint32_t w1, w2, w3;
-  uint32_t l1, l2;
+  uint32_t w1, w2, w3, w4;
+  uint32_t l1, l2, l3;
   float dropped;
   float prune0;
   float open;
@@ -167,8 +172,8 @@
 };
 __device__ __forceinline__ KdFast kd_fast_state(float prune0, float slack = 0.f) {
   KdFast s{};
-  s.w1 = s.w2 = s.w3 = 0xffffffffu;
-  s.l1 = s.l2 = 0u;
+  s.w1 = s.w2 = s.w3 = s.w4 = 0xffffffffu;
+  s.l1 = s.l2 = s.l3 = 0u;
   s.dropped = INFINITY;
   s.prune0 = prune0;
   s.open = kd_open_bound(prune0, slack);
@@ -187,19 +192,22 @@
   const kd_f32x2 X[4] = {{x0.x, x0.y}, {x0.z, x0.w}, {x1.x, x1.y}, {x1.z, x1.w}};
   const kd_f32x2 Y[4] = {{y0.x, y0.y}, {y0.z, y0.w}, {y1.x, y1.y}, {y1.z, y1.w}};
   const kd_f32x2 Z[4] = {{z0.x, z0.y}, {z0.z, z0.w}, {z1.x, z1.y}, {z1.z, z1.w}};
-  const uint32_t o1 = s.w1, o2 = s.w2;
+  const uint32_t o1 = s.w1, o2 = s.w2, o3 = s.w3;
 #pragma unroll
   for (int i = 0; i < 4; i++) {
     const kd_f32x2 dx = X[i] - qx, dy = Y[i] - qy, dz = Z[i] - qz;
     const kd_f32x2 d2 = __builtin_elementwise_fma(dx, dx, __builtin_elementwise_fma(dy, dy, dz * dz));
     const uint32_t k0 = (__float_as_uint(d2.x) & ~7u) | static_cast<uint32_t>(2 * i), k1 = (__float_as_uint(d2.y) & ~7u) | static_cast<uint32_t>(2 * i + 1);
+    s.w4 = kd_umed3(s.w3, s.w4, k0);
     s.w3 = kd_umed3(s.w2, s.w3, k0);
     s.w2 = kd_umed3(s.w1, s.w2, k0);
     s.w1 = min(s.w1, k0);
+    s.w4 = kd_umed3(s.w3, s.w4, k1);
     s.w3 = kd_umed3(s.w2, s.w3, k1);
     s.w2 = kd_umed3(s.w1, s.w2, k1);
     s.w1 = min(s.w1, k1);
   }
+  s.l3 = s.w3 != o3 ? (s.w3 == o2 ? s.l2 : (s.w3 == o1 ? s.l1 : k)) : s.l3;
   s.l2 = s.w2 != o2 ? (s.w2 == o1 ? s.l1 : k) : s.l2;
   s.l1 = s.w1 != o1 ? k : s.l1;
   s.open = kd_open_bound(fminf(s.prune0, kd_key_hi(s.w1)), s.slack);
@@ -441,7 +449,7 @@
 
 template <int STRIDE>
 __device__ __forceinline__ KdBest kd_nearest(const KdView& t, float qx, float qy, float qz, float bound2, int seed, uint32_t* __restrict__ stack, int tid, float slack = 0.f) {
-  if (t.n == 0) return {bound2, -1, -1, INFINITY, 0};
+  if (t.n == 0) return {bound2, -1, -1, -1, INFINITY, 0};
   float prune0 = bound2;
   if (seed >= 0 && static_cast<uint32_t>(seed) < t.n) {
     const float4 c = t.pts[seed];
@@ -496,15 +504,17 @@
   r.ambiguous = !(hit || miss) || (hit && ((s.w1 ^ s.w2) < 8u));
   r.best.idx = hit ? static_cast<int>(kd_bound(t.n, t.depth, s.l1) + (s.w1 & 7u)) : -1;
   r.best.idx2 = (hit && s.w2 < kKdNoneKey) ? static_cast<int>(kd_bound(t.n, t.depth, s.l2) + (s.w2 & 7u)) : -1;
+  const bool third = s.w3 < kKdNoneKey && s.w3 != s.w2;
+  r.best.idx3 = (hit && third) ? static_cast<int>(kd_bound(t.n, t.depth, s.l3) + (s.w3 & 7u)) : -1;
   r.best.d2 = hit ? lo : bound2;
-  r.best.r2 = hit ? fminf(kd_key_lo(s.w3), s.dropped) : fminf(lo, s.dropped);
+  r.best.r2 = hit ? fminf(kd_key_lo(third ? s.w4 : s.w3), s.dropped) : fminf(lo, s.dropped);
   r.best.leaves = s.leaves;
   return r;
 }
 
 template <int STRIDE>
 __device__ __forceinline__ KdBestFast kd_nearest_fast(const KdView& t, float qx, float qy, float qz, float bound2, int seed, uint32_t* __restrict__ stack, int tid, float slack = 0.f) {
-  if (t.n == 0) return {{bound2, -1, -1, INFINITY, 0}, false};
+  if (t.n == 0) return {{bound2, -1, -1, -1, INFINITY, 0}, false};
   float prune0 = bound2;
   if (seed >= 0 && static_cast<uint32_t>(seed) < t.n) {
     const float4 c = t.pts[seed];
diff --git a/small_gicp_amd/csrc/linearize.hip b/small_gicp_amd/csrc/linearize.hip
--- a/small_gicp_amd/csrc/linearize.hip
+++ b/small_gicp_amd/csrc/linearize.hip
@@ -17,7 +17,7 @@
 
 int comm_allreduce_sum(sga_context* ctx, double* d_buf, size_t count);
 template <typename Real>
-int grid_search_pass(sga_context* ctx, const sga_index* idx, const float4* src_pts, int n, const Rigid<Real>& T, float reach2, int* nn, int* nn2, float* rex, uint32_t* stats);
+int grid_search_pass(sga_context* ctx, const sga_index* idx, const float4* src_pts, int n, const Rigid<Real>& T, float reach2, int* nn, int* nn2, int* nn3, float* rex, uint32_t* stats);
 int grid_rings_for(const sga_index* idx, double reach);
 
 #ifndef SGA_SPACING_REF
@@ -114,6 +114,7 @@
   FusedTail tail;
   int* __restrict__ cert_nn;
   int* __restrict__ cert_nn2;
+  int* __restrict__ cert_nn3;
   float* __restrict__ cert_rex;
   uint32_t* __restrict__ cert_walked;
   Rigid<Real> T_prev;
@@ -160,6 +161,7 @@
   float cert_pad;
   int* __restrict__ nn;
   int* __restrict__ nn2;
+  int* __restrict__ nn3;
   float* __restrict__ rex;
   int check;
   Rigid<Real> T_prev;
@@ -182,6 +184,20 @@
   return ok ? lim * 0.9999995f : -1.f;
 }
 
+__device__ __forceinline__ int cert_nearest(const int (&c)[3], const float (&d)[3], float& best_d2) {
+  int slot = 0, cb = c[0];
+  float db = d[0];
+#pragma unroll
+  for (int k = 1; k < 3; k++) {
+    const bool nearer = c[k] >= 0 && (d[k] < db || (d[k] == db && c[k] < cb));
+    slot = nearer ? k : slot;
+    cb = nearer ? c[k] : cb;
+    db = nearer ? d[k] : db;
+  }
+  best_d2 = db;
+  return slot;
+}
+
 template <typename Real, int BLOCK>
 __device__ __forceinline__ int walk_lane(const NNParams<Real>& p, int i, float fx, float fy, float fz, int seed, float slack, uint32_t* __restrict__ kd_stack, int tid) {
   KdBest nb{};
@@ -194,6 +210,7 @@
   if (exact) nb = kd_nearest<BLOCK>(p.kd, fx, fy, fz, p.bound2, seed, kd_stack, tid, slack);
   p.nn[i] = nb.idx;
   p.nn2[i] = nb.idx2;
+  p.nn3[i] = nb.idx3;
   p.rex[i] = rex_from_r2(nb.r2);
   if (p.leaves != nullptr) p.leaves[i] = nb.leaves;
   return nb.idx;
@@ -207,24 +224,25 @@
     Real ox, oy, oz;
     transform_point<Real>(p.T_prev, ps.x, ps.y, ps.z, ox, oy, oz);
     const float moved = sqrtf(kd_dist2(static_cast<float>(ox), static_cast<float>(oy), static_cast<float>(oz), fx, fy, fz));
-    const int cand2 = p.nn2[i];
-    float d1 = INFINITY, d2 = INFINITY;
-    if (seed >= 0) {
-      const float4 c = p.kd.pts[seed];
-      d1 = kd_dist2(c.x, c.y, c.z, fx, fy, fz);
-    }
-    if (cand2 >= 0) {
-      const float4 c = p.kd.pts[cand2];
-      d2 = kd_dist2(c.x, c.y, c.z, fx, fy, fz);
-    }
-    const bool swap = cand2 >= 0 && (d2 < d1 || (d2 == d1 && cand2 < seed));
-    const int best = swap ? cand2 : seed;
-    const float r = certify(p.rex[i], moved, best >= 0, swap ? d2 : d1, p.within2, p.cert_pad);
+    const int c[3] = {seed, p.nn2[i], p.nn3[i]};
+    float d[3];
+#pragma unroll
+    for (int k = 0; k < 3; k++) {
+      d[k] = INFINITY;
+      if (c[k] >= 0) {
+        const float4 m = p.kd.pts[c[k]];
+        d[k] = kd_dist2(m.x, m.y, m.z, fx, fy, fz);
+      }
+    }
+    float best_d2;
+    const int slot = cert_nearest(c, d, best_d2);
+    const int best = c[slot];
+    const float r = certify(p.rex[i], moved, best >= 0, best_d2, p.within2, p.cert_pad);
     if (r >= 0.f) {
       p.rex[i] = r;
-      if (swap) {
-        p.nn[i] = cand2;
-        p.nn2[i] = seed;
+      if (slot != 0) {
+        p.nn[i] = best;
+        (slot == 1 ? p.nn2 : p.nn3)[i] = seed;
       }
       return best;
     }
@@ -233,12 +251,13 @@
     const unsigned long long walking = __ballot(true);
     if (threadIdx.x == __ffsll(static_cast<long long>(walking)) - 1) p.walked[tile] += static_cast<uint32_t>(__popcll(walking));
     if (p.grid_walk & 2) {
-      int g_nn, g_nn2;
+      int g_nn, g_nn2, g_nn3;
       float g_rex, g_seen;
       bool g_face = false;
-      if (grid_ring1_lane(p.grid, fx, fy, fz, p.bound2, g_nn, g_nn2, g_rex, g_seen, &g_face) && !(g_face && g_nn >= 0 && (p.grid_walk & 32) && g_rex - g_seen < slack)) {
+      if (grid_ring1_lane(p.grid, fx, fy, fz, p.bound2, g_nn, g_nn2, g_nn3, g_rex, g_seen, &g_face) && !(g_face && g_nn >= 0 && (p.grid_walk & 32) && g_rex - g_seen < slack)) {
         p.nn[i] = g_nn;
         p.nn2[i] = g_nn2;
+        p.nn3[i] = g_nn3;
         p.rex[i] = g_rex;
         return g_nn;
       }
@@ -336,23 +355,25 @@
           Real ox, oy, oz;
           transform_point<Real>(p.T_prev, ps.x, ps.y, ps.z, ox, oy, oz);
           const float moved = sqrtf(kd_dist2(static_cast<float>(ox), static_cast<float>(oy), static_cast<float>(oz), fx, fy, fz));
-          float d1 = INFINITY, d2 = INFINITY;
-          if (seed >= 0) {
-            const float4 c = p.kd.pts[seed];
-            d1 = kd_dist2(c.x, c.y, c.z, fx, fy, fz);
+          const int c[3] = {seed, cand2, p.nn3[i]};
+          float d[3];
+#pragma unroll
+          for (int k = 0; k < 3; k++) {
+            d[k] = INFINITY;
+            if (c[k] >= 0) {
+              const float4 m = p.kd.pts[c[k]];
+              d[k] = kd_dist2(m.x, m.y, m.z, fx, fy, fz);
+            }
           }
-          if (cand2 >= 0) {
-            const float4 c = p.kd.pts[cand2];
-            d2 = kd_dist2(c.x, c.y, c.z, fx, fy, fz);
-          }
-          const bool swap = cand2 >= 0 && (d2 < d1 || (d2 == d1 && cand2 < seed));
-          const int best = swap ? cand2 : seed;
-          const float r = certify(p.rex[i], moved, best >= 0, swap ? d2 : d1, p.within2, p.cert_pad);
+          float best_d2;
+          const int slot = cert_nearest(c, d, best_d2);
+          const int best = c[slot];
+          const float r = certify(p.rex[i], moved, best >= 0, best_d2, p.within2, p.cert_pad);
           if (r >= 0.f) {
             p.rex[i] = r;
-            if (swap) {
-              p.nn[i] = cand2;
-              p.nn2[i] = seed;
+            if (slot != 0) {
+              p.nn[i] = best;
+              (slot == 1 ? p.nn2 : p.nn3)[i] = seed;
             }
             need = false;
           }
@@ -414,12 +435,13 @@
           const bool trying = busy && fresh;
           if (__ballot(trying) != 0ull) {
             if (trying) {
-              int g_nn, g_nn2;
+              int g_nn, g_nn2, g_nn3;
               float g_rex, g_seen;
               bool g_face = false;
-              if (grid_ring1_lane(p.grid, qx, qy, qz, p.bound2, g_nn, g_nn2, g_rex, g_seen, &g_face) && !(g_face && g_nn >= 0 && (p.grid_walk & 32) && g_rex - g_seen < s.slack)) {
+              if (grid_ring1_lane(p.grid, qx, qy, qz, p.bound2, g_nn, g_nn2, g_nn3, g_rex, g_seen, &g_face) && !(g_face && g_nn >= 0 && (p.grid_walk & 32) && g_rex - g_seen < s.slack)) {
                 p.nn[qi] = g_nn;
                 p.nn2[qi] = g_nn2;
+                p.nn3[qi] = g_nn3;
                 p.rex[qi] = g_rex;
                 busy = false;
                 fresh = false;
@@ -449,6 +471,7 @@
         const KdBest nb = kd_result(s, p.bound2);
         p.nn[qi] = nb.idx;
         p.nn2[qi] = nb.idx >= 0 ? nb.idx2 : -2 - static_cast<int>(node - (1u << D));
+        p.nn3[qi] = nb.idx3;
         p.rex[qi] = rex_from_r2(nb.r2);
         busy = false;
       }
@@ -725,21 +748,23 @@
   if constexpr (TARGET != 2 && TARGET != 3) {
     float4 m4[PTS];
     if constexpr (CERT && TARGET == 0) {
-      int c2[PTS];
+      int c2[PTS], c3[PTS];
       float rx[PTS];
-      float4 m4b[PTS];
+      float4 m4b[PTS], m4c[PTS];
       {
         SGA_STAGE_PARAMS(p);
 #pragma unroll
         for (int u = 0; u < PTS; u++) {
           const int i = first + u * stride;
           c2[u] = act[u] ? p.cert_nn2[i] : -1;
+          c3[u] = act[u] ? p.cert_nn3[i] : -1;
           rx[u] = act[u] ? p.cert_rex[i] : 0.f;
         }
 #pragma unroll
         for (int u = 0; u < PTS; u++) {
           m4[u] = jn[u] >= 0 ? p.tgt_pts[jn[u]] : make_float4(0.f, 0.f, 0.f, 0.f);
           m4b[u] = c2[u] >= 0 ? p.tgt_pts[c2[u]] : make_float4(0.f, 0.f, 0.f, 0.f);
+          m4c[u] = c3[u] >= 0 ? p.tgt_pts[c3[u]] : make_float4(0.f, 0.f, 0.f, 0.f);
         }
       }
       SGA_STAGE_PARAMS(p);
@@ -752,17 +777,20 @@
           Real ox, oy, oz;
           transform_point<Real>(p.T_prev, P[u][0], P[u][1], P[u][2], ox, oy, oz);
           const float moved = sqrtf(kd_dist2(static_cast<float>(ox), static_cast<float>(oy), static_cast<float>(oz), fx, fy, fz));
-          const float d1 = jn[u] >= 0 ? kd_dist2(m4[u].x, m4[u].y, m4[u].z, fx, fy, fz) : INFINITY;
-          const float d2 = c2[u] >= 0 ? kd_dist2(m4b[u].x, m4b[u].y, m4b[u].z, fx, fy, fz) : INFINITY;
-          const bool swap = c2[u] >= 0 && (d2 < d1 || (d2 == d1 && c2[u] < jn[u]));
-          const int best = swap ? c2[u] : jn[u];
-          const float r = certify(rx[u], moved, best >= 0, swap ? d2 : d1, p.cert_within2, p.cert_pad);
+          const int c[3] = {jn[u], c2[u], c3[u]};
+          const float d[3] = {jn[u] >= 0 ? kd_dist2(m4[u].x, m4[u].y, m4[u].z, fx, fy, fz) : INFINITY,
+                              c2[u] >= 0 ? kd_dist2(m4b[u].x, m4b[u].y, m4b[u].z, fx, fy, fz) : INFINITY,
+                              c3[u] >= 0 ? kd_dist2(m4c[u].x, m4c[u].y, m4c[u].z, fx, fy, fz) : INFINITY};
+          float best_d2;
+          const int slot = cert_nearest(c, d, best_d2);
+          const int best = c[slot];
+          const float r = certify(rx[u], moved, best >= 0, best_d2, p.cert_within2, p.cert_pad);
           failed = !(r >= 0.f);
           p.cert_rex[i] = failed ? -fminf(fmaxf(moved, p.cert_slack_min), p.cert_slack_max) : r;
-          if (swap) {
-            p.cert_nn[i] = c2[u];
-            p.cert_nn2[i] = jn[u];
-            m4[u] = m4b[u];
+          if (slot != 0) {
+            p.cert_nn[i] = best;
+            (slot == 1 ? p.cert_nn2 : p.cert_nn3)[i] = jn[u];
+            m4[u] = slot == 1 ? m4b[u] : m4c[u];
           }
           jn[u] = failed ? -1 : best;
         }
@@ -786,16 +814,18 @@
         for (int u = 0; u < PTS; u++) {
           const int i = first + u * stride;
           if (!act[u] || jn[u] < 0) continue;
-          const int j2 = p.cert_nn2[i];
+          const int jc[2] = {p.cert_nn2[i], p.cert_nn3[i]};
           const double ax = static_cast<double>(m4[u].x) - Q[u][0], ay = static_cast<double>(m4[u].y) - Q[u][1], az = static_cast<double>(m4[u].z) - Q[u][2];
           double d1 = ax * ax + ay * ay + az * az;
-          if (j2 >= 0) {
-            const float4 c = p.tgt_pts[j2];
+#pragma unroll
+          for (int k = 0; k < 2; k++) {
+            if (jc[k] < 0) continue;
+            const float4 c = p.tgt_pts[jc[k]];
             const double bx = static_cast<double>(c.x) - Q[u][0], by = static_cast<double>(c.y) - Q[u][1], bz = static_cast<double>(c.z) - Q[u][2];
             const double d2 = bx * bx + by * by + bz * bz;
-            if (d2 < d1 || (d2 == d1 && j2 < jn[u])) {
+            if (d2 < d1 || (d2 == d1 && jc[k] < jn[u])) {
               d1 = d2;
-              jn[u] = j2;
+              jn[u] = jc[k];
               m4[u] = c;
             }
           }
@@ -959,7 +989,7 @@
         Sym3<Real> Mh{};
         bool inl = false;
         bool g_settled = false;
-        int g_nn = -1, g_nn2 = -1;
+        int g_nn = -1, g_nn2 = -1, g_nn3 = -1;
         float g_rex = 0.f, g_seen = INFINITY;
         bool g_face = false;
         if (Gw > 1) {
@@ -970,7 +1000,7 @@
             transform_point<Real>(p.T, Real(ps.x), Real(ps.y), Real(ps.z), t[0], t[1], t[2]);
             gx = static_cast<float>(t[0]), gy = static_cast<float>(t[1]), gz = static_cast<float>(t[2]);
           }
-          g_settled = grid_ring1_group(q.grid, Gw, gl, has, gx, gy, gz, q.bound2, g_nn, g_nn2, g_rex, g_seen, &g_face);
+          g_settled = grid_ring1_group(q.grid, Gw, gl, has, gx, gy, gz, q.bound2, g_nn, g_nn2, g_nn3, g_rex, g_seen, &g_face);
         }
         if (mine) {
           const float4 ps = p.src_pts[i];
@@ -980,7 +1010,7 @@
           const float fx = static_cast<float>(t[0]), fy = static_cast<float>(t[1]), fz = static_cast<float>(t[2]);
           int j = -1;
           bool settled = g_settled;
-          if (Gw == 1 && (q.grid_walk & 1)) settled = grid_ring1_lane(q.grid, fx, fy, fz, q.bound2, g_nn, g_nn2, g_rex, g_seen, &g_face);
+          if (Gw == 1 && (q.grid_walk & 1)) settled = grid_ring1_lane(q.grid, fx, fy, fz, q.bound2, g_nn, g_nn2, g_nn3, g_rex, g_seen, &g_face);
           if (settled && g_face && g_nn >= 0 && (q.grid_walk & 32)) {
             const float need = -__hip_atomic_load(&q.rex[i], __ATOMIC_RELAXED, __HIP_MEMORY_SCOPE_AGENT);
             if (g_rex - g_seen < need) settled = false;
@@ -988,6 +1018,7 @@
           if (settled) {
             q.nn[i] = g_nn;
             q.nn2[i] = g_nn2;
+            q.nn3[i] = g_nn3;
             q.rex[i] = g_rex;
             j = g_nn;
           }
@@ -1517,6 +1548,7 @@
     p.kd = make_kd_view(idx);
   }
   p.cert_nn2 = (!voxel && sizeof(Real) == 8) ? pb->hint2.p : nullptr;
+  p.cert_nn3 = (!voxel && sizeof(Real) == 8) ? pb->hint3.p : nullptr;
   p.store_maha = fp->robust_kind != SGA_ROBUST_NONE ? 1 : 0;
   p.partials = pb->partials.p;
   const int ncols = kModelCols, out_n = with_model ? kRow : SGA_ACCUM_DOUBLES;
@@ -1533,7 +1565,7 @@
   q.slack_min = static_cast<float>(kSlackMin * unit), q.slack_max = static_cast<float>(kSlackMax * unit);
   q.cert_pad = std::max(g_cert_pad, 0.f);
   q.bound2 = p.bound2 * (1.f + kSearchMargin) * (1.f + kSearchMargin);
-  q.nn = pb->hint.p, q.nn2 = pb->hint2.p, q.rex = pb->rex.p, q.walked = pb->walked.p;
+  q.nn = pb->hint.p, q.nn2 = pb->hint2.p, q.nn3 = pb->hint3.p, q.rex = pb->rex.p, q.walked = pb->walked.p;
   q.fast = g_fast_scan;
   q.leaves = pb->dbg_leaves.n >= pb->n ? pb->dbg_leaves.p : nullptr;
 
@@ -1571,12 +1603,12 @@
           SGA_TRY(pb->grid_stats.alloc(4));
           SGA_HIP(hipMemsetAsync(pb->grid_stats.p, 0, 4 * sizeof(uint32_t), ctx->stream));
         }
-        SGA_TRY(grid_search_pass<Real>(ctx, idx, pb->src_pts(), p.n, p.T, q.bound2, pb->hint.p, pb->hint2.p, pb->rex.p, pb->grid_stats.p));
+        SGA_TRY(grid_search_pass<Real>(ctx, idx, pb->src_pts(), p.n, p.T, q.bound2, pb->hint.p, pb->hint2.p, pb->hint3.p, pb->rex.p, pb->grid_stats.p));
         pb->grid_passes++;
         break;
       case Route::kCertify:
         if constexpr (sizeof(Real) == 4) {
-          p.cert_nn = q.nn, p.cert_nn2 = q.nn2, p.cert_rex = q.rex, p.cert_walked = q.walked;
+          p.cert_nn = q.nn, p.cert_nn2 = q.nn2, p.cert_nn3 = q.nn3, p.cert_rex = q.rex, p.cert_walked = q.walked;
           p.T_prev = q.T_prev, p.cert_within2 = q.within2, p.cert_pad = q.cert_pad;
           p.cert_slack_min = q.slack_min, p.cert_slack_max = q.slack_max;
           const size_t lds = std::max<size_t>(words, 1) * 64 * sizeof(uint32_t) * (kTile / 64);
@@ -2234,6 +2266,18 @@
   SGA_HIP(hipStreamSynchronize(ctx->stream));
   return SGA_OK;
 }
+int sga_problem_get_certificates(sga_context* ctx, const sga_problem* pb, int* cand, float* rex) {
+  if (!ctx || !pb || !cand || !rex) return fail(SGA_ERR_INVALID, "null argument");
+  if (pb->n == 0) return SGA_OK;
+  if (pb->hint.n < pb->n || pb->hint2.n < pb->n || pb->hint3.n < pb->n || pb->rex.n < pb->n) return fail(SGA_ERR_INVALID, "the problem holds no certificates");
+  SGA_ENTER(ctx);
+  SGA_HIP(hipMemcpy2DAsync(cand, 3 * sizeof(int), pb->hint.p, sizeof(int), sizeof(int), pb->n, hipMemcpyDeviceToHost, ctx->stream));
+  SGA_HIP(hipMemcpy2DAsync(cand + 1, 3 * sizeof(int), pb->hint2.p, sizeof(int), sizeof(int), pb->n, hipMemcpyDeviceToHost, ctx->stream));
+  SGA_HIP(hipMemcpy2DAsync(cand + 2, 3 * sizeof(int), pb->hint3.p, sizeof(int), sizeof(int), pb->n, hipMemcpyDeviceToHost, ctx->stream));
+  SGA_HIP(hipMemcpyAsync(rex, pb->rex.p, pb->n * sizeof(float), hipMemcpyDeviceToHost, ctx->stream));
+  SGA_HIP(hipStreamSynchronize(ctx->stream));
+  return SGA_OK;
+}
 
 #ifdef SGA_KD_TRIPS
 int sga_debug_kd_trips(unsigned long long* out16) {
diff --git a/small_gicp_amd/csrc/multi.hip b/small_gicp_amd/csrc/multi.hip
--- a/small_gicp_amd/csrc/multi.hip
+++ b/small_gicp_amd/csrc/multi.hip
@@ -339,6 +339,7 @@
     sga_problem* pb = s.problem;
     if (pb->n > 0 && pb->hint.n >= pb->n) SGA_HIP(hipMemsetAsync(pb->hint.p, 0xff, pb->n * sizeof(int), s.ctx->stream));
     if (pb->n > 0 && pb->hint2.n >= pb->n) SGA_HIP(hipMemsetAsync(pb->hint2.p, 0xff, pb->n * sizeof(int), s.ctx->stream));
+    if (pb->n > 0 && pb->hint3.n >= pb->n) SGA_HIP(hipMemsetAsync(pb->hint3.p, 0xff, pb->n * sizeof(int), s.ctx->stream));
     pb->prev_valid = false;
   }
   m->model_valid = false;
diff --git a/small_gicp_amd/csrc/optimizer.hip b/small_gicp_amd/csrc/optimizer.hip
--- a/small_gicp_amd/csrc/optimizer.hip
+++ b/small_gicp_amd/csrc/optimizer.hip
@@ -242,6 +242,7 @@
     SGA_HIP(hipSetDevice(ctx->device));
     if (problem->n > 0) SGA_HIP(hipMemsetAsync(problem->hint.p, 0xff, problem->n * sizeof(int), ctx->stream));
     if (problem->n > 0 && problem->hint2.n >= problem->n) SGA_HIP(hipMemsetAsync(problem->hint2.p, 0xff, problem->n * sizeof(int), ctx->stream));
+    if (problem->n > 0 && problem->hint3.n >= problem->n) SGA_HIP(hipMemsetAsync(problem->hint3.p, 0xff, problem->n * sizeof(int), ctx->stream));
   }
   problem->prev_valid = false;
   GpuReduction g{ctx, problem, &setting->factor};
diff --git a/small_gicp_amd/csrc/problem.hip b/small_gicp_amd/csrc/problem.hip
--- a/small_gicp_amd/csrc/problem.hip
+++ b/small_gicp_amd/csrc/problem.hip
@@ -230,9 +230,9 @@
   p->math_mode = SGA_MATH_FP32;
 }
 
-__global__ void problem_state_init_kernel(int* __restrict__ corr, int* __restrict__ hint, int* __restrict__ hint2, uint32_t* __restrict__ walked, size_t n) {
+__global__ void problem_state_init_kernel(int* __restrict__ corr, int* __restrict__ hint, int* __restrict__ hint2, int* __restrict__ hint3, uint32_t* __restrict__ walked, size_t n) {
   const size_t i = blockIdx.x * static_cast<size_t>(blockDim.x) + threadIdx.x;
-  if (i < n) corr[i] = hint[i] = hint2[i] = -1;
+  if (i < n) corr[i] = hint[i] = hint2[i] = hint3[i] = -1;
   if (i < n / 64 + 1) walked[i] = 0u;
 }
 
@@ -247,10 +247,11 @@
     SGA_TRY(pb->corr.alloc(n));
     SGA_TRY(pb->hint.alloc(n));
     SGA_TRY(pb->hint2.alloc(n));
+    SGA_TRY(pb->hint3.alloc(n));
     SGA_TRY(pb->rex.alloc(n));
     SGA_TRY(pb->maha.alloc(n * 6));
   }
-  hipLaunchKernelGGL(problem_state_init_kernel, dim3((n + 255) / 256 + 1), dim3(256), 0, ctx->stream, pb->corr.p, pb->hint.p, pb->hint2.p, pb->walked.p, n);
+  hipLaunchKernelGGL(problem_state_init_kernel, dim3((n + 255) / 256 + 1), dim3(256), 0, ctx->stream, pb->corr.p, pb->hint.p, pb->hint2.p, pb->hint3.p, pb->walked.p, n);
   SGA_HIP(hipGetLastError());
   pb->state_fresh = true;
   return SGA_OK;
```

Result: no change. 8814 iterations/s, median of 2 (-0.9%).
